# uc-vision/smart-tree

Measured on AMD Instinct MI355X. Metric: points/sec end-to-end (voxelize->sparse-UNet->skeleton), 1M-pt tree, higher is better.
Workload: dtype f32

## Files before the change

### include/smarttree_hip.h

```cpp
#ifndef SMARTTREE_HIP_H
#define SMARTTREE_HIP_H

#include <stdint.h>

#ifdef __cplusplus
extern "C" {
#endif

int st_version(void);
#define ST_SKELETON_STATS_ENTRIES 16
#define ST_SKELETON_TUNING_ENTRIES 24
int st_abi_entries(int what);
const char* st_last_error(void);
int64_t st_query_workspace(int op, int64_t a, int64_t b, int64_t c);

int64_t st_scan_workspace_bytes(int64_t n);
int st_scan_u32(const uint32_t* in, uint32_t* out, int64_t n, uint32_t* total, void* ws, int64_t ws_bytes, void* stream);
int64_t st_sort_workspace_bytes(int64_t n);
int st_sort_pairs_u32(uint32_t* keys, uint32_t* vals, int64_t n, int key_bits, void* ws, int64_t ws_bytes, void* stream);

int64_t st_voxelize_workspace_bytes(int64_t n_points, int max_blocks, int64_t max_voxels);
int st_voxelize_blocks(const float* xyz, const float* rgb, int64_t n, double voxel_size, double block_size,
                       double buffer_size, int min_points, int max_blocks, int64_t max_voxels, float* feats,
                       int32_t* coords, uint8_t* mask, int64_t* point_index, float* block_centres,
                       int64_t* n_voxels_host, int64_t* n_blocks_host, void* ws, int64_t ws_bytes, void* stream);

int64_t st_hash_capacity(int64_t n);
int st_build_coord_hash(const int32_t* coords, int64_t n, unsigned long long* keys, unsigned* vals, int64_t cap, void* stream);
int st_build_subm_rulebook(const int32_t* coords, int64_t n, const unsigned long long* keys, const unsigned* vals,
                           int64_t cap, int32_t* nbr , void* stream);
int64_t st_spatial_order_workspace_bytes(int64_t n);
int st_spatial_order(const int32_t* coords, int64_t n, int32_t* order , void* ws, int64_t ws_bytes, void* stream);
int st_move_rows(const void* src, int row_words, const int32_t* order, int64_t n, void* dst, int scatter, void* stream);
int64_t st_strided_workspace_bytes(int64_t n_fine);
int st_build_strided_outputs(const int32_t* coords, int64_t n, int64_t max_out, int32_t* out_coords,
                             unsigned long long* ckeys, unsigned* cvals, int64_t ccap, int64_t* n_out_host,
                             int32_t* extent_host , void* ws, int64_t ws_bytes, void* stream);
int st_build_strided_rulebook(const int32_t* coords, int64_t n, const unsigned long long* fkeys, const unsigned* fvals,
                              int64_t fcap, const int32_t* out_coords, int64_t n_out, const unsigned long long* ckeys,
                              const unsigned* cvals, int64_t ccap, const int32_t* extent_host,
                              int32_t* nbr_down , int32_t* nbr_up ,
                              int32_t* up_order ,
                              void* stream);

int st_sparse_conv_fwd(const float* x0, int c0, const float* x1, int cin, const int32_t* nbr, int K, int64_t n_out,
                       const float* w, int cout, const float* scale, const float* shift, const float* residual,
                       int relu, float* y, const int32_t* row_order ,
                       void* stream, int64_t nbr_stride );
int st_sparse_conv_mfma_fwd(const float* x0, int c0, const float* x1, int cin, const int32_t* nbr, int K, int64_t n_out,
                            const float* wp, int cout, const float* scale, const float* shift, const float* residual,
                            int relu, float* y, const int32_t* row_order ,
                            void* stream, int64_t nbr_stride ,
                            int variant );
int st_sparse_conv_b3_fwd(const float* x0, int c0, const float* x1, int cin, const int32_t* nbr, int K, int64_t n_out, const void* wq,
                          int cout, const float* scale, const float* shift, const float* residual, int relu, float* y,
                          const int32_t* row_order, void* stream, int64_t nbr_stride, int variant);
int st_sparse_conv_f16_fwd(const void* x0, int c0, const void* x1, int cin, const int32_t* nbr, int K, int64_t n_out,
                           const void* w, int cout, const float* scale, const float* shift, const void* residual, int relu,
                           void* y, int in_half, int out_half, const int32_t* row_order, void* stream, int64_t nbr_stride );

int64_t st_brick_pyramid_workspace_bytes(int64_t n0, int n_blocks, int coord_bound, int depth, const int64_t* caps);
int st_brick_pyramid(const int32_t* coords0 , int64_t n0, int n_blocks ,
                     int coord_bound , int depth, const int32_t* blk_seg ,
                     int nseg, const int64_t* caps ,
                     int32_t* order0 , int32_t* const* coords_out ,
                     int32_t* const* subm , int32_t* const* down ,
                     int32_t* const* up , int32_t* const* up_order ,
                     int64_t* counts_host , void* ws, int64_t ws_bytes, void* stream);
int st_head_param_floats(void);
int st_pointwise_mlp_heads(const float* x, int64_t n, const float* params, float* radius, float* direction,
                           float* class_l, float* medial_vector , int64_t* class_idx , void* stream);

int st_centre_cloud(const float* xyz, int64_t n, float* out, void* ws, int64_t ws_bytes, void* stream);
int st_medial_points(const float* xyz, const float* mv, int64_t n, float* medial, float* radius, void* stream);
int64_t st_knn_workspace_bytes(int64_t n_dst);
int st_knn_radius(const float* src, int64_t n1, const float* dst, int64_t n2, int K, float r, const float* bound,
                  int bound_mode, float cell_hint, int64_t* idx, float* dist, void* ws, int64_t ws_bytes, void* stream);
int64_t st_make_edges_workspace_bytes(int64_t n);
int st_make_edges(const int64_t* idx, const float* dist, int64_t n, int K, int64_t* edges, float* w,
                  int64_t* n_edges_host, void* ws, int64_t ws_bytes, void* stream);
int64_t st_connected_components_workspace_bytes(int64_t n);
int st_connected_components(const int64_t* edges, int64_t E, int64_t n, int32_t* labels, void* ws, int64_t ws_bytes, void* stream);
int64_t st_component_layout_workspace_bytes(int64_t n);
int st_component_layout(const int32_t* labels, int64_t n, int min_vertices, int32_t* comp_size, int32_t* comp_off,
                        int32_t* vert_order, int32_t* new_id, int64_t* n_comp_host, int64_t* n_kept_host, void* ws,
                        int64_t ws_bytes, void* stream);
int64_t st_component_csr_workspace_bytes(int64_t m);
int st_component_csr(const int64_t* edges, const float* w, int64_t E, const int32_t* new_id, int64_t m, uint32_t* row_off,
                     uint32_t* col, float* wgt, void* ws, int64_t ws_bytes, void* stream);
int64_t st_skeleton_workspace_bytes(int64_t m, int64_t n_comp);
int st_skeleton_components(int n_comp, const int32_t* comp_off, const int32_t* comp_size_host, int64_t m, const float* pts,
                           const float* rad, const float* ysurf, const uint32_t* row_off, const uint32_t* col,
                           const float* wgt, float grid_cell, int stages, int block_threads, float* dist, int32_t* pred,
                           int32_t* root_local, float* tree_dist, int32_t* branch_parent, int32_t* branch_off,
                           int32_t* branch_len, int32_t* n_branches, int32_t* path_verts, int32_t* branch_of,
                           int64_t* stats_host, void* ws, int64_t ws_bytes, void* stream);
#define ST_SKELETON_STAGE_ARGS                                                                                          \
    int n_comp, const int32_t *comp_off, const int32_t *comp_size_host, int64_t m, const float *pts, const float *rad, \
        const float *ysurf, const uint32_t *row_off, const uint32_t *col, const float *wgt, float grid_cell,           \
        int block_threads, float *dist, int32_t *pred, int32_t *root_local, float *tree_dist, int32_t *branch_parent,  \
        int32_t *branch_off, int32_t *branch_len, int32_t *n_branches, int32_t *path_verts, int32_t *branch_of,        \
        int64_t *stats_host, void *ws, int64_t ws_bytes, void *stream
int st_sssp(ST_SKELETON_STAGE_ARGS);
int st_tree_distance(ST_SKELETON_STAGE_ARGS);
int st_sample_tree(ST_SKELETON_STAGE_ARGS);
int64_t st_assemble_workspace_bytes(int64_t cap_b);
int st_assemble_branches(int n_comp, const int32_t* comp_off, const int32_t* n_branches, const int32_t* branch_parent,
                         const int32_t* branch_off, const int32_t* branch_len, const int32_t* path_verts,
                         const int32_t* vert_order, const float* medial, const float* radius, int32_t* tree_off,
                         int32_t* parent, int32_t* start, int32_t* length, float* xyz, float* rad, int64_t cap_b,
                         int64_t cap_p, int64_t* counts_host, void* ws, int64_t ws_bytes, void* stream);
int st_post_process(int n_trees, const int32_t* tree_off, const int32_t* parent, const int32_t* start, const int32_t* len,
                    float* xyz, const float* rad_in, float* rad_out, uint8_t* keep, uint8_t* repaired, uint8_t* smoothed,
                    int32_t* depth_scratch, int do_prune, float min_radius, float min_length, int do_repair, int do_smooth, int kernel_size,
                    void* stream);

int st_points_to_nearest_tube(const float* pts, int64_t n, const float* a, const float* b, const float* r1, const float* r2,
                              int64_t m, float* vec, int64_t* idx, float* rad, void* stream);

int64_t st_sample_tubes_workspace_bytes(int64_t m);
int st_sample_tubes_count(const float* a, const float* b, int64_t m, double spacing, int32_t* count, int32_t* off,
                          int64_t* total_host, void* ws, int64_t ws_bytes, void* stream);
int st_sample_tubes_fill(const float* a, const float* b, const float* r1, const float* r2, int64_t m, double spacing,
                         const int32_t* off, int64_t total, float* pts, float* rad, int32_t* tube_of, void* stream);
int64_t st_skeleton_match_workspace_bytes(int64_t n);
int st_skeleton_match(const float* pts, const float* rad, int64_t n, const float* a, const float* b, const float* r1,
                      const float* r2, int64_t m, const float* thr, int n_thr, int ref_mode, float* dist, int32_t* idx,
                      float* tube_rad, void* tally, void* ws, int64_t ws_bytes, void* stream);

int st_centre_cloud_seg(const float* xyz, int64_t n, const int32_t* seg_off, int nseg, float* out, void* ws,
                        int64_t ws_bytes , void* stream);
int st_centre_cloud_box_seg(const float* xyz, int64_t n, const int32_t* seg_off, int nseg, float* out, void* ws,
                            int64_t ws_bytes , void* stream, float* box_out);
int st_voxelize_blocks_box_seg(const float* xyz, const float* rgb, int64_t n, const int32_t* seg_off, int nseg,
                               double voxel_size, double block_size, double buffer_size, int min_points, int max_blocks,
                               int64_t max_voxels, float* feats, int32_t* coords, uint8_t* mask, int64_t* point_index,
                               float* block_centres, int32_t* blk_seg, int32_t* seg_vox_off, int32_t* seg_blk_off,
                               int64_t* n_voxels_host, int64_t* n_blocks_host, void* ws, int64_t ws_bytes, void* stream,
                               const float* centred_box );
int64_t st_voxelize_workspace_bytes_seg(int64_t n_points, int max_blocks, int64_t max_voxels, int nseg);
int st_voxelize_blocks_seg(const float* xyz, const float* rgb, int64_t n, const int32_t* seg_off, int nseg,
                           double voxel_size, double block_size, double buffer_size, int min_points, int max_blocks,
                           int64_t max_voxels, float* feats, int32_t* coords, uint8_t* mask, int64_t* point_index,
                           float* block_centres, int32_t* blk_seg ,
                           int32_t* seg_vox_off , int32_t* seg_blk_off , int64_t* n_voxels_host,
                           int64_t* n_blocks_host, void* ws, int64_t ws_bytes, void* stream);
int st_build_strided_outputs_seg(const int32_t* coords, int64_t n, int64_t max_out, int32_t* out_coords,
                                 unsigned long long* ckeys, unsigned* cvals, int64_t ccap, int64_t* n_out_host,
                                 int32_t* extent_host, const int32_t* blk_seg, int nseg, int32_t* ext_dev ,
                                 void* ws, int64_t ws_bytes, void* stream);
int st_build_strided_rulebook_seg(const int32_t* coords, int64_t n, const unsigned long long* fkeys, const unsigned* fvals,
                                  int64_t fcap, const int32_t* out_coords, int64_t n_out, const unsigned long long* ckeys,
                                  const unsigned* cvals, int64_t ccap, const int32_t* extent_host, int32_t* nbr_down,
                                  int32_t* nbr_up, int32_t* up_order, const int32_t* blk_seg, const int32_t* ext_dev,
// ... 124 lines not shown
```

### smart_tree_amd/_lib.py

```python
from __future__ import annotations

import ctypes
from ctypes import c_double, c_float, c_int, c_int64, c_void_p
from pathlib import Path

import torch

_PKG = Path(__file__).resolve().parent
LIB_PATH = _PKG / "libsmarttree_hip.so"

_LIB = None
_ALLOW_HOST_POINTERS = False

P = c_void_p
I64 = c_int64

SIGNATURES = {
    "st_version": (c_int, []),
    "st_abi_entries": (c_int, [c_int]),
    "st_last_error": (ctypes.c_char_p, []),
    "st_scan_workspace_bytes": (I64, [I64]),
    "st_scan_u32": (c_int, [P, P, I64, P, P, I64, P]),
    "st_sort_workspace_bytes": (I64, [I64]),
    "st_sort_pairs_u32": (c_int, [P, P, I64, c_int, P, I64, P]),
    "st_voxelize_workspace_bytes": (I64, [I64, c_int, I64]),
    "st_voxelize_blocks": (c_int, [P, P, I64, c_double, c_double, c_double, c_int, c_int, I64, P, P, P, P, P,
                                   ctypes.POINTER(I64), ctypes.POINTER(I64), P, I64, P]),
    "st_hash_capacity": (I64, [I64]),
    "st_build_coord_hash": (c_int, [P, I64, P, P, I64, P]),
    "st_build_subm_rulebook": (c_int, [P, I64, P, P, I64, P, P]),
    "st_strided_workspace_bytes": (I64, [I64]),
    "st_spatial_order_workspace_bytes": (I64, [I64]),
    "st_spatial_order": (c_int, [P, I64, P, P, I64, P]),
    "st_move_rows": (c_int, [P, c_int, P, I64, P, c_int, P]),
    "st_build_strided_outputs": (c_int, [P, I64, I64, P, P, P, I64, ctypes.POINTER(I64), ctypes.POINTER(ctypes.c_int32),
                                         P, I64, P]),
    "st_build_strided_rulebook": (c_int, [P, I64, P, P, I64, P, I64, P, P, I64, ctypes.POINTER(ctypes.c_int32), P, P, P, P]),
    "st_sparse_conv_fwd": (c_int, [P, c_int, P, c_int, P, c_int, I64, P, c_int, P, P, P, c_int, P, P, P, I64]),
    "st_sparse_conv_mfma_fwd": (c_int, [P, c_int, P, c_int, P, c_int, I64, P, c_int, P, P, P, c_int, P, P, P, I64, c_int]),
    "st_sparse_conv_b3_fwd": (c_int, [P, c_int, P, c_int, P, c_int, I64, P, c_int, P, P, P, c_int, P, P, P, I64, c_int]),
    "st_sparse_conv_f16_fwd": (c_int, [P, c_int, P, c_int, P, c_int, I64, P, c_int, P, P, P, c_int, P, c_int, c_int, P, P, I64]),
    "st_brick_pyramid_workspace_bytes": (I64, [I64, c_int, c_int, c_int, ctypes.POINTER(I64)]),
    "st_brick_pyramid": (c_int, [P, I64, c_int, c_int, c_int, P, c_int, ctypes.POINTER(I64), P, ctypes.POINTER(P), ctypes.POINTER(P),
                                 ctypes.POINTER(P), ctypes.POINTER(P), ctypes.POINTER(P), ctypes.POINTER(I64), P, I64, P]),
    "st_head_param_floats": (c_int, []),
    "st_pointwise_mlp_heads": (c_int, [P, I64, P, P, P, P, P, P, P]),
    "st_knn_workspace_bytes": (I64, [I64]),
    "st_knn_radius": (c_int, [P, I64, P, I64, c_int, c_float, P, c_int, c_float, P, P, P, I64, P]),
    "st_medial_points": (c_int, [P, P, I64, P, P, P]),
    "st_centre_cloud": (c_int, [P, I64, P, P, I64, P]),
    "st_make_edges_workspace_bytes": (I64, [I64]),
    "st_make_edges": (c_int, [P, P, I64, c_int, P, P, ctypes.POINTER(I64), P, I64, P]),
    "st_connected_components_workspace_bytes": (c_int64, [c_int64]),
    "st_connected_components": (c_int, [P, I64, I64, P, P, I64, P]),
    "st_component_layout_workspace_bytes": (I64, [I64]),
    "st_component_layout": (c_int, [P, I64, c_int, P, P, P, P, ctypes.POINTER(I64), ctypes.POINTER(I64), P, I64, P]),
    "st_component_csr_workspace_bytes": (I64, [I64]),
    "st_component_csr": (c_int, [P, P, I64, P, I64, P, P, P, P, I64, P]),
    "st_assemble_workspace_bytes": (c_int64, [c_int64]),
    "st_assemble_branches": (c_int, [c_int, P, P, P, P, P, P, P, P, P, P, P, P, P, P, P, c_int64, c_int64, P, P, c_int64, P]),
    "st_points_to_nearest_tube": (c_int, [P, c_int64, P, P, P, P, c_int64, P, P, P, P]),
    "st_post_process": (c_int, [c_int, P, P, P, P, P, P, P, P, P, P, P, c_int, c_float, c_float, c_int, c_int, c_int, P]),
    "st_sample_tubes_workspace_bytes": (I64, [I64]),
    "st_sample_tubes_count": (c_int, [P, P, I64, c_double, P, P, ctypes.POINTER(I64), P, I64, P]),
    "st_sample_tubes_fill": (c_int, [P, P, P, P, I64, c_double, P, I64, P, P, P, P]),
    "st_skeleton_match_workspace_bytes": (I64, [I64]),
    "st_skeleton_match": (c_int, [P, P, I64, P, P, P, P, I64, P, c_int, c_int, P, P, P, P, P, I64, P]),
    "st_skeleton_workspace_bytes": (I64, [I64, I64]),
    "st_synth_points_seg": (c_int, [P, P, P, P, P, P, c_int, P, P, P, P, P, P, P, P, P, P]),
    "st_synth_philox": (None, [P, P, P]),
    "st_prediction_metrics_tally_ints": (I64, [c_int, c_int, c_int]),
    "st_prediction_metrics_tally_sums": (I64, [c_int]),
    "st_prediction_metrics_workspace_bytes": (I64, [I64, c_int, c_int]),
    "st_prediction_metrics": (c_int, [P, P, P, c_int, P, c_int, P, I64, P, c_int, c_int, c_int, P, c_int, P, c_int, P, P, P, I64, P]),
    "st_render_workspace_bytes": (I64, [c_int, c_int, c_int]),
    "st_render_clear": (c_int, [c_int, c_int, c_int, P, I64, P]),
    "st_render_points": (c_int, [P, P, I64, I64, c_float, P, c_int, c_int, c_int, c_float, P, I64, P]),
    "st_render_segments": (c_int, [P, P, P, P, I64, I64, c_float, P, c_int, c_int, c_int, c_float, P, I64, P]),
    "st_render_resolve": (c_int, [P, c_int, c_int, c_int, c_int, c_float, c_int, P, P, P, P, I64, P]),
    "st_centre_cloud_seg": (c_int, [P, I64, P, c_int, P, P, I64, P]),
    "st_centre_cloud_box_seg": (c_int, [P, I64, P, c_int, P, P, I64, P, P]),
    "st_voxelize_blocks_box_seg": (c_int, [P, P, I64, P, c_int, c_double, c_double, c_double, c_int, c_int, I64, P, P, P, P, P, P, P, P,
                                           ctypes.POINTER(I64), ctypes.POINTER(I64), P, I64, P, P]),
    "st_voxelize_workspace_bytes_seg": (I64, [I64, c_int, I64, c_int]),
    "st_voxelize_blocks_seg": (c_int, [P, P, I64, P, c_int, c_double, c_double, c_double, c_int, c_int, I64, P, P, P, P, P, P, P, P,
                                       ctypes.POINTER(I64), ctypes.POINTER(I64), P, I64, P]),
    "st_voxelize_cloud_workspace_bytes": (I64, [I64, I64, c_int]),
    "st_voxelize_cloud_seg": (c_int, [P, P, I64, P, c_int, c_double, I64, P, P, P, P, P, ctypes.POINTER(I64), P, I64, P]),
    "st_loss_workspace_bytes": (I64, []),
    "st_loss_forward": (c_int, [P, P, P, c_int, P, c_int, P, I64, c_int, c_int, ctypes.POINTER(ctypes.c_double), P, I64, P]),
    "st_build_strided_outputs_seg": (c_int, [P, I64, I64, P, P, P, I64, ctypes.POINTER(I64), ctypes.POINTER(ctypes.c_int32),
                                             P, c_int, P, P, I64, P]),
    "st_build_strided_rulebook_seg": (c_int, [P, I64, P, P, I64, P, I64, P, P, I64, ctypes.POINTER(ctypes.c_int32), P, P, P, P, P, P]),
    "st_knn_workspace_bytes_seg": (I64, [I64, c_int]),
    "st_knn_radius_seg": (c_int, [P, I64, P, I64, c_int, c_float, P, c_int, c_float, P, P, P, P, c_int, P, I64, P, c_float]),
    "st_radius_count_seg": (c_int, [P, I64, P, I64, c_int, c_float, P, c_int, c_float, P, P, P, c_int, P, I64, P, c_float, P]),
    "st_connected_components_knn": (c_int, [P, I64, c_int, P, P, P, I64, P]),
    "st_component_csr_knn": (c_int, [P, P, I64, c_int, P, P, I64, P, P, P, P, I64, P]),
    "st_component_csr_knn_workspace_bytes": (I64, [I64, I64, c_int]),
    "st_make_edges_seg": (c_int, [P, P, I64, c_int, P, P, ctypes.POINTER(I64), P, c_int, P, I64, P]),
    "st_component_layout_seg": (c_int, [P, I64, c_int, P, c_int, P, P, P, P, P, P, P, ctypes.POINTER(I64), ctypes.POINTER(I64), P, I64, P,
                                        ctypes.POINTER(I64)]),
    "st_skeleton_workspace_bytes_seg": (I64, [I64, I64, c_int]),
    "st_skeleton_components_seg": (c_int, [c_int, P, P, P, c_int, I64, P, P, P, P, P, P, c_float, c_int, c_int, P, P, P, P, P, P, P, P,
                                           P, P, ctypes.POINTER(I64), P, I64, P, ctypes.POINTER(I64)]),
    "st_post_process_seg": (c_int, [c_int, P, P, P, P, P, P, P, P, P, P, P, c_int, c_float, c_float, c_int, c_int, c_int, P, c_int, P]),
    "st_loss_backward": (c_int, [P, P, P, c_int, P, c_int, P, I64, c_int, c_int, c_double, c_double, P, P, P, P, P]),
    "st_sparse_conv_wgrad_workspace_bytes": (I64, [c_int, c_int, c_int, I64]),
    "st_sparse_conv_wgrad": (c_int, [P, c_int, P, c_int, P, c_int, I64, I64, P, c_int, P, P, I64, P]),
    "st_sparse_conv_h_fwd": (c_int, [P, c_int, P, c_int, P, c_int, I64, I64, P, c_int, P, P]),
    "st_sparse_conv_wgrad_h_workspace_bytes": (I64, [c_int, c_int, c_int, I64]),
    "st_sparse_conv_wgrad_h": (c_int, [P, c_int, P, c_int, P, c_int, I64, I64, P, c_int, P, P, I64, P]),
    "st_move_rows_h": (c_int, [P, c_int, P, I64, P, c_int, P]),
    "st_bn_workspace_bytes": (I64, [I64, c_int]),
    "st_bn_stats": (c_int, [P, c_int, I64, c_int, P, P, I64, P]),
    "st_bn_apply": (c_int, [P, c_int, I64, c_int, P, P, P, P, P, P]),
    "st_bn_backward_stats": (c_int, [P, P, c_int, I64, c_int, P, P, P, P, I64, P]),
    "st_bn_backward_apply": (c_int, [P, P, c_int, I64, c_int, P, P, P, P, P, P, P]),
    "st_bridge_components_workspace_bytes": (I64, [I64, I64, c_int]),
    "st_bridge_components_seg": (c_int, [P, I64, P, I64, P, P, I64, P, c_int, c_float, P, P, I64, ctypes.POINTER(I64),
                                         ctypes.POINTER(I64), P, I64, P]),
    "st_skeleton_components": (c_int, [c_int, P, P, I64, P, P, P, P, P, P, c_float, c_int, c_int, P, P, P, P, P, P, P, P,
                                       P, P, ctypes.POINTER(I64), P, I64, P]),
    "st_segment_workspace_bytes": (I64, [I64, I64, c_int]),
    "st_segment_points_seg": (c_int, [P, I64, P, P, P, P, P, I64, P, c_int, c_float, c_int, P, P, P, P, P, P, I64, P]),
}


ENQUEUE_ONLY = frozenset({
    "st_version", "st_abi_entries", "st_last_error", "st_scan_workspace_bytes", "st_sort_workspace_bytes", "st_voxelize_workspace_bytes",
    "st_hash_capacity", "st_strided_workspace_bytes", "st_head_param_floats", "st_knn_workspace_bytes",
    "st_make_edges_workspace_bytes", "st_connected_components_workspace_bytes", "st_component_layout_workspace_bytes",
    "st_component_csr_workspace_bytes", "st_assemble_workspace_bytes", "st_skeleton_workspace_bytes",
    "st_build_coord_hash", "st_build_subm_rulebook", "st_build_strided_rulebook", "st_sparse_conv_fwd",
    "st_sparse_conv_mfma_fwd", "st_sparse_conv_b3_fwd", "st_sparse_conv_f16_fwd", "st_pointwise_mlp_heads", "st_medial_points", "st_centre_cloud",
    "st_connected_components", "st_component_csr", "st_post_process", "st_knn_radius", "st_brick_pyramid_workspace_bytes",
    "st_centre_cloud_seg", "st_centre_cloud_box_seg", "st_voxelize_workspace_bytes_seg", "st_build_strided_rulebook_seg", "st_knn_workspace_bytes_seg",
    "st_knn_radius_seg", "st_skeleton_workspace_bytes_seg", "st_post_process_seg", "st_radius_count_seg",
    "st_voxelize_cloud_workspace_bytes", "st_loss_workspace_bytes", "st_spatial_order_workspace_bytes", "st_spatial_order", "st_connected_components_knn", "st_component_csr_knn", "st_component_csr_knn_workspace_bytes", "st_move_rows",
    "st_loss_backward", "st_sparse_conv_wgrad_workspace_bytes", "st_sparse_conv_wgrad",
    "st_sparse_conv_h_fwd", "st_sparse_conv_wgrad_h_workspace_bytes", "st_sparse_conv_wgrad_h", "st_move_rows_h",
    "st_bn_workspace_bytes", "st_bn_stats", "st_bn_apply", "st_bn_backward_stats", "st_bn_backward_apply",
    "st_sample_tubes_workspace_bytes", "st_sample_tubes_fill", "st_skeleton_match_workspace_bytes", "st_skeleton_match",
    "st_synth_points_seg", "st_synth_philox",
    "st_prediction_metrics_tally_ints", "st_prediction_metrics_tally_sums", "st_prediction_metrics_workspace_bytes", "st_prediction_metrics",
    "st_render_workspace_bytes", "st_render_clear", "st_render_points", "st_render_segments", "st_render_resolve",
    "st_bridge_components_workspace_bytes", "st_segment_workspace_bytes", "st_segment_points_seg",
})


NOWAIT_VARIANTS = ("st_make_edges", "st_assemble_branches", "st_make_edges_seg")


class StRenderItem(ctypes.Structure):
    _fields_ = [("count", c_int64), ("mode", ctypes.c_int32), ("n_classes", ctypes.c_int32), ("data", c_void_p), ("cmap", c_void_p),
                ("lo", c_float), ("hi", c_float), ("rgb", c_float * 3), ("reserved", c_float)]


class _Bound:

    def __init__(self, cdll):
        self._cdll = cdll

    def __getattr__(self, name):
        return getattr(self._cdll, name)


def declare(cdll, pydll=None):
    out = _Bound(cdll) if pydll is not None else cdll
    for name, (res, args) in SIGNATURES.items():
        for handle in ((cdll, pydll) if pydll is not None else (cdll,)):
            fn = getattr(handle, name)
            fn.restype = res
            fn.argtypes = args
        if pydll is not None:
            setattr(out, name, getattr(pydll if name in ENQUEUE_ONLY else cdll, name))
    for name in NOWAIT_VARIANTS:
        setattr(out, name + "_nowait", getattr(pydll if pydll is not None else cdll, name))
    return out


def lib():
    global _LIB
    if _LIB is None:
        if not LIB_PATH.exists():
            raise RuntimeError(
                f"{LIB_PATH} is missing: the HIP extension has not been built. "
                "Run `python -c 'import __graft_entry__ as g; g.build()'` (needs hipcc). "
                "smart_tree_amd has no CPU fallback.")
        import os
        if os.environ.get("ST_CDLL_ONLY") == "1":
            _LIB = declare(ctypes.CDLL(str(LIB_PATH)))
        else:
            _LIB = declare(ctypes.CDLL(str(LIB_PATH)), ctypes.PyDLL(str(LIB_PATH)))
    return _LIB


class StError(RuntimeError):
    pass


def check(rc: int) -> None:
    if rc != 0:
        raise StError(f"smarttree_hip error {rc}: {lib().st_last_error().decode()}")


def ptr(t):
    if t is None:
        return None
    if not t.is_cuda and not _ALLOW_HOST_POINTERS:
        raise StError("smart_tree_amd kernels need tensors on the GPU (got a CPU tensor); there is no CPU fallback")
    if not t.is_contiguous():
        raise StError("smart_tree_amd kernels need contiguous tensors")
    return t.data_ptr()


_HAS_GPU = None
_RAW_STREAM = getattr(torch._C, "_cuda_getCurrentRawStream", None)


def stream(device=None):
    global _HAS_GPU
    if _HAS_GPU is None:
        _HAS_GPU = torch.cuda.is_available()
    if _HAS_GPU and not _ALLOW_HOST_POINTERS:
        if _RAW_STREAM is not None:
            idx = device.index if isinstance(device, torch.device) and device.index is not None else torch.cuda.current_device()
            return _RAW_STREAM(idx)
        return torch.cuda.current_stream(device).cuda_stream
    return None
# ... 8 lines not shown
```

### smart_tree_amd/csrc/brick.hip

```cpp
#include "st_common.h"
#include "st_grid.h"
#include "st_rule.h"

#define BK_BLOCK 256
#define BK_MAX_DEPTH 6

struct alignas(16) BkRec {
    unsigned long long mask[8];
    unsigned char cum[8];
    unsigned tidx;
    unsigned cum_hi;
};

struct BkLevel {
    int mb;
    unsigned mt;
    int64_t ntab;
    uint32_t* p;
    BkRec* rec;
    uint32_t* base;
    int64_t slot_cap;
    int64_t* n_slots;
    int64_t* n_vox;
};

struct BkState {
    int ext[ST_MAX_SEG][3];
    unsigned fail;
};

__device__ __forceinline__ unsigned bk_spread3(unsigned v) {
    v &= 0x7fu;
    v = (v | (v << 8)) & 0x0000700fu;
    v = (v | (v << 4)) & 0x000430c3u;
    v = (v | (v << 2)) & 0x00049249u;
    return v;
}
__device__ __forceinline__ unsigned bk_compact3(unsigned v) {
    v &= 0x00049249u;
    v = (v | (v >> 2)) & 0x000430c3u;
    v = (v | (v >> 4)) & 0x0000700fu;
    v = (v | (v >> 8)) & 0x0000007fu;
    return v;
}
__device__ __forceinline__ unsigned bk_morton(int bz, int by, int bx) { return (bk_spread3((unsigned)bz) << 2) | (bk_spread3((unsigned)by) << 1) | bk_spread3((unsigned)bx); }
__device__ __forceinline__ unsigned bk_cum(const BkRec& r, int w) { return (unsigned)r.cum[w] + (((r.cum_hi >> w) & 1u) << 8); }

__device__ __forceinline__ int64_t bk_tab(const BkLevel& L, int b, int z, int y, int x) {
    return (int64_t)b * L.mt + bk_morton(z >> 3, y >> 3, x >> 3);
}
__device__ __forceinline__ int bk_lookup(const BkLevel& L, int b, int z, int y, int x) {
    const int lim = 8 << L.mb;
    if ((unsigned)z >= (unsigned)lim || (unsigned)y >= (unsigned)lim || (unsigned)x >= (unsigned)lim) return -1;
    const int64_t t = bk_tab(L, b, z, y, x);
    const uint32_t s = L.p[t];
    if (L.p[t + 1] == s) return -1;
    const BkRec& r = L.rec[s];
    const int w = z & 7, bit = ((y & 7) << 3) | (x & 7);
    const unsigned long long m = r.mask[w];
    if (!((m >> bit) & 1ull)) return -1;
    return (int)(L.base[s] + bk_cum(r, w) + (unsigned)__popcll(m & ((1ull << bit) - 1ull)));
}

#define BK_LOOP(i, n) for (int64_t i = (int64_t)blockIdx.x * blockDim.x + threadIdx.x; i < (n); i += (int64_t)gridDim.x * blockDim.x)

static inline unsigned bk_grid(int64_t n) {
    int64_t g = st_div_up(n > 0 ? n : 1, BK_BLOCK);
    return (unsigned)(g < 16384 ? g : 16384);
}

__global__ void __launch_bounds__(BK_BLOCK) k_bk_mark0(const int32_t* coords, int64_t n, BkLevel L, BkState* st, const int32_t* blk_seg,
                                                       int nseg, int nblk) {
    __shared__ int m[ST_MAX_SEG * 3];
    st_ext_clear(m, nseg);
    const int lim = 8 << L.mb;
    BK_LOOP(i, n) {
        const int4 c = reinterpret_cast<const int4*>(coords)[i];
        if ((unsigned)c.x >= (unsigned)nblk || (unsigned)c.y >= (unsigned)lim || (unsigned)c.z >= (unsigned)lim || (unsigned)c.w >= (unsigned)lim) {
            atomicOr(&st->fail, 2u);
            continue;
        }
        L.p[bk_tab(L, c.x, c.y, c.z, c.w)] = 1u;
        st_ext_offer(m, blk_seg ? blk_seg[c.x] : 0, c.y, c.z, c.w);
    }
    st_ext_flush(m, nseg, &st->ext[0][0]);
// ... 202 lines not shown
                word |= (unsigned long long)rb << (8 * oy);
            }
        }
        Lc.rec[s].mask[w] = word;
    }
}

__global__ void __launch_bounds__(BK_BLOCK) k_bk_emit(BkLevel L, int32_t* coords, int64_t cap, BkState* st) {
    if (st->fail) return;
    const int64_t ns = *L.n_slots < L.slot_cap ? *L.n_slots : L.slot_cap;
    BK_LOOP(idx, ns * 8) {
        const int64_t s = idx >> 3;
        const int w = (int)(idx & 7);
        const BkRec& r = L.rec[s];
        unsigned long long m = r.mask[w];
        if (m == 0ull) continue;
        const unsigned t = r.tidx, mc = t & (L.mt - 1u);
        const int b = (int)(t >> (3 * L.mb));
        const int z = (int)(bk_compact3(mc >> 2) << 3) | w, y0 = (int)(bk_compact3(mc >> 1) << 3), x0 = (int)(bk_compact3(mc) << 3);
        int64_t row = (int64_t)L.base[s] + bk_cum(r, w);
        while (m) {
            const int bit = __ffsll((long long)m) - 1;
            m &= m - 1ull;
            if (row < cap) reinterpret_cast<int4*>(coords)[row] = make_int4(b, z, y0 + (bit >> 3), x0 + (bit & 7));
            else atomicOr(&st->fail, 1u);
            row++;
        }
    }
}

__global__ void __launch_bounds__(BK_BLOCK) k_bk_updown(const int32_t* coords, const int64_t* n_dev, int64_t cap_f, BkLevel Lc, const BkState* st,
                                                        int level, const int32_t* blk_seg, const int64_t* m_dev, int64_t cap_c,
                                                        int32_t* nbr_up, int32_t* nbr_down, uint32_t* parity_count) {
    __shared__ uint32_t hist[8];
    if (st->fail) return;
    if (threadIdx.x < 8) hist[threadIdx.x] = 0;
    __syncthreads();
    const int64_t n = *n_dev < cap_f ? *n_dev : cap_f;
    const int64_t m = *m_dev < cap_c ? *m_dev : cap_c;
    BK_LOOP(i, n) {
        const int4 c4 = reinterpret_cast<const int4*>(coords)[i];
        const int b = c4.x, c[3] = {c4.y, c4.z, c4.w};
        const int* e = st->ext[blk_seg ? blk_seg[b] : 0];
        const int omax[3] = {st_rule_omax(e[0], level), st_rule_omax(e[1], level), st_rule_omax(e[2], level)};
        atomicAdd(&hist[st_rule_parity_class(c[0], c[1], c[2])], 1u);
        int64_t t_have = -1;
        int slot = -1, w_have = -1;
        unsigned bs = 0u, cu = 0u;
        unsigned long long mw = 0ull;
        const int limc = 8 << Lc.mb;
#pragma unroll
        for (int kz = 0; kz < 3; kz++)
#pragma unroll
            for (int j = 0; j < 9; j++) {
                const int k = kz * 9 + j;
                int r = -1, o[3];
                if (st_rule_out(c, k, omax, o)) {
                    const int oz = o[0], oy = o[1], ox = o[2];
                    if (oz < limc && oy < limc && ox < limc) {
                        const int64_t tc = bk_tab(Lc, b, oz, oy, ox);
                        if (tc != t_have) {
                            t_have = tc;
                            w_have = -1;
                            const uint32_t sc = Lc.p[tc];
                            slot = Lc.p[tc + 1] != sc ? (int)sc : -1;
                            bs = slot >= 0 ? Lc.base[slot] : 0u;
                        }
                        if (slot >= 0) {
                            const int wz = oz & 7;
                            if (wz != w_have) { w_have = wz; const BkRec& rc = Lc.rec[slot]; mw = rc.mask[wz]; cu = bs + bk_cum(rc, wz); }
                            const int bit = ((oy & 7) << 3) | (ox & 7);
                            if ((mw >> bit) & 1ull) r = (int)(cu + (unsigned)__popcll(mw & ((1ull << bit) - 1ull)));
                        }
                    }
                }
                nbr_up[(int64_t)k * cap_f + i] = r;
                if (r >= 0 && r < m) nbr_down[(int64_t)k * cap_c + r] = (int32_t)i;
            }
    }
    __syncthreads();
    if (threadIdx.x < 8 && hist[threadIdx.x]) atomicAdd(&parity_count[threadIdx.x], hist[threadIdx.x]);
}

struct BkPlan {
    int depth;
    int mb[BK_MAX_DEPTH + 1];
    int64_t ntab[BK_MAX_DEPTH + 1], slot_cap[BK_MAX_DEPTH + 1];
};

static bool bk_plan(int64_t n0, int n_blocks, int coord_bound, int depth, const int64_t* caps, BkPlan* P) {
    if (depth < 0 || depth > BK_MAX_DEPTH || n_blocks < 1 || coord_bound < 1) return false;
    P->depth = depth;
    int bound = coord_bound;
    for (int l = 0; l <= depth; l++) {
        int nb = (bound + 7) / 8, mb = 0;
        while ((1 << mb) < nb) mb++;
        if (mb > 7) return false;
        P->mb[l] = mb;
        P->ntab[l] = (int64_t)n_blocks << (3 * mb);
        if (P->ntab[l] >= (1ll << 31)) return false;
        const int64_t cap = l == 0 ? n0 : caps[l];
        if ((l == 0 && caps && caps[0] > cap ? caps[0] : cap) >= ST_RULE_ROW_LIMIT) return false;
        P->slot_cap[l] = cap < P->ntab[l] ? cap : P->ntab[l];
        bound = (bound - 1) / 2 + 1;
    }
    return true;
}

struct BkLayout {
    BkState* st;
    int64_t* counts;
    uint32_t* p[BK_MAX_DEPTH + 1];
    BkRec* rec[BK_MAX_DEPTH + 1];
    uint32_t* base[BK_MAX_DEPTH + 1];
    char* scan_ws;
    int64_t scan_bytes;
};

static void bk_layout(StArena& a, const BkPlan& P, BkLayout* Y) {
    Y->st = a.take<BkState>(1);
    Y->counts = a.take<int64_t>(2 * (BK_MAX_DEPTH + 1));
    int64_t scan_n = 1;
    for (int l = 0; l <= P.depth; l++) {
        Y->p[l] = a.take<uint32_t>(P.ntab[l] + 1);
        Y->rec[l] = a.take<BkRec>(P.slot_cap[l]);
        Y->base[l] = a.take<uint32_t>(P.slot_cap[l] + 1);
        if (P.ntab[l] + 1 > scan_n) scan_n = P.ntab[l] + 1;
        if (P.slot_cap[l] + 1 > scan_n) scan_n = P.slot_cap[l] + 1;
    }
    Y->scan_bytes = st_scan_ws_bytes(scan_n);
    Y->scan_ws = a.take<char>(Y->scan_bytes);
}

extern "C" int64_t st_brick_pyramid_workspace_bytes(int64_t n0, int n_blocks, int coord_bound, int depth, const int64_t* caps) {
    BkPlan P;
    if (!bk_plan(n0 > 0 ? n0 : 1, n_blocks, coord_bound, depth, caps, &P)) return 0;
    StArena a(nullptr, 0);
    BkLayout Y;
    bk_layout(a, P, &Y);
    return a.used;
}

extern "C" int st_brick_pyramid(const int32_t* coords0, int64_t n0, int n_blocks, int coord_bound, int depth, const int32_t* blk_seg,
                                int nseg, const int64_t* caps, int32_t* order0, int32_t* const* coords_out, int32_t* const* subm,
                                int32_t* const* down, int32_t* const* up, int32_t* const* up_order, int64_t* counts_host, void* ws,
                                int64_t ws_bytes, void* stream_) {
    hipStream_t stream = (hipStream_t)stream_;
    for (int l = 0; l <= depth && l <= BK_MAX_DEPTH; l++) counts_host[l] = 0;
    if (n0 <= 0) return ST_OK;
    ST_REQUIRE(nseg >= 1 && nseg <= ST_MAX_SEG && (nseg == 1 || blk_seg), "brick pyramid: 1 <= clouds per batch <= %d", ST_MAX_SEG);
    ST_REQUIRE(caps && caps[0] >= n0, "brick pyramid: caps[0] must hold the input voxels");
    if (nseg == 1) blk_seg = nullptr;
    BkPlan P;
    ST_REQUIRE(bk_plan(n0, n_blocks, coord_bound, depth, caps, &P), "brick pyramid: cannot be sized for %d blocks of %d^3 cells", n_blocks, coord_bound);
    StArena a(ws, ws_bytes);
    BkLayout Y;
    bk_layout(a, P, &Y);
    if (!a.ok() || !Y.scan_ws) {
        st_set_error("brick pyramid: workspace too small (%lld < %lld)", (long long)ws_bytes, (long long)a.used);
        return ST_ERR_WORKSPACE;
    }
    (void)hipMemsetAsync(Y.st, 0, sizeof(BkState), stream);
    (void)hipMemsetAsync(Y.counts, 0, 2 * (BK_MAX_DEPTH + 1) * sizeof(int64_t), stream);
    BkLevel L[BK_MAX_DEPTH + 1];
    for (int l = 0; l <= depth; l++) {
        L[l].mb = P.mb[l]; L[l].mt = 1u << (3 * P.mb[l]); L[l].ntab = P.ntab[l]; L[l].p = Y.p[l]; L[l].rec = Y.rec[l];
        L[l].base = Y.base[l]; L[l].slot_cap = P.slot_cap[l]; L[l].n_slots = &Y.counts[2 * l]; L[l].n_vox = &Y.counts[2 * l + 1];
        (void)hipMemsetAsync(Y.p[l], 0, (P.ntab[l] + 1) * sizeof(uint32_t), stream);
    }
    auto close_flags = [&](int l) -> int {
        ST_TRY(st_exclusive_scan_u32(L[l].p, L[l].p, L[l].ntab + 1, reinterpret_cast<uint32_t*>(L[l].n_slots), Y.scan_ws, Y.scan_bytes, stream));
        hipLaunchKernelGGL(k_bk_init_rec, dim3(bk_grid(L[l].ntab)), dim3(BK_BLOCK), 0, stream, L[l], Y.st);
        return ST_OK;
    };
    auto close_bits = [&](int l) -> int {
        hipLaunchKernelGGL(k_bk_count, dim3(bk_grid(L[l].slot_cap)), dim3(BK_BLOCK), 0, stream, L[l]);
        ST_TRY(st_exclusive_scan_u32(L[l].base, L[l].base, L[l].slot_cap, reinterpret_cast<uint32_t*>(L[l].n_vox), Y.scan_ws, Y.scan_bytes,
                                     stream, L[l].n_slots));
        return ST_OK;
    };
    hipLaunchKernelGGL(k_bk_mark0, dim3(bk_grid(n0)), dim3(BK_BLOCK), 0, stream, coords0, n0, L[0], Y.st, blk_seg, nseg, n_blocks);
    ST_TRY(close_flags(0));
    hipLaunchKernelGGL(k_bk_bits0, dim3(bk_grid(n0)), dim3(BK_BLOCK), 0, stream, coords0, n0, L[0], (const BkState*)Y.st);
    ST_TRY(close_bits(0));
    hipLaunchKernelGGL(k_bk_order0, dim3(bk_grid(n0)), dim3(BK_BLOCK), 0, stream, coords0, n0, L[0], order0, coords_out[0], (const BkState*)Y.st);
    for (int l = 0;; l++) {
        const int64_t cap = caps[l];
        hipLaunchKernelGGL(k_bk_subm, dim3(bk_grid(cap)), dim3(BK_BLOCK), 0, stream, (const int32_t*)coords_out[l], (const int64_t*)L[l].n_vox, cap,
                           L[l], subm[l], (const BkState*)Y.st);
        if (l == depth) break;
        const int64_t cap_c = caps[l + 1];
        hipLaunchKernelGGL(k_bk_coarse_mark, dim3(bk_grid(L[l].slot_cap)), dim3(BK_BLOCK), 0, stream, L[l], L[l + 1], (const BkState*)Y.st, l, blk_seg);
        ST_TRY(close_flags(l + 1));
        hipLaunchKernelGGL(k_bk_coarse_stencil, dim3(bk_grid(L[l + 1].slot_cap * 8)), dim3(BK_BLOCK), 0, stream, L[l], L[l + 1], (const BkState*)Y.st, l,
                           blk_seg);
        ST_TRY(close_bits(l + 1));
        hipLaunchKernelGGL(k_bk_emit, dim3(bk_grid(L[l + 1].slot_cap * 8)), dim3(BK_BLOCK), 0, stream, L[l + 1], coords_out[l + 1], cap_c, Y.st);
        (void)hipMemsetAsync(down[l], 0xff, 27 * cap_c * sizeof(int32_t), stream);
        uint32_t* pc = reinterpret_cast<uint32_t*>(up_order[l] + cap);
        (void)hipMemsetAsync(pc, 0, 16 * sizeof(uint32_t), stream);
        hipLaunchKernelGGL(k_bk_updown, dim3(bk_grid(cap)), dim3(BK_BLOCK), 0, stream, (const int32_t*)coords_out[l], (const int64_t*)L[l].n_vox, cap,
                           L[l + 1], (const BkState*)Y.st, l, blk_seg, (const int64_t*)L[l + 1].n_vox, cap_c, up[l], down[l], pc);
        st_rule_parity_order(coords_out[l], cap, L[l].n_vox, &Y.st->fail, pc, up_order[l], stream);
    }
    struct { int64_t counts[2 * (BK_MAX_DEPTH + 1)]; } hc;
    unsigned hfail = 0;
    (void)hipMemcpyAsync(&hc, Y.counts, sizeof(hc), hipMemcpyDeviceToHost, stream);
    (void)hipMemcpyAsync(&hfail, &Y.st->fail, sizeof(unsigned), hipMemcpyDeviceToHost, stream);
    st_stream_wait(stream);
    ST_CHECK_LAUNCH();
    ST_REQUIRE(!(hfail & 2u), "brick pyramid: a coordinate lies outside the declared bounds (%d blocks, %d cells per axis)", n_blocks, coord_bound);
    for (int l = 0; l <= depth; l++) counts_host[l] = hc.counts[2 * l + 1];
    bool over = (hfail & 1u) != 0;
    for (int l = 0; l <= depth; l++) over = over || hc.counts[2 * l + 1] > caps[l] || hc.counts[2 * l] > P.slot_cap[l];
    if (over) {
        st_set_error("brick pyramid: a level needs more rows than its capacity (caps)");
        return ST_ERR_WORKSPACE;
    }
    ST_REQUIRE(hc.counts[1] == n0, "brick pyramid: %lld distinct voxels among %lld input rows (duplicate coordinates)", (long long)hc.counts[1],
               (long long)n0);
    return ST_OK;
}
```

### smart_tree_amd/csrc/prims.hip

```cpp
#include <cstdarg>

#include "st_common.h"

static thread_local char g_err[512] = "";

void st_set_error(const char* fmt, ...) {
    va_list ap;
    va_start(ap, fmt);
    vsnprintf(g_err, sizeof(g_err), fmt, ap);
    va_end(ap);
}

extern "C" const char* st_last_error(void) { return g_err; }
void st_stream_wait(hipStream_t stream) { (void)hipStreamSynchronize(stream); }

extern "C" int st_version(void) { return 111; }

#define SCAN_BLOCK 256
#define SCAN_ITEMS 16
#define SCAN_TILE (SCAN_BLOCK * SCAN_ITEMS)
#define SCAN_DIRECT_BLOCKS 1024

__device__ __forceinline__ void scan_load(const uint32_t* in, int64_t base, int64_t n, uint32_t (&v)[SCAN_ITEMS]) {
    if (base + SCAN_ITEMS <= n && ((((uintptr_t)in) & 15) == 0)) {
        const uint4* p = reinterpret_cast<const uint4*>(in + base);
#pragma unroll
        for (int q = 0; q < SCAN_ITEMS / 4; q++) {
            const uint4 t = p[q];
            v[4 * q] = t.x; v[4 * q + 1] = t.y; v[4 * q + 2] = t.z; v[4 * q + 3] = t.w;
        }
    } else {
#pragma unroll
        for (int i = 0; i < SCAN_ITEMS; i++) v[i] = base + i < n ? in[base + i] : 0u;
    }
}

__global__ void __launch_bounds__(SCAN_BLOCK) k_scan_reduce(const uint32_t* in, uint32_t* block_sums, int64_t n, const int64_t* n_dev) {
    __shared__ uint32_t lds[SCAN_BLOCK / 64 + 1];
    if (n_dev) {
        const int64_t m = *n_dev;
        n = m < n ? m : n;
        if ((int64_t)blockIdx.x * SCAN_TILE >= n) { if (threadIdx.x == 0) block_sums[blockIdx.x] = 0u; return; }
    }
    int64_t base = (int64_t)blockIdx.x * SCAN_TILE + (int64_t)threadIdx.x * SCAN_ITEMS;
    uint32_t v[SCAN_ITEMS];
    scan_load(in, base, n, v);
    uint32_t s = 0;
#pragma unroll
    for (int i = 0; i < SCAN_ITEMS; i++) s += v[i];
    uint32_t total;
    block_exclusive_scan(s, lds, &total);
    if (threadIdx.x == 0) block_sums[blockIdx.x] = total;
}

__global__ void __launch_bounds__(SCAN_BLOCK) k_scan_apply(const uint32_t* in, uint32_t* out, const uint32_t* block_sums,
                                                           int64_t n, uint32_t* total_out, int sums_scanned, const int64_t* n_dev) {
    __shared__ uint32_t lds[SCAN_BLOCK / 64 + 1];
    if (n_dev) {
        const int64_t m = *n_dev;
        n = m < n ? m : n;
        const bool last_live = (int64_t)blockIdx.x * SCAN_TILE < n && ((int64_t)blockIdx.x + 1) * SCAN_TILE >= n;
        if ((int64_t)blockIdx.x * SCAN_TILE >= n && !(n == 0 && blockIdx.x == 0)) return;
        if (total_out && !last_live && !(n == 0)) total_out = nullptr;
    } else if (blockIdx.x != gridDim.x - 1) {
        total_out = nullptr;
    }
    uint32_t carry;
    if (sums_scanned) {
        carry = block_sums[blockIdx.x];
    } else {
        uint32_t pre = 0;
        for (int64_t j = threadIdx.x; j < (int64_t)blockIdx.x; j += SCAN_BLOCK) pre += block_sums[j];
        block_exclusive_scan(pre, lds, &carry);
    }
    int64_t base = (int64_t)blockIdx.x * SCAN_TILE + (int64_t)threadIdx.x * SCAN_ITEMS;
    uint32_t v[SCAN_ITEMS];
    scan_load(in, base, n, v);
    uint32_t s = 0;
#pragma unroll
    for (int i = 0; i < SCAN_ITEMS; i++) s += v[i];
    uint32_t total;
    uint32_t ex = block_exclusive_scan(s, lds, &total) + carry;
    if (base + SCAN_ITEMS <= n && ((((uintptr_t)out) & 15) == 0)) {
        uint4* p = reinterpret_cast<uint4*>(out + base);
#pragma unroll
        for (int q = 0; q < SCAN_ITEMS / 4; q++) {
            uint4 t;
            t.x = ex; ex += v[4 * q];
            t.y = ex; ex += v[4 * q + 1];
            t.z = ex; ex += v[4 * q + 2];
            t.w = ex; ex += v[4 * q + 3];
            p[q] = t;
        }
    } else {
#pragma unroll
        for (int i = 0; i < SCAN_ITEMS; i++) {
            if (base + i < n) out[base + i] = ex;
            ex += v[i];
        }
// ... 193 lines not shown
```

### smart_tree_amd/csrc/rulebook.hip

```cpp
#include "st_common.h"
#include "st_grid.h"
#include "st_rule.h"

#define RB_BLOCK 256

static inline unsigned rb_grid(int64_t n) {
    int64_t g = st_div_up(n > 0 ? n : 1, RB_BLOCK);
    return (unsigned)(g < 8192 ? g : 8192);
}

__global__ void __launch_bounds__(RB_BLOCK) k_rb_insert(const int32_t* coords, int64_t n, unsigned long long* keys,
                                                        unsigned* vals, unsigned long long cap, unsigned* fail) {
    for (int64_t i = (int64_t)blockIdx.x * blockDim.x + threadIdx.x; i < n; i += (int64_t)gridDim.x * blockDim.x) {
        unsigned long long key = st_pack_key(coords[4 * i], coords[4 * i + 1], coords[4 * i + 2], coords[4 * i + 3]);
        if (!st_hash_insert_min(keys, vals, cap, key, (unsigned)i) && fail) atomicOr(fail, 1u);
    }
}

__global__ void __launch_bounds__(RB_BLOCK) k_rb_subm(const int32_t* coords, int64_t n, const unsigned long long* keys,
                                                      const unsigned* vals, unsigned long long cap, int32_t* nbr) {
    for (int64_t o = (int64_t)blockIdx.x * blockDim.x + threadIdx.x; o < n; o += (int64_t)gridDim.x * blockDim.x) {
        const int b = coords[4 * o], z = coords[4 * o + 1], y = coords[4 * o + 2], x = coords[4 * o + 3];
#pragma unroll
        for (int dz = -1; dz <= 1; dz++) {
// ... 285 lines not shown
                                        int32_t* extent_host , void* ws, int64_t ws_bytes,
                                        void* stream_) {
    return st_build_strided_outputs_seg(coords, n, max_out, out_coords, ckeys, cvals, ccap, n_out_host, extent_host, nullptr, 1,
                                        nullptr, ws, ws_bytes, stream_);
}

extern "C" int st_build_strided_rulebook_seg(const int32_t* coords, int64_t n, const unsigned long long* fkeys,
                                         const unsigned* fvals, int64_t fcap, const int32_t* out_coords, int64_t n_out,
                                         const unsigned long long* ckeys, const unsigned* cvals, int64_t ccap,
                                         const int32_t* extent_host, int32_t* nbr_down, int32_t* nbr_up,
                                         int32_t* up_order , const int32_t* blk_seg, const int32_t* ext_dev,
                                         void* stream_) {
    hipStream_t stream = (hipStream_t)stream_;
    if (n == 0) return ST_OK;
    ST_REQUIRE((blk_seg == nullptr) == (ext_dev == nullptr), "strided: blk_seg and ext_dev go together");
    ST_REQUIRE(up_order == nullptr || n < ST_RULE_ROW_LIMIT, "strided: the tagged row order holds at most 2^28 rows");
    (void)fkeys; (void)fvals; (void)fcap;
    if (n_out) (void)hipMemsetAsync(nbr_down, 0xff, 27 * n_out * sizeof(int32_t), stream);
    uint32_t* pc = up_order ? reinterpret_cast<uint32_t*>(up_order + n) : nullptr;
    if (pc) (void)hipMemsetAsync(pc, 0, 16 * sizeof(uint32_t), stream);
    hipLaunchKernelGGL(k_rb_up_nbr, dim3(rb_grid(n)), dim3(RB_BLOCK), 0, stream, coords, n, extent_host[0], extent_host[1],
                       extent_host[2], ckeys, cvals, (unsigned long long)ccap, nbr_up, nbr_down, n_out, pc, blk_seg, ext_dev);
    if (pc) st_rule_parity_order(coords, n, nullptr, nullptr, pc, up_order, stream);
    ST_CHECK_LAUNCH();
    return ST_OK;
}

extern "C" int st_build_strided_rulebook(const int32_t* coords, int64_t n, const unsigned long long* fkeys,
                                         const unsigned* fvals, int64_t fcap, const int32_t* out_coords, int64_t n_out,
                                         const unsigned long long* ckeys, const unsigned* cvals, int64_t ccap,
                                         const int32_t* extent_host, int32_t* nbr_down, int32_t* nbr_up,
                                         int32_t* up_order , void* stream_) {
    return st_build_strided_rulebook_seg(coords, n, fkeys, fvals, fcap, out_coords, n_out, ckeys, cvals, ccap, extent_host,
                                         nbr_down, nbr_up, up_order, nullptr, nullptr, stream_);
}

__device__ __forceinline__ uint32_t rb_spread3(uint32_t v) {
    v &= 0x3ffu;
    v = (v | (v << 16)) & 0x030000ffu;
    v = (v | (v << 8)) & 0x0300f00fu;
    v = (v | (v << 4)) & 0x030c30c3u;
    v = (v | (v << 2)) & 0x09249249u;
    return v;
}
__global__ void __launch_bounds__(RB_BLOCK) k_rb_morton_keys(const int32_t* coords, int64_t n, uint32_t* keys, uint32_t* vals) {
    for (int64_t i = (int64_t)blockIdx.x * blockDim.x + threadIdx.x; i < n; i += (int64_t)gridDim.x * blockDim.x) {
        keys[i] = (rb_spread3((uint32_t)coords[4 * i + 1]) << 2) | (rb_spread3((uint32_t)coords[4 * i + 2]) << 1) |
                  rb_spread3((uint32_t)coords[4 * i + 3]);
        vals[i] = (uint32_t)i;
    }
}
__global__ void __launch_bounds__(RB_BLOCK) k_rb_block_keys(const int32_t* coords, int64_t n, const uint32_t* vals, uint32_t* keys) {
    for (int64_t i = (int64_t)blockIdx.x * blockDim.x + threadIdx.x; i < n; i += (int64_t)gridDim.x * blockDim.x)
        keys[i] = (uint32_t)coords[4 * (int64_t)vals[i]];
}

extern "C" int64_t st_spatial_order_workspace_bytes(int64_t n) {
    StArena a(nullptr, 0);
    a.take<uint32_t>(n);
    a.take<char>(st_sort_ws_bytes(n));
    return a.used;
}

extern "C" int st_spatial_order(const int32_t* coords, int64_t n, int32_t* order, void* ws, int64_t ws_bytes, void* stream_) {
    hipStream_t stream = (hipStream_t)stream_;
    if (n <= 0) return ST_OK;
    ST_REQUIRE(n < (1ll << 31), "spatial_order: too many voxels");
    StArena a(ws, ws_bytes);
    uint32_t* keys = a.take<uint32_t>(n);
    const int64_t sb = st_sort_ws_bytes(n);
    char* sw = a.take<char>(sb);
    if (!keys || !sw) { st_set_error("spatial_order: workspace too small (%lld < %lld)", (long long)ws_bytes, (long long)a.used); return ST_ERR_WORKSPACE; }
    uint32_t* vals = reinterpret_cast<uint32_t*>(order);
    hipLaunchKernelGGL(k_rb_morton_keys, dim3(rb_grid(n)), dim3(RB_BLOCK), 0, stream, coords, n, keys, vals);
    ST_TRY(st_radix_sort_pairs_u32(keys, vals, n, 30, sw, sb, stream));
    hipLaunchKernelGGL(k_rb_block_keys, dim3(rb_grid(n)), dim3(RB_BLOCK), 0, stream, coords, n, (const uint32_t*)vals, keys);
    ST_TRY(st_radix_sort_pairs_u32(keys, vals, n, 16, sw, sb, stream));
    ST_CHECK_LAUNCH();
    return ST_OK;
}

template <int VEC>
__global__ void __launch_bounds__(RB_BLOCK) k_rb_move_rows(const uint32_t* __restrict__ src, int row_words, const int32_t* __restrict__ order,
                                                           int64_t n, uint32_t* __restrict__ dst, int scatter) {
    const int per_row = row_words / VEC;
    const int64_t total = n * per_row;
    for (int64_t t = (int64_t)blockIdx.x * blockDim.x + threadIdx.x; t < total; t += (int64_t)gridDim.x * blockDim.x) {
        const int64_t p = t / per_row;
        const int c = (int)(t % per_row) * VEC;
        const int64_t o = order[p];
        const int64_t from = (scatter ? p : o) * row_words + c, to = (scatter ? o : p) * row_words + c;
        if (VEC == 4) *reinterpret_cast<uint4*>(dst + to) = *reinterpret_cast<const uint4*>(src + from);
        else dst[to] = src[from];
    }
}

extern "C" int st_move_rows(const void* src, int row_words, const int32_t* order, int64_t n, void* dst, int scatter, void* stream_) {
    hipStream_t stream = (hipStream_t)stream_;
    if (n <= 0) return ST_OK;
    ST_REQUIRE(row_words >= 1 && row_words <= 256, "move_rows: rows of 1..256 words");
    const bool vec = row_words % 4 == 0 && ((((uintptr_t)src) | ((uintptr_t)dst)) & 15) == 0;
    const int64_t total = n * (vec ? row_words / 4 : row_words);
    if (vec)
        hipLaunchKernelGGL((k_rb_move_rows<4>), dim3(rb_grid(total)), dim3(RB_BLOCK), 0, stream, (const uint32_t*)src, row_words, order, n,
                           (uint32_t*)dst, scatter);
    else
        hipLaunchKernelGGL((k_rb_move_rows<1>), dim3(rb_grid(total)), dim3(RB_BLOCK), 0, stream, (const uint32_t*)src, row_words, order, n,
                           (uint32_t*)dst, scatter);
    ST_CHECK_LAUNCH();
    return ST_OK;
}
```

### smart_tree_amd/csrc/skeleton.hip

```cpp
#include "st_common.h"
#include "st_grid.h"
#include "smarttree_hip.h"

#include <atomic>

#define SK_MAX_WAVES 16
#define SK_EMPTY64 0xffffffffffffffffull
#define SK_WIDE_BLOCK 256
#define SK_SSSP_BLOCKS 2048
#define SK_MARK 0xfffffffeu
#define SK_ANC 64

struct SkJob {
    unsigned seq, done, quit;
    int len, id, csz, nrows, ny, x0, y0, z0, z1, path_off;
    float rp;
    unsigned gone;
    unsigned alive;
};

struct SkArgs {
    int C;
    int64_t m;
    const int* comp_off;
// ... 1428 lines not shown
    A->s_cursor = a.take<int>(C);
    A->s_wide = a.take<int>(C);
    H->sort_keys = a.take<unsigned>(m);
    A->order = a.take<unsigned>(m);
    A->order_init = a.take<float>(m);
    H->sort_bytes = st_sort_ws_bytes(m);
    H->sort_ws = a.take<char>(H->sort_bytes);
    A->blk_first = a.take<int>(C);
    A->blk_count = a.take<int>(C);
    A->blk_comp = a.take<int>(C + st_div_up(m, 1024));
    A->hl_comp = a.take<int>(SK_HELP_POOL);
    A->hl_rank = a.take<int>(SK_HELP_POOL);
    A->c_nhelp = a.take<int>(C);
    A->jobs = a.take<SkJob>(C);
    A->grid = a.take<StGrid>(1);
    A->cell_start = a.take<uint32_t>(sk_grid_cells(nseg, m) + 1);
    A->recs = a.take<float4>(m);
    H->gws_bytes = st_grid_ws_bytes(m, sk_grid_cells(nseg, m));
    H->gws = a.take<char>(H->gws_bytes);
}

#define ST_TUNE_DEFAULT INT64_MIN
#define ST_TUNE_ENTRIES 24
#define SK_MAX_LAUNCH_BATCH 32
struct SkTuning {
    float prune_factor = 1.0f, grid_mean_mult = 1.0f;
    int small_work = SK_SMALL_WORK, iters_per_launch = SK_ITERS_PER_LAUNCH, launch_batch = 24, local_items = 0, wave_work = SK_WAVE_WORK, long_mode = 1;
    int sssp_hops = 6 , sssp_batch = 36 , sssp_lanes = 32, sssp_first = 2, sssp_blocks = SK_SSSP_BLOCKS, sssp_lcap = SK_LQ;
    int sssp_coop = 0, helpers = -1;
    long long help_lifetime_us = SK_HELP_LIFETIME_US, help_timeout_us = SK_HELP_TIMEOUT_US, help_announce_us = SK_HELP_ANNOUNCE_US;
    bool small_work_set = false, iters_set = false, long_set = false, launch_set = false;
    long long* ticks = nullptr;
    explicit SkTuning(const int64_t* t) {
        if (!t) return;
        auto has = [&](int i) { return t[i] != ST_TUNE_DEFAULT; };
        if (has(0)) prune_factor = (float)t[0] / 1000.0f;
        if (has(1)) { small_work = (int)t[1]; small_work_set = true; }
        if (has(2)) { iters_per_launch = (int)t[2]; iters_set = true; }
        if (has(3)) { launch_batch = t[3] < 1 ? 1 : (t[3] > SK_MAX_LAUNCH_BATCH ? SK_MAX_LAUNCH_BATCH : (int)t[3]); launch_set = true; }
        if (has(4)) local_items = (int)t[4];
        if (has(5)) wave_work = (int)t[5];
        if (has(6)) sssp_hops = t[6] < 1 ? 1 : (int)t[6];
        if (has(7)) sssp_batch = t[7] < 1 ? 1 : (t[7] > 64 ? 64 : (int)t[7]);
        if (has(8)) sssp_lanes = t[8] == 64 ? 64 : (t[8] == 32 ? 32 : 16);
        if (has(9)) sssp_first = t[9] < 1 ? 1 : (t[9] > 8 ? 8 : (int)t[9]);
        if (has(10)) sssp_blocks = t[10] < 1 ? 1 : (t[10] > 8192 ? 8192 : (int)t[10]);
        if (has(11)) grid_mean_mult = (float)t[11] / 100.0f;
        if (has(12)) { sssp_coop = (t[12] & 1) != 0; if (t[12] >= 256) helpers = (int)(t[12] >> 8) - 1; }
        if (has(13)) sssp_lcap = t[13] == 0 ? -SK_LQ : (t[13] > SK_LQ ? SK_LQ : (int)t[13]);
        if (has(14)) { long_mode = t[14] != 0; long_set = true; }
        if (has(15)) ticks = (long long*)(intptr_t)t[15];
        if (has(16)) help_lifetime_us = t[16] < 0 ? 0 : t[16];
        if (has(17)) help_timeout_us = t[17] < 0 ? 0 : t[17];
        if (has(18)) help_announce_us = t[18] < 0 ? 0 : t[18];
    }
};

static std::atomic<int> g_helpers_out{0};
static int sk_cu_count() {
    int dev = 0, cus = 0;
    if (hipGetDevice(&dev) != hipSuccess || hipDeviceGetAttribute(&cus, hipDeviceAttributeMultiprocessorCount, dev) != hipSuccess) {
        (void)hipGetLastError();
        return 0;
    }
    return cus;
}
static int sk_helper_cap() {
    const int cap = sk_cu_count() * 5 / 8;
    return cap < SK_HELP_POOL ? cap : SK_HELP_POOL;
}
struct SkHelperLease {
    int n = 0;
    int take(int want) {
        const int cap = sk_helper_cap();
        int cur = g_helpers_out.load();
        do { n = want < cap - cur ? want : cap - cur; if (n <= 0) { n = 0; return 0; } } while (!g_helpers_out.compare_exchange_weak(cur, cur + n));
        return n;
    }
    ~SkHelperLease() { if (n > 0) g_helpers_out.fetch_sub(n); }
};

static_assert(ST_TUNE_ENTRIES == ST_SKELETON_TUNING_ENTRIES, "header and library disagree about the tuning array");
extern "C" int st_abi_entries(int what) {
    return what == 0 ? ST_SKELETON_STATS_ENTRIES : (what == 1 ? ST_SKELETON_TUNING_ENTRIES : (what == 2 ? ST_MAX_SEG : -1));
}

extern "C" int64_t st_skeleton_workspace_bytes_seg(int64_t m, int64_t n_comp, int nseg) {
    StArena a(nullptr, 0);
    SkArgs A;
    SkHost H;
    sk_layout(a, m > 0 ? m : 1, n_comp > 0 ? n_comp : 1, &A, &H, nseg);
    return a.used;
}
extern "C" int64_t st_skeleton_workspace_bytes(int64_t m, int64_t n_comp) { return st_skeleton_workspace_bytes_seg(m, n_comp, 1); }

template <class T>
static inline T* sk_rw(const T* p) { return const_cast<T*>(p); }

static inline unsigned sk_vgrid(int64_t m) {
    int64_t g = st_div_up(m > 0 ? m : 1, SK_WIDE_BLOCK);
    return (unsigned)(g < 2048 ? g : 2048);
}

static int sk_read(void* dst, const void* src, size_t bytes, hipStream_t stream) {
    (void)hipMemcpyAsync(dst, src, bytes, hipMemcpyDeviceToHost, stream);
    st_stream_wait(stream);
    ST_CHECK_LAUNCH();
    return ST_OK;
}

extern "C" int st_skeleton_components_seg(int n_comp, const int32_t* comp_off, const int32_t* comp_seg,
                                          const int32_t* vert_seg_off, int nseg, int64_t m,
                                      const float* pts, const float* rad, const float* ysurf, const uint32_t* row_off,
                                      const uint32_t* col, const float* wgt, float grid_cell, int stages, int block_threads,
                                      float* dist, int32_t* pred, int32_t* root_local, float* tree_dist,
                                      int32_t* branch_parent, int32_t* branch_off, int32_t* branch_len, int32_t* n_branches,
                                      int32_t* path_verts, int32_t* branch_of, int64_t* stats_host, void* ws,
                                      int64_t ws_bytes, void* stream_, const int64_t* tuning) {
    hipStream_t stream = (hipStream_t)stream_;
    const bool time_select = stats_host && stats_host[7] != 0;
    if (stats_host) for (int i = 0; i < ST_SKELETON_STATS_ENTRIES; i++) if (i != 7) stats_host[i] = 0;
    if (n_comp <= 0 || m <= 0) return ST_OK;
    ST_REQUIRE(!(stages & 2) || tree_dist != nullptr, "skeleton: stage 2 needs a tree_dist buffer");
    if (block_threads <= 0) block_threads = 1024;
    ST_REQUIRE(block_threads % 64 == 0 && block_threads <= 1024, "skeleton: block_threads must be a multiple of 64, <= 1024");
    ST_REQUIRE(m < (1ll << 28), "skeleton: at most 2^28 graph vertices");
    ST_REQUIRE(nseg >= 1 && nseg <= ST_MAX_SEG, "skeleton: 1 <= clouds per batch <= %d", ST_MAX_SEG);
    ST_REQUIRE(nseg == 1 || (comp_seg && vert_seg_off), "skeleton: a batch needs comp_seg and vert_seg_off");
    if (nseg == 1) { comp_seg = nullptr; vert_seg_off = nullptr; }
    StArena a(ws, ws_bytes);
    SkArgs A;
    SkHost H;
    memset(&A, 0, sizeof(A));
    sk_layout(a, m, n_comp, &A, &H, nseg);
    if (!a.ok() || !H.gws) {
        st_set_error("skeleton: workspace too small (%lld < %lld)", (long long)ws_bytes, (long long)a.used);
        return ST_ERR_WORKSPACE;
    }
    A.C = n_comp; A.m = m; A.comp_off = comp_off; A.comp_seg = comp_seg; A.pts = pts; A.rad = rad; A.ysurf = ysurf;
    A.row_off = row_off; A.col = col; A.wgt = wgt; A.help_bits = A.term_bits + sk_term_words(m, n_comp); A.fcnt = A.cnt + 8;
    A.dist = dist; A.pred = pred; A.root_local = root_local; A.tree_dist = tree_dist;
    A.branch_parent = branch_parent; A.branch_off = branch_off; A.branch_len = branch_len; A.n_branches = n_branches;
    A.path_verts = path_verts; A.branch_of = branch_of;
    const SkTuning T(tuning);
    A.ticks = T.ticks;
    A.help_lifetime = T.help_lifetime_us * 100; A.help_timeout = T.help_timeout_us * 100; A.help_announce = T.help_announce_us * 100;
    A.prune_factor = T.prune_factor; A.small_work = T.small_work; A.iters_per_launch = T.iters_per_launch; A.local_items = T.local_items; A.wave_work = T.wave_work; A.long_mode = T.long_mode;
    int first_launches = T.launch_batch;
    SkHelperLease lease;
    int helpers_want = 0;
    if ((stages & 4) && T.helpers != 0 && block_threads >= 256 && m >= SK_HELP_MIN && (T.helpers > 0 || nseg <= SK_HELP_SEGS))
        helpers_want = T.helpers > 0 ? T.helpers : (int)st_min64(SK_HELP_POOL, m / SK_HELP_PER);
    const bool helpers_avail = lease.take(helpers_want) > 0;
    if (nseg > 1 || helpers_avail) {
        if (!T.small_work_set) A.small_work = 1 << 20;
        if (!T.iters_set) A.iters_per_launch = 1 << 20;
        if (!T.launch_set && A.long_mode && A.iters_per_launch >= (1 << 20)) first_launches = 1;
    } else if (!T.long_set) {
        A.long_mode = 0;
    }

    const unsigned vg = sk_vgrid(m);
    const unsigned fg = (unsigned)st_min64(st_div_up(m, SK_WIDE_BLOCK), T.sssp_blocks);
    unsigned h[8 + 3 * (SK_FS + 1)];
    int64_t sssp_rounds = 0;
    const bool defer_plateaus = (stages & 1) && (stages & 4) && !(stages & 2);
    auto resolve_plateaus = [&](unsigned unresolved) -> int {
// ... 176 lines not shown
```

### smart_tree_amd/csrc/sparse_conv.hip

```cpp
#include "st_common.h"
#include "st_rule.h"

#define CONV_BLOCK 256

typedef _Float16 st_h;
typedef _Float16 st_v4h __attribute__((ext_vector_type(4)));
__device__ __forceinline__ float4 conv_load4(const float* p) { return *reinterpret_cast<const float4*>(p); }
__device__ __forceinline__ float4 conv_load4(const st_h* p) {
    const st_v4h v = *reinterpret_cast<const st_v4h*>(p);
    return make_float4((float)v.x, (float)v.y, (float)v.z, (float)v.w);
}
__device__ __forceinline__ void conv_store4(float* p, float a, float b, float c, float d) { *reinterpret_cast<float4*>(p) = make_float4(a, b, c, d); }
__device__ __forceinline__ void conv_store4(st_h* p, float a, float b, float c, float d) {
    *reinterpret_cast<st_v4h*>(p) = st_v4h{(st_h)a, (st_h)b, (st_h)c, (st_h)d};
}

template <int CIN, int COT, class TIN = float, class TOUT = float>
__global__ void __launch_bounds__(CONV_BLOCK) k_sparse_conv(const TIN* __restrict__ x0, int c0,
                                                            const TIN* __restrict__ x1, const int32_t* __restrict__ nbr,
                                                            int K, int64_t n_out, int64_t nstride, const float* __restrict__ w, int cout,
                                                            const float* __restrict__ scale, const float* __restrict__ shift,
                                                            const float* __restrict__ residual, int relu,
                                                            TOUT* __restrict__ y, const int32_t* __restrict__ row_order) {
    const int co_tiles = cout / COT;
// ... 53 lines not shown
#pragma unroll 2
            for (int ci = 0; ci < CIN; ci += 4) {
                const TIN* row = ci < c0 ? x0 + (int64_t)idx * c0 + ci : x1 + (int64_t)idx * c1 + (ci - c0);
                const float4 v = conv_load4(row);
                const float xs[4] = {v.x, v.y, v.z, v.w};
#pragma unroll
                for (int j = 0; j < 4; j++)
#pragma unroll
                    for (int c = 0; c < COT; c++) acc[c] = fmaf(xs[j], wk[(ci + j) * cout + c], acc[c]);
            }
        } else {
            for (int ci = 0; ci < CIN; ci++) {
                const float xv = (float)x0[(int64_t)idx * CIN + ci];
#pragma unroll
                for (int c = 0; c < COT; c++) acc[c] = fmaf(xv, wk[ci * cout + c], acc[c]);
            }
        }
    }
    if (!active) return;
#pragma unroll
    for (int c = 0; c < COT; c++) {
        float v = acc[c];
        if (scale) v = fmaf(v, scale[co0 + c], shift[co0 + c]);
        if (residual) v += residual[o * cout + co0 + c];
        if (relu) v = v > 0.0f ? v : 0.0f;
        acc[c] = v;
    }
    TOUT* out = y + o * cout + co0;
    if (COT % 4 == 0) {
#pragma unroll
        for (int c = 0; c < COT; c += 4) conv_store4(out + c, acc[c], acc[c + 1], acc[c + 2], acc[c + 3]);
    } else {
#pragma unroll
        for (int c = 0; c < COT; c++) out[c] = (TOUT)acc[c];
    }
}

__global__ void __launch_bounds__(CONV_BLOCK) k_sparse_conv_any(const float* __restrict__ x0, int c0, const float* __restrict__ x1, int cin,
                                                                const int32_t* __restrict__ nbr, int K, int64_t n_out, int64_t nstride,
                                                                const float* __restrict__ w, int cout, const float* __restrict__ scale,
                                                                const float* __restrict__ shift, const float* __restrict__ residual, int relu,
                                                                float* __restrict__ y, const int32_t* __restrict__ row_order) {
    const int64_t pos = (int64_t)blockIdx.x * CONV_BLOCK + threadIdx.x;
    if (pos >= n_out) return;
    const int co0 = (int)blockIdx.y * 4, nco = cout - co0 < 4 ? cout - co0 : 4;
    const int32_t entry = row_order ? row_order[pos] : 0;
    const int64_t o = row_order ? (int64_t)st_rule_row(entry) : pos;
    const uint32_t live = st_rule_live_offsets(entry, K);
    const int c1 = cin - c0;
    float acc[4] = {0.0f, 0.0f, 0.0f, 0.0f};
    for (int k = 0; k < K; k++) {
        if (K <= 32 && !((live >> k) & 1u)) continue;
        const int idx = nbr ? nbr[(int64_t)k * nstride + o] : (int)o;
        if (idx < 0) continue;
        const float* __restrict__ wk = w + (int64_t)k * cin * cout + co0;
        for (int ci = 0; ci < cin; ci++) {
            const float xv = ci < c0 ? x0[(int64_t)idx * c0 + ci] : x1[(int64_t)idx * c1 + (ci - c0)];
            for (int c = 0; c < nco; c++) acc[c] = fmaf(xv, wk[(int64_t)ci * cout + c], acc[c]);
        }
    }
    for (int c = 0; c < nco; c++) {
        float v = acc[c];
        if (scale) v = fmaf(v, scale[co0 + c], shift[co0 + c]);
        if (residual) v += residual[o * cout + co0 + c];
        if (relu) v = v > 0.0f ? v : 0.0f;
        y[o * cout + co0 + c] = v;
    }
}

struct ConvArgs {
    const void* x0;
    int c0;
    const void* x1;
    const int32_t* nbr;
    int K;
    int64_t n_out, nstride;
    const void* w;
    const float *scale, *shift;
    const void* residual;
    int relu;
    void* y;
    const int32_t* row_order;
    hipStream_t stream;
};

static int conv_check_args(ConvArgs* a, int cin) {
    if (a->nstride <= 0) a->nstride = a->n_out;
    ST_REQUIRE(a->K >= 1 && (a->nbr != nullptr || a->K == 1), "conv: a NULL neighbour table means pointwise (K = 1)");
    ST_REQUIRE(a->c0 > 0 && a->c0 <= cin && (a->c0 == cin || a->x1 != nullptr), "conv: bad concat split");
    ST_REQUIRE((a->scale == nullptr) == (a->shift == nullptr), "conv: scale and shift go together");
    return ST_OK;
}

template <int CIN, int COT, class TIN = float, class TOUT = float>
static int conv_launch(const ConvArgs& a, int cout) {
    int64_t blocks = st_div_up(a.n_out, CONV_BLOCK) * (cout / COT);
    hipLaunchKernelGGL((k_sparse_conv<CIN, COT, TIN, TOUT>), dim3((unsigned)blocks), dim3(CONV_BLOCK), 0, a.stream, (const TIN*)a.x0, a.c0,
                       (const TIN*)a.x1, a.nbr, a.K, a.n_out, a.nstride, (const float*)a.w, cout, a.scale, a.shift, (const float*)a.residual,
                       a.relu, (TOUT*)a.y, a.row_order);
    ST_CHECK_LAUNCH();
    return ST_OK;
}

typedef float st_v4f __attribute__((ext_vector_type(4)));
#define MF_BLOCK 256

struct MfF32 {
    typedef float T;
    typedef float4 W, A, B;
    static constexpr int CHUNK = 16, PLANES = 1;
    typedef float4 Row;
    static __device__ __forceinline__ Row no_row() { return make_float4(0.0f, 0.0f, 0.0f, 0.0f); }
    static __device__ __forceinline__ Row load_row(const T* row) { return *reinterpret_cast<const float4*>(row); }
    static __device__ __forceinline__ A fragment(const Row& r) { return r; }
    static __device__ __forceinline__ B load_b(const W* wc, int) { return *wc; }
    static __device__ __forceinline__ void mma(const A& a, const B& b, st_v4f& d) {
        d = __builtin_amdgcn_mfma_f32_16x16x4f32(a.x, b.x, d, 0, 0, 0);
        d = __builtin_amdgcn_mfma_f32_16x16x4f32(a.y, b.y, d, 0, 0, 0);
        d = __builtin_amdgcn_mfma_f32_16x16x4f32(a.z, b.z, d, 0, 0, 0);
        d = __builtin_amdgcn_mfma_f32_16x16x4f32(a.w, b.w, d, 0, 0, 0);
    }
};

typedef __bf16 st_bf8 __attribute__((ext_vector_type(8)));
struct StB3 { uint4 h, m, l; };
__device__ __forceinline__ unsigned b3_pack_hi(unsigned u0, unsigned u1) { return __builtin_amdgcn_perm(u1, u0, 0x07060302u); }
__device__ __forceinline__ void b3_split_pair(float a0, float a1, unsigned* h, unsigned* m, unsigned* l) {
    const unsigned u0 = __float_as_uint(a0), u1 = __float_as_uint(a1);
    *h = b3_pack_hi(u0, u1);
    const float r0 = a0 - __uint_as_float(u0 & 0xffff0000u), r1 = a1 - __uint_as_float(u1 & 0xffff0000u);
    const unsigned v0 = __float_as_uint(r0), v1 = __float_as_uint(r1);
    *m = b3_pack_hi(v0, v1);
    const float s0 = r0 - __uint_as_float(v0 & 0xffff0000u), s1 = r1 - __uint_as_float(v1 & 0xffff0000u);
    *l = b3_pack_hi(__float_as_uint(s0), __float_as_uint(s1));
}
__device__ __forceinline__ StB3 b3_split8(float4 a, float4 b) {
    StB3 o;
    b3_split_pair(a.x, a.y, &o.h.x, &o.m.x, &o.l.x);
    b3_split_pair(a.z, a.w, &o.h.y, &o.m.y, &o.l.y);
    b3_split_pair(b.x, b.y, &o.h.z, &o.m.z, &o.l.z);
    b3_split_pair(b.z, b.w, &o.h.w, &o.m.w, &o.l.w);
    return o;
}
__device__ __forceinline__ st_bf8 b3_bf8(uint4 v) { return __builtin_bit_cast(st_bf8, v); }

struct MfB3 {
    typedef float T;
    typedef uint4 W;
    typedef StB3 A;
    struct B { st_bf8 h, m, l; };
    static constexpr int CHUNK = 32, PLANES = 3;
    struct Row { float4 lo4, hi4; };
    static __device__ __forceinline__ Row no_row() { return Row{make_float4(0.0f, 0.0f, 0.0f, 0.0f), make_float4(0.0f, 0.0f, 0.0f, 0.0f)}; }
    static __device__ __forceinline__ Row load_row(const T* row) { return Row{*reinterpret_cast<const float4*>(row), *reinterpret_cast<const float4*>(row + 4)}; }
    static __device__ __forceinline__ A fragment(const Row& r) { return b3_split8(r.lo4, r.hi4); }
    static __device__ __forceinline__ B load_b(const W* wc, int plane) { return B{b3_bf8(wc[0]), b3_bf8(wc[plane]), b3_bf8(wc[2 * plane])}; }
    static __device__ __forceinline__ void mma(const A& a, const B& b, st_v4f& d) {
        const st_bf8 ah = b3_bf8(a.h), am = b3_bf8(a.m), al = b3_bf8(a.l);
        d = __builtin_amdgcn_mfma_f32_16x16x32_bf16(al, b.h, d, 0, 0, 0);
        d = __builtin_amdgcn_mfma_f32_16x16x32_bf16(ah, b.l, d, 0, 0, 0);
        d = __builtin_amdgcn_mfma_f32_16x16x32_bf16(am, b.m, d, 0, 0, 0);
        d = __builtin_amdgcn_mfma_f32_16x16x32_bf16(am, b.h, d, 0, 0, 0);
        d = __builtin_amdgcn_mfma_f32_16x16x32_bf16(ah, b.m, d, 0, 0, 0);
        d = __builtin_amdgcn_mfma_f32_16x16x32_bf16(ah, b.h, d, 0, 0, 0);
    }
};

typedef _Float16 st_v8h __attribute__((ext_vector_type(8)));
struct MfF16 {
    typedef st_h T;
// ... 50 lines not shown
        bool any = false;
#pragma unroll
        for (int t = 0; t < RT; t++) {
            idx[t] = (!PAIR || k < K) && orow[t] >= 0 && ((live[t] >> k) & 1u) ? (nbr ? nbr[(int64_t)k * nstride + orow[t]] : (int)orow[t]) : -1;
            any = any || idx[t] >= 0;
        }
        if (LDSW) __syncthreads();
        if (__ballot(any) == 0ull) continue;
        const W* wb = LDSW ? wl : w + (int64_t)j * WSTEP;
#pragma unroll
        for (int c = 0; c < NC; c++) {
            const int ci = PAIR ? LCH * (g & 1) : OP::CHUNK * c + LCH * g;
            typename OP::A a[RT];
#pragma unroll
            for (int t = 0; t < RT; t++) {
                typename OP::Row r = OP::no_row();
                if (idx[t] >= 0) {
                    const T* row = PAIR ? x0 + (int64_t)idx[t] * CIN + ci : ci < c0 ? x0 + (int64_t)idx[t] * c0 + ci : x1 + (int64_t)idx[t] * c1 + (ci - c0);
                    r = OP::load_row(row);
                }
                a[t] = OP::fragment(r);
            }
#pragma unroll
            for (int ct = 0; ct < CT; ct++) {
                const typename OP::B b = OP::load_b(wb + (c * OP::PLANES * 4 + g) * COUT + ct * 16 + i16, PLANE);
#pragma unroll
                for (int t = 0; t < RT; t++) OP::mma(a[t], b, acc[t][ct]);
            }
        }
    }
#pragma unroll
    for (int ct = 0; ct < CT; ct++) {
        const int ch = ct * 16 + i16;
        const float sc = scale ? scale[ch] : 1.0f, sh = scale ? shift[ch] : 0.0f;
#pragma unroll
        for (int t = 0; t < RT; t++)
#pragma unroll
            for (int r = 0; r < 4; r++) {
                const int64_t pos = obase + t * 16 + g * 4 + r;
                if (pos >= n_out) continue;
                const int64_t o = row_order ? (int64_t)st_rule_row(row_order[pos]) : pos;
                float v = acc[t][ct][r];
                if (scale) v = fmaf(v, sc, sh);
                if (residual) v += (float)residual[o * COUT + ch];
                if (relu) v = v > 0.0f ? v : 0.0f;
                y[o * COUT + ch] = (T)v;
            }
    }
}

template <int CIN, int COUT, int RT, bool LDSW>
__global__ void __launch_bounds__(MF_BLOCK) k_sparse_conv_mfma(MF_PARAMS(float, float4)) { conv_rule_gemm<MfF32, CIN, COUT, RT, LDSW>(MF_ARGS); }
template <int CIN, int COUT, int RT>
__global__ void __launch_bounds__(MF_BLOCK) k_sparse_conv_mfma_b3(MF_PARAMS(float, uint4)) { conv_rule_gemm<MfB3, CIN, COUT, RT, false>(MF_ARGS); }
template <int COUT, int RT>
__global__ void __launch_bounds__(MF_BLOCK) k_sparse_conv_mfma_b3_c16(MF_PARAMS(float, uint4)) { conv_rule_gemm<MfB3, 16, COUT, RT, false>(MF_ARGS); }
template <int CIN, int COUT, int RT>
__global__ void __launch_bounds__(MF_BLOCK) k_sparse_conv_mfma_f16x(MF_PARAMS(st_h, st_v8h)) { conv_rule_gemm<MfF16, CIN, COUT, RT, false>(MF_ARGS); }
template <int COUT, int RT>
__global__ void __launch_bounds__(MF_BLOCK) k_sparse_conv_mfma_f16x_c16(MF_PARAMS(st_h, st_v8h)) { conv_rule_gemm<MfF16, 16, COUT, RT, false>(MF_ARGS); }

template <class T, class W>
using mf_kernel_t = void (*)(MF_PARAMS(T, W));
template <int CIN, int COUT, int RT>
static mf_kernel_t<float, uint4> b3_kernel() {
    if constexpr (CIN == 16) return k_sparse_conv_mfma_b3_c16<COUT, RT>;
    else return k_sparse_conv_mfma_b3<CIN, COUT, RT>;
}
template <int CIN, int COUT, int RT>
static mf_kernel_t<st_h, st_v8h> f16x_kernel() {
    if constexpr (CIN == 16) return k_sparse_conv_mfma_f16x_c16<COUT, RT>;
    else return k_sparse_conv_mfma_f16x<CIN, COUT, RT>;
}

template <class T, class W>
static int mf_launch(mf_kernel_t<T, W> kernel, int rt, const ConvArgs& a) {
    hipLaunchKernelGGL(kernel, dim3((unsigned)st_div_up(a.n_out, (MF_BLOCK / 64) * 16 * rt)), dim3(MF_BLOCK), 0, a.stream, (const T*)a.x0, a.c0,
                       (const T*)a.x1, a.nbr, a.K, a.n_out, a.nstride, (const W*)a.w, a.scale, a.shift, (const T*)a.residual, a.relu, (T*)a.y,
                       a.row_order);
    ST_CHECK_LAUNCH();
    return ST_OK;
}

static int conv_row_tiles(const ConvArgs& a) { return a.n_out >= (a.row_order == nullptr ? 56000 : 300000) ? 2 : 1; }

template <int CIN, int COUT>
static int conv_launch_mfma(const ConvArgs& a, int v) {
    if (v == 0) v = (a.row_order == nullptr && a.n_out >= 150000) ? 18 : 1;
    switch (v) {
        case 1: return mf_launch(k_sparse_conv_mfma<CIN, COUT, 1, false>, 1, a);
        case 2: return mf_launch(k_sparse_conv_mfma<CIN, COUT, 2, false>, 2, a);
        case 4: return mf_launch(k_sparse_conv_mfma<CIN, COUT, 4, false>, 4, a);
        case 17: return mf_launch(k_sparse_conv_mfma<CIN, COUT, 1, true>, 1, a);
        default: return mf_launch(k_sparse_conv_mfma<CIN, COUT, 2, true>, 2, a);
    }
}

extern "C" int st_sparse_conv_b3_fwd(const float* x0, int c0, const float* x1, int cin, const int32_t* nbr, int K, int64_t n_out,
                                     const void* wq, int cout, const float* scale, const float* shift, const float* residual,
                                     int relu, float* y, const int32_t* row_order, void* stream_, int64_t nbr_stride, int variant) {
    ConvArgs a = {x0, c0, x1, nbr, K, n_out, nbr_stride, wq, scale, shift, residual, relu, y, row_order, (hipStream_t)stream_};
    ST_TRY(conv_check_args(&a, cin));
    ST_REQUIRE((cin % 32 == 0 || (cin == 16 && c0 == cin)) && cout % 16 == 0 && c0 % 8 == 0,
               "conv(b3): Cin % 32 (or Cin = 16 without concat), Cout % 16 and a concat split % 8 are required");
    if (n_out <= 0) return ST_OK;
    const int rt = variant == 1 || variant == 2 ? variant : conv_row_tiles(a);
#define B3_CASE(CI, CO) \
    if (cin == CI && cout == CO) return rt == 2 ? mf_launch(b3_kernel<CI, CO, 2>(), 2, a) : mf_launch(b3_kernel<CI, CO, 1>(), 1, a);
    B3_CASE(16, 16)
    B3_CASE(16, 32)
    B3_CASE(32, 16)
    B3_CASE(32, 32)
    B3_CASE(32, 64)
    B3_CASE(64, 32)
    B3_CASE(64, 64)
#undef B3_CASE
    st_set_error("conv(b3): no kernel instance for cin=%d cout=%d", cin, cout);
    return ST_ERR_INVALID;
}

extern "C" int st_sparse_conv_f16_fwd(const void* x0, int c0, const void* x1, int cin, const int32_t* nbr, int K, int64_t n_out,
                                      const void* w, int cout, const float* scale, const float* shift, const void* residual,
                                      int relu, void* y, int in_half, int out_half, const int32_t* row_order, void* stream_,
                                      int64_t nbr_stride) {
    ConvArgs a = {x0, c0, x1, nbr, K, n_out, nbr_stride, w, scale, shift, residual, relu, y, row_order, (hipStream_t)stream_};
    ST_TRY(conv_check_args(&a, cin));
    ST_REQUIRE(in_half || out_half, "conv(f16): neither side is half precision -- use st_sparse_conv_fwd");
    if (n_out <= 0) return ST_OK;
    if (in_half && out_half) {
        ST_REQUIRE(cin % 16 == 0 && cout % 16 == 0 && c0 % 16 == 0, "conv(f16): channels and concat split must be multiples of 16");
        const int rt = conv_row_tiles(a);
#define F16X_CASE(CI, CO) \
    if (cin == CI && cout == CO) return rt == 2 ? mf_launch(f16x_kernel<CI, CO, 2>(), 2, a) : mf_launch(f16x_kernel<CI, CO, 1>(), 1, a);
        F16X_CASE(16, 16)
        F16X_CASE(16, 32)
        F16X_CASE(32, 16)
        F16X_CASE(32, 32)
        F16X_CASE(32, 64)
        F16X_CASE(64, 32)
        F16X_CASE(64, 64)
#undef F16X_CASE
        st_set_error("conv(f16): no kernel instance for cin=%d cout=%d", cin, cout);
        return ST_ERR_INVALID;
    }
    ST_REQUIRE(residual == nullptr && c0 == cin, "conv(f16): the converting kernels take no residual and no concat");
    ST_REQUIRE(cin % 4 == 0 && cout % 4 == 0, "conv(f16): channels must be multiples of 4");
#define CAST_CASE(CI, CO, COT_) \
    if (cin == CI && cout == CO) return in_half ? conv_launch<CI, COT_, st_h, float>(a, cout) : conv_launch<CI, COT_, float, st_h>(a, cout);
    CAST_CASE(8, 16, 16)
    CAST_CASE(16, 8, 8)
    CAST_CASE(16, 32, 16)
    CAST_CASE(32, 16, 16)
#undef CAST_CASE
    st_set_error("conv(f16): no converting kernel instance for cin=%d cout=%d", cin, cout);
    return ST_ERR_INVALID;
}

extern "C" int st_sparse_conv_mfma_fwd(const float* x0, int c0, const float* x1, int cin, const int32_t* nbr, int K,
                                       int64_t n_out, const float* wp, int cout, const float* scale, const float* shift,
                                       const float* residual, int relu, float* y, const int32_t* row_order, void* stream_,
                                       int64_t nbr_stride, int variant) {
    ConvArgs a = {x0, c0, x1, nbr, K, n_out, nbr_stride, wp, scale, shift, residual, relu, y, row_order, (hipStream_t)stream_};
    ST_TRY(conv_check_args(&a, cin));
    ST_REQUIRE(cin % 16 == 0 && cout % 16 == 0 && c0 % 16 == 0, "conv(mfma): channels and concat split must be multiples of 16");
    if (n_out <= 0) return ST_OK;
#define MFMA_CASE(CI, CO) \
    if (cin == CI && cout == CO) return conv_launch_mfma<CI, CO>(a, variant);
    MFMA_CASE(16, 16)
    MFMA_CASE(16, 32)
    MFMA_CASE(32, 16)
    MFMA_CASE(32, 32)
    MFMA_CASE(32, 64)
    MFMA_CASE(64, 32)
    MFMA_CASE(64, 64)
#undef MFMA_CASE
    st_set_error("conv(mfma): no kernel instance for cin=%d cout=%d", cin, cout);
    return ST_ERR_INVALID;
}

extern "C" int st_sparse_conv_fwd(const float* x0, int c0, const float* x1, int cin, const int32_t* nbr, int K,
                                  int64_t n_out, const float* w, int cout, const float* scale, const float* shift,
                                  const float* residual, int relu, float* y, const int32_t* row_order, void* stream_,
                                  int64_t nbr_stride) {
    ConvArgs a = {x0, c0, x1, nbr, K, n_out, nbr_stride, w, scale, shift, residual, relu, y, row_order, (hipStream_t)stream_};
    ST_TRY(conv_check_args(&a, cin));
    ST_REQUIRE(cout >= 1, "conv: cout must be positive");
    if (n_out <= 0) return ST_OK;
#define CONV_CASE(CI, CO, COT_) \
    if (cin == CI && cout == CO && (c0 == cin || (CI % 4 == 0 && c0 % 4 == 0))) return conv_launch<CI, COT_>(a, cout);
    CONV_CASE(3, 8, 8)
    CONV_CASE(8, 8, 8)
    CONV_CASE(8, 16, 16)
    CONV_CASE(16, 8, 8)
    CONV_CASE(16, 16, 16)
    CONV_CASE(16, 32, 16)
    CONV_CASE(32, 16, 16)
    CONV_CASE(32, 32, 16)
    CONV_CASE(32, 64, 16)
    CONV_CASE(64, 32, 16)
    CONV_CASE(64, 64, 16)
#undef CONV_CASE
    hipLaunchKernelGGL(k_sparse_conv_any, dim3((unsigned)st_div_up(n_out, CONV_BLOCK), (unsigned)st_div_up(cout, 4)), dim3(CONV_BLOCK), 0, a.stream, x0, c0,
                       x1, cin, nbr, K, n_out, a.nstride, w, cout, scale, shift, residual, relu, y, row_order);
    ST_CHECK_LAUNCH();
    return ST_OK;
}

#define HEAD_W1 0
#define HEAD_S1 64
#define HEAD_T1 72
#define HEAD_W2 80
#define HEAD_S2 112
#define HEAD_T2 116
#define HEAD_W3 120
#define HEAD_STRIDE 132

template <int NOUT>
__device__ __forceinline__ void head_eval(const float* __restrict__ p, const float* x, float* out) {
    float h1[8], h2[4];
#pragma unroll
    for (int co = 0; co < 8; co++) {
        float a = 0.0f;
#pragma unroll
        for (int ci = 0; ci < 8; ci++) a = fmaf(x[ci], p[HEAD_W1 + ci * 8 + co], a);
        a = fmaf(a, p[HEAD_S1 + co], p[HEAD_T1 + co]);
        h1[co] = a > 0.0f ? a : 0.0f;
    }
#pragma unroll
    for (int co = 0; co < 4; co++) {
        float a = 0.0f;
#pragma unroll
        for (int ci = 0; ci < 8; ci++) a = fmaf(h1[ci], p[HEAD_W2 + ci * 4 + co], a);
        a = fmaf(a, p[HEAD_S2 + co], p[HEAD_T2 + co]);
        h2[co] = a > 0.0f ? a : 0.0f;
    }
#pragma unroll
    for (int co = 0; co < NOUT; co++) {
        float a = 0.0f;
#pragma unroll
        for (int ci = 0; ci < 4; ci++) a = fmaf(h2[ci], p[HEAD_W3 + ci * NOUT + co], a);
        out[co] = a;
    }
}

__global__ void __launch_bounds__(CONV_BLOCK) k_heads(const float* __restrict__ x, int64_t n, const float* __restrict__ params,
                                                      float* __restrict__ radius, float* __restrict__ direction,
                                                      float* __restrict__ class_l, float* __restrict__ medial_vector,
                                                      int64_t* __restrict__ class_idx) {
    int64_t i = (int64_t)blockIdx.x * CONV_BLOCK + threadIdx.x;
    if (i >= n) return;
    const float4 a = *reinterpret_cast<const float4*>(x + i * 8);
    const float4 b = *reinterpret_cast<const float4*>(x + i * 8 + 4);
    const float xv[8] = {a.x, a.y, a.z, a.w, b.x, b.y, b.z, b.w};
    float r[1], d[3], c[2];
    head_eval<1>(params, xv, r);
    head_eval<3>(params + HEAD_STRIDE, xv, d);
    head_eval<2>(params + 2 * HEAD_STRIDE, xv, c);
    float norm = sqrtf(d[0] * d[0] + d[1] * d[1] + d[2] * d[2]);
    float den = norm > 1e-12f ? norm : 1e-12f;
    d[0] /= den; d[1] /= den; d[2] /= den;
    radius[i] = r[0];
    direction[3 * i] = d[0]; direction[3 * i + 1] = d[1]; direction[3 * i + 2] = d[2];
    class_l[2 * i] = c[0]; class_l[2 * i + 1] = c[1];
    if (medial_vector) {
        float e = expf(r[0]);
        medial_vector[3 * i] = e * d[0]; medial_vector[3 * i + 1] = e * d[1]; medial_vector[3 * i + 2] = e * d[2];
    }
    if (class_idx) class_idx[i] = c[1] > c[0] ? 1 : 0;
}

extern "C" int st_head_param_floats(void) { return 3 * HEAD_STRIDE; }

extern "C" int st_pointwise_mlp_heads(const float* x, int64_t n, const float* params, float* radius, float* direction,
                                      float* class_l, float* medial_vector, int64_t* class_idx, void* stream_) {
    hipStream_t stream = (hipStream_t)stream_;
    if (n <= 0) return ST_OK;
    hipLaunchKernelGGL(k_heads, dim3((unsigned)st_div_up(n, CONV_BLOCK)), dim3(CONV_BLOCK), 0, stream, x, n, params, radius,
                       direction, class_l, medial_vector, class_idx);
    ST_CHECK_LAUNCH();
    return ST_OK;
}
```

### smart_tree_amd/csrc/st_rule.h

```cpp
#pragma once

#include "st_common.h"


__host__ __device__ inline int st_rule_omax(int ext, int level = 0) { return (ext >> level) >> 1; }

__device__ __forceinline__ bool st_rule_axis(int c, int k, int omax, int* o) {
    const int n = c + 1 - k;
    *o = n >> 1;
    return !(n & 1) && n >= 0 && *o <= omax;
}
__device__ __forceinline__ bool st_rule_out(const int c[3], int kz, int ky, int kx, const int omax[3], int o[3]) {
    const bool z = st_rule_axis(c[0], kz, omax[0], &o[0]);
    const bool y = st_rule_axis(c[1], ky, omax[1], &o[1]);
    const bool x = st_rule_axis(c[2], kx, omax[2], &o[2]);
    return z && y && x;
}
__device__ __forceinline__ bool st_rule_out(const int c[3], int k, const int omax[3], int o[3]) {
    return st_rule_out(c, k / 9, (k / 3) % 3, k % 3, omax, o);
}

#define ST_RULE_ROW_LIMIT (1ll << 28)
#define ST_RULE_ROW_MASK 0x0fffffff

__device__ __forceinline__ int st_rule_parity_class(int z, int y, int x) { return ((z & 1) << 2) | ((y & 1) << 1) | (x & 1); }
__device__ __forceinline__ int32_t st_rule_tag(int64_t row, int cls) { return (int32_t)((uint32_t)row | ((8u + (uint32_t)cls) << 28)); }
__device__ __forceinline__ int32_t st_rule_row(int32_t entry) { return entry & ST_RULE_ROW_MASK; }
__device__ __forceinline__ uint32_t st_rule_live_offsets(int32_t entry, int K) {
    const uint32_t tag = (uint32_t)entry >> 28;
    if (!(tag & 8u) || K != 27) return 0xffffffffu;
    const uint32_t ax[3] = {(tag & 4u) ? 5u : 2u, (tag & 2u) ? 5u : 2u, (tag & 1u) ? 5u : 2u};
    uint32_t live = 0;
#pragma unroll
    for (int k = 0; k < 27; k++)
        if (((ax[0] >> (k / 9)) & (ax[1] >> ((k / 3) % 3)) & (ax[2] >> (k % 3))) & 1u) live |= 1u << k;
    return live;
}

void st_rule_parity_order(const int32_t* coords, int64_t cap, const int64_t* n_dev, const unsigned* fail, uint32_t* pc, int32_t* order,
                          hipStream_t stream);

__device__ __forceinline__ void st_ext_clear(int* m, int nseg) {
    for (int i = threadIdx.x; i < nseg * 3; i += blockDim.x) m[i] = 0;
    __syncthreads();
}
__device__ __forceinline__ void st_ext_offer(int* m, int seg, int z, int y, int x) {
    if (z > m[3 * seg]) atomicMax(&m[3 * seg], z);
    if (y > m[3 * seg + 1]) atomicMax(&m[3 * seg + 1], y);
    if (x > m[3 * seg + 2]) atomicMax(&m[3 * seg + 2], x);
}
__device__ __forceinline__ void st_ext_flush(const int* m, int nseg, int* ext) {
    __syncthreads();
    for (int i = threadIdx.x; i < nseg * 3; i += blockDim.x) if (m[i]) atomicMax(&ext[i], m[i]);
}
```

### smart_tree_amd/model/model.py

```python
from __future__ import annotations

import contextlib

from typing import Dict, Mapping

import numpy as np
import torch

from . import sparse_ops as ops
from .. import profiling

BN_EPS = 1e-4


def _conv_weight(t: torch.Tensor) -> torch.Tensor:
    cout, cin = t.shape[0], t.shape[-1]
    return t.reshape(cout, -1, cin).permute(1, 2, 0).contiguous().float()


class _Affine:

    def __init__(self, sd: Mapping[str, torch.Tensor], prefix: str, device):
        g = sd[prefix + ".weight"].double()
        b = sd[prefix + ".bias"].double()
# ... 19 lines not shown
        self.bn: Dict[str, _Affine] = {}
        self.use_mfma = True
        self.fp16 = bool(fp16)
        self.wp16: Dict[str, torch.Tensor] = {}
        self.wq: Dict[str, torch.Tensor] = {}
        self.use_b3 = True
        for key, t in sd.items():
            if key.endswith(".weight") and t.ndim == 5 and "_head." not in key:
                name = key[: -len(".weight")]
                self.w[name] = _conv_weight(t).to(self.device)
                cin_, cout_ = self.w[name].shape[1], self.w[name].shape[2]
                if self.fp16 and not (ops.mfma_eligible(cin_, cout_, 16) or (cin_, cout_) in ((3, 8), (8, 8), (8, 16), (16, 8))):
                    raise ValueError(f"fp16 storage mode has kernels for the shipped widths only (layer {name}: {cin_} -> {cout_})")
                if ops.mfma_eligible(cin_, cout_, 16):
                    self.wp[name] = ops.mfma_weight(self.w[name])
                    if self.w[name].shape[1] % 32 == 0 or (self.w[name].shape[0] == 27 and ops.b3_eligible(*self.w[name].shape[1:], self.w[name].shape[1])):
                        self.wq[name] = ops.b3_weight(self.w[name])
                    if self.fp16:
                        self.wp16[name] = ops.mfma_weight16_half(self.w[name])
            elif key.endswith(".running_mean") and "_head." not in key:
                p = key[: -len(".running_mean")]
                self.bn[p] = _Affine(sd, p, self.device)
        self.generic_heads = not self._heads_are_standard(sd)
        self.head_params = None if self.generic_heads else self._pack_heads(sd).to(self.device)
        if self.generic_heads:
            self.head_layers = {}
            for name in ("radius_head", "direction_head", "class_head"):
                mat = lambda i: sd[f"{name}.sequence.{i}.weight"].reshape(sd[f"{name}.sequence.{i}.weight"].shape[0], -1).T.contiguous().float()
                self.head_layers[name] = [(mat(0).unsqueeze(0).to(self.device), _Affine(sd, f"{name}.sequence.1", self.device)),
                                          (mat(3).unsqueeze(0).to(self.device), _Affine(sd, f"{name}.sequence.4", self.device)),
                                          (mat(6).unsqueeze(0).to(self.device), None)]
        self.use_bricks = True
        self.spatial_order = True
        self.trace = None

    def eval(self):
        return self

    def to(self, device):
        return self if torch.device(device) == self.device else Smart_Tree(self._state, device, self.fp16)

    @staticmethod
    def _heads_are_standard(sd) -> bool:
        for name, nout in (("radius_head", 1), ("direction_head", 3), ("class_head", 2)):
            shapes = [tuple(sd[f"{name}.sequence.{i}.weight"].reshape(sd[f"{name}.sequence.{i}.weight"].shape[0], -1).shape) for i in (0, 3, 6)]
            if shapes != [(8, 8), (4, 8), (nout, 4)]:
                return False
        return True

    def _generic_heads(self, x: torch.Tensor, with_tail: bool):
        n = x.shape[0]
        outs = []
        for name in ("radius_head", "direction_head", "class_head"):
            h = x
            for w, aff in self.head_layers[name]:
                h = ops.sparse_conv(h, w, None, n, scale=aff.scale if aff else None, shift=aff.shift if aff else None, relu=aff is not None)
            outs.append(h)
        radius, direction, class_l = outs[0], torch.nn.functional.normalize(outs[1]), outs[2]
        if not with_tail:
            return radius, direction, class_l, None, None
        return radius, direction, class_l, torch.exp(radius) * direction, torch.argmax(class_l, dim=1, keepdim=True)

    @staticmethod
    def _pack_heads(sd) -> torch.Tensor:
        blocks = []
        for name, nout in (("radius_head", 1), ("direction_head", 3), ("class_head", 2)):
            def mat(i):
                t = sd[f"{name}.sequence.{i}.weight"]
                return t.reshape(t.shape[0], t.shape[-1]).T.contiguous().double()

            def affine(i):
                g, b = sd[f"{name}.sequence.{i}.weight"].double(), sd[f"{name}.sequence.{i}.bias"].double()
                m, v = sd[f"{name}.sequence.{i}.running_mean"].double(), sd[f"{name}.sequence.{i}.running_var"].double()
                s = g / torch.sqrt(v + BN_EPS)
                return s, b - m * s

            s1, t1 = affine(1)
            s2, t2 = affine(4)
            w3 = torch.zeros(12, dtype=torch.float64)
            w3[: 4 * nout] = mat(6).reshape(-1)
            blocks.append(torch.cat([mat(0).reshape(-1), s1, t1, mat(3).reshape(-1), s2, t2, w3]))
        return torch.cat(blocks).float().contiguous()

    def _conv(self, name, x, nbr, n_out, x1=None, bn=None, residual=None, relu=False, row_order=None):
        a = self.bn[bn] if bn else None
        out_half = self.fp16 and self.w[name].shape[2] % 16 == 0
        return ops.sparse_conv(x, self.w[name], nbr, n_out, x1=x1, scale=a.scale if a else None,
                               shift=a.shift if a else None, residual=residual, relu=relu,
                               wp=self.wp.get(name) if self.use_mfma else None, out_half=out_half,
                               wp16=self.wp16.get(name), row_order=row_order,
                               wq=self.wq.get(name) if self.use_mfma and self.use_b3 and not self.fp16 else None)

    def _res_block(self, prefix, x, nbr, x1=None):
        n = x.shape[0]
        h = self._conv(prefix + ".sequence.0", x, nbr, n, x1=x1, bn=prefix + ".sequence.1", relu=True)
        ident = self._conv(prefix + ".identity.0", x, None, n, x1=x1) if x1 is not None else x
        return self._conv(prefix + ".sequence.3", h, nbr, n, bn=prefix + ".sequence.4", residual=ident, relu=True)

    def _ublock(self, prefix, x, pyr, level):
        x = self._res_block(prefix + ".Head", x, pyr.subm[level])
        self._record(f"head{level}", x)
        if level == self.depth:
            return x
        n_fine, n_coarse = x.shape[0], pyr.coords[level + 1].shape[0]
        z = self._conv(prefix + ".Encode.sequence.0", x, pyr.down[level], n_coarse, bn=prefix + ".Encode.sequence.1",
                       relu=True)
        self._record(f"enc{level}", z)
        z = self._ublock(prefix + ".U", z, pyr, level + 1)
        d = self._conv(prefix + ".Decode.sequence.0", z, pyr.up[level], n_fine, bn=prefix + ".Decode.sequence.1",
                       relu=True, row_order=pyr.up_order[level] if pyr.up_order else None)
        self._record(f"dec{level}", d)
        x = self._res_block(prefix + ".Tail", x, pyr.subm[level], x1=d)
        self._record(f"tail{level}", x)
        return x

    def _record(self, name, x):
        if self.trace is not None:
            self.trace[name] = x

    def features(self, sparse_input):
        coords = sparse_input.indices.contiguous()
        feats = sparse_input.features.contiguous().float()
        blk_seg, n_seg = getattr(sparse_input, "blk_seg", None), getattr(sparse_input, "n_seg", 1)
        reorder = self.spatial_order and self.trace is None and coords.shape[0] > 1
        hint = getattr(sparse_input, "brick_hint", None)
        bricks = ops.brick_pyramid(coords, self.depth, hint[0], hint[1], blk_seg, n_seg) if reorder and hint and self.use_bricks else None
        if bricks is not None:
            pyr, order = bricks
            feats = ops.move_rows(feats, order)
        else:
            order = ops.spatial_order(coords) if reorder else None
            if order is not None:
                coords, feats = ops.move_rows(coords, order), ops.move_rows(feats, order)
            pyr = ops.build_pyramid(coords, self.depth, blk_seg, n_seg)
        gate = getattr(self, "conv_gate", None)
        with (gate() if gate is not None else contextlib.nullcontext()), profiling.kernel_family("k_sparse_conv* (one forward pass)"):
            x = self._conv("input_conv.sequence.0", feats, None, feats.shape[0], bn="input_conv.sequence.1", relu=True)
            self._record("input", x)
            x = self._ublock("UNet", x, pyr, 0)
        if order is not None:
            x = ops.move_rows(x, order, scatter=True)
        return x

    def forward(self, sparse_input) -> Dict[str, torch.Tensor]:
        x = self.features(sparse_input)
        radius, direction, class_l, _, _ = self._generic_heads(x, False) if self.generic_heads else ops.mlp_heads(x, self.head_params)
        return {"radius": radius, "direction": direction, "class_l": class_l}

    __call__ = forward

    def forward_fused_tail(self, sparse_input):
        x = self.features(sparse_input)
        return self._generic_heads(x, True) if self.generic_heads else ops.mlp_heads(x, self.head_params, with_tail=True)
```

### smart_tree_amd/model/model_inference.py

```python
from __future__ import annotations

from pathlib import Path

import numpy as np
import torch

from .. import profiling
from ..data_types.cloud import Cloud, MaskedCloud
from ..dataset.dataset import SingleTreeInference, voxelize_cloud
from .model import Smart_Tree
from .sparse import sparse_from_batch

_WEIGHTS_DIR = Path(__file__).resolve().parent / "weights"


def _load_state_dict(weights_path):
    p = Path(str(weights_path))
    if not p.exists():
        bundled = _WEIGHTS_DIR / (p.name.replace("_model_weights.pt", "").replace("_model.pt", "").replace(".npz", "") + ".npz")
        if not bundled.exists():
            raise FileNotFoundError(f"weights not found: {weights_path}")
        p = bundled
    if p.suffix == ".npz":
        with np.load(p) as z:
            return {k: torch.from_numpy(z[k]) for k in z.files}
    return torch.load(str(p), map_location="cpu", weights_only=True)


def load_model(model_path, weights_path, device=torch.device("cuda:0"), fp16: bool = False):
    return Smart_Tree(_load_state_dict(weights_path), device=device, fp16=fp16).eval()


class ModelInference:
    def __init__(self, model_path, weights_path, voxel_size: float, block_size: float, buffer_size: float,
                 num_workers=8, batch_size=4, device=torch.device("cuda:0"), verbose=False, fp16: bool = False,
                 blocking: str = "blocks"):
        if blocking not in ("blocks", "whole"):
            raise ValueError(f"ModelInference: blocking must be 'blocks' or 'whole', got {blocking!r}")
        self.blocking = blocking
        self.device = torch.device(device)
        self.verbose = verbose
        self.voxel_size = voxel_size
        self.block_size = block_size
        self.buffer_size = buffer_size
        self.num_workers = num_workers
        self.batch_size = batch_size
        self.model = load_model(model_path, weights_path, self.device, fp16=fp16)
        self.on_network_done = None
        self.last_point_index = None
        if self.verbose:
            print("Model Loaded Succesfully")

    def forward(self, cloud: Cloud, return_masked: bool = True) -> Cloud:
        cloud = cloud.to_device(self.device)
        if cloud.rgb is None:
            cloud = Cloud(cloud.xyz, torch.zeros_like(cloud.xyz), seg_off=cloud.seg_off, centred_box=cloud.centred_box)
        with profiling.stage("voxelize"):
            if self.blocking == "whole":
                vb = voxelize_cloud(cloud.xyz, cloud.rgb, self.voxel_size, seg_off=cloud.seg_off)
                if vb.n_seg > 1:
                    vb.blk_seg = torch.arange(vb.n_seg, dtype=torch.int32, device=self.device)
            else:
                vb = SingleTreeInference(cloud, self.voxel_size, self.block_size, self.buffer_size).batch
        hint = None
        if self.blocking == "blocks" and vb.block_centres.shape[0] > 0:
            hint = (int(vb.block_centres.shape[0]), int(round((self.block_size + 2 * self.buffer_size) / self.voxel_size)) + 2)
        sparse_input = sparse_from_batch(vb.feats[:, :3].contiguous(), vb.coords, device=self.device, blk_seg=vb.blk_seg,
                                         n_seg=vb.n_seg, brick_hint=hint)
        with profiling.stage("unet"):
            _, _, _, mv, cls = self.model.forward_fused_tail(sparse_input)
        masks = vb.mask
        self.last_point_index = vb.point_index
        lc = Cloud(xyz=sparse_input.features, rgb=vb.feats[:, 3:6].contiguous(), medial_vector=mv, class_l=cls,
                   seg_off=vb.seg_vox_off)
        if self.on_network_done is not None:
            self.on_network_done()
        return MaskedCloud(lc, masks) if return_masked else lc

    @staticmethod
    def from_cfg(cfg):
        return ModelInference(model_path=cfg.model_path, weights_path=cfg.weights_path, voxel_size=cfg.voxel_size,
                              block_size=cfg.block_size, buffer_size=cfg.buffer_size, num_workers=cfg.num_workers,
                              batch_size=cfg.batch_size, blocking=getattr(cfg, "blocking", "blocks"))
```

### smart_tree_amd/model/sparse_ops.py

```python
from __future__ import annotations

import ctypes
from dataclasses import dataclass, field
from typing import List, Optional

import torch

from .. import _lib, profiling


@dataclass
class CoordHash:
    keys: torch.Tensor
    vals: torch.Tensor
    cap: int


def build_coord_hash(coords: torch.Tensor) -> CoordHash:
    L = _lib.lib()
    n = coords.shape[0]
    cap = L.st_hash_capacity(n)
    keys = torch.empty(cap, dtype=torch.int64, device=coords.device)
    vals = torch.empty(cap, dtype=torch.int32, device=coords.device)
    _lib.check(L.st_build_coord_hash(_lib.ptr(coords), n, _lib.ptr(keys), _lib.ptr(vals), cap, _lib.stream(coords.device)))
    return CoordHash(keys, vals, cap)


def build_subm_rulebook(coords: torch.Tensor, h: CoordHash) -> torch.Tensor:
    L = _lib.lib()
    n = coords.shape[0]
    nbr = torch.empty((27, n), dtype=torch.int32, device=coords.device)
    _lib.check(L.st_build_subm_rulebook(_lib.ptr(coords), n, _lib.ptr(h.keys), _lib.ptr(h.vals), h.cap, _lib.ptr(nbr),
                                        _lib.stream(coords.device)))
    return nbr


@dataclass
class StridedRulebook:
    out_coords: torch.Tensor
    out_hash: CoordHash
    nbr_down: torch.Tensor
    nbr_up: torch.Tensor
    up_order: torch.Tensor = None


def build_strided_rulebook(coords: torch.Tensor, h: CoordHash, blk_seg: Optional[torch.Tensor] = None,
                           n_seg: int = 1) -> StridedRulebook:
    L = _lib.lib()
    dev = coords.device
    n = coords.shape[0]
    if blk_seg is None or blk_seg.numel() == 0:
        n_seg = 1
    ext_dev = torch.empty(3 * n_seg, dtype=torch.int32, device=dev) if n_seg > 1 else None
    ws = _lib.workspace(L.st_strided_workspace_bytes(n), dev)
    n_out = ctypes.c_int64(0)
    extent = (ctypes.c_int32 * 3)()
    rc = -1
    for max_out in (n + 1024, 8 * n + 1024):
        out_coords = torch.empty((max_out, 4), dtype=torch.int32, device=dev)
        ccap = L.st_hash_capacity(max_out)
        ckeys = torch.empty(ccap, dtype=torch.int64, device=dev)
        cvals = torch.empty(ccap, dtype=torch.int32, device=dev)
        rc = L.st_build_strided_outputs_seg(_lib.ptr(coords), n, max_out, _lib.ptr(out_coords), _lib.ptr(ckeys),
                                            _lib.ptr(cvals), ccap, ctypes.byref(n_out), extent, _lib.ptr(blk_seg) if n_seg > 1 else None,
                                            n_seg, _lib.ptr(ext_dev), _lib.ptr(ws), ws.numel(), _lib.stream(dev))
        if rc == 0 or b"max_out" not in L.st_last_error():
            break
    _lib.check(rc)
    m = n_out.value
    out_coords = out_coords[:m].contiguous()
    nbr_down = torch.empty((27, m), dtype=torch.int32, device=dev)
    nbr_up = torch.empty((27, n), dtype=torch.int32, device=dev)
    up_order = torch.empty(n + 16, dtype=torch.int32, device=dev)
    _lib.check(L.st_build_strided_rulebook_seg(_lib.ptr(coords), n, _lib.ptr(h.keys), _lib.ptr(h.vals), h.cap,
                                               _lib.ptr(out_coords), m, _lib.ptr(ckeys), _lib.ptr(cvals), ccap, extent,
                                               _lib.ptr(nbr_down), _lib.ptr(nbr_up), _lib.ptr(up_order),
                                               _lib.ptr(blk_seg) if n_seg > 1 else None, _lib.ptr(ext_dev), _lib.stream(dev)))
    return StridedRulebook(out_coords, CoordHash(ckeys, cvals, ccap), nbr_down, nbr_up, up_order[:n])


@dataclass
class RulebookPyramid:
    coords: List[torch.Tensor] = field(default_factory=list)
    subm: List[torch.Tensor] = field(default_factory=list)
    down: List[torch.Tensor] = field(default_factory=list)
    up: List[torch.Tensor] = field(default_factory=list)
    up_order: List[torch.Tensor] = field(default_factory=list)


def build_pyramid(coords: torch.Tensor, depth: int, blk_seg: Optional[torch.Tensor] = None, n_seg: int = 1) -> RulebookPyramid:
    pyr = RulebookPyramid()
    h = build_coord_hash(coords)
    for level in range(depth + 1):
        pyr.coords.append(coords)
        pyr.subm.append(build_subm_rulebook(coords, h))
        if level == depth:
            break
        s = build_strided_rulebook(coords, h, blk_seg, n_seg)
        pyr.down.append(s.nbr_down)
        pyr.up.append(s.nbr_up)
        pyr.up_order.append(s.up_order)
        coords, h = s.out_coords, s.out_hash
    return pyr


def brick_pyramid(coords: torch.Tensor, depth: int, n_blocks: int, coord_bound: int, blk_seg: Optional[torch.Tensor] = None,
                  n_seg: int = 1):
    L = _lib.lib()
    dev = coords.device
    n0 = coords.shape[0]
    if n0 == 0 or n_blocks < 1 or coord_bound < 1:
        return None
    if blk_seg is None or blk_seg.numel() == 0:
        n_seg = 1
    i32 = dict(dtype=torch.int32, device=dev)
    for attempt in range(2):
        caps = [n0]
        for l in range(depth):
            side = -(-int(coord_bound) // (2 << l)) + 1
            geom = int(n_blocks) * side ** 3
            caps.append((3 * caps[-1]) // 4 + 4096 if attempt == 0 else min(8 * caps[-1] + 4096, geom))
        if attempt == 1 and sum(caps) * 27 * 4 * 3 > (16 << 30):
            return None
        c_caps = (ctypes.c_int64 * (depth + 1))(*caps)
        nbytes = L.st_brick_pyramid_workspace_bytes(n0, int(n_blocks), int(coord_bound), depth, c_caps)
        if nbytes <= 0 or nbytes > (24 << 30):
            return None
        try:
            ws = _lib.workspace(nbytes, dev)
            order0 = torch.empty(n0, **i32)
            coords_out = [torch.empty((caps[l], 4), **i32) for l in range(depth + 1)]
            subm = [torch.empty((27, caps[l]), **i32) for l in range(depth + 1)]
            down = [torch.empty((27, caps[l + 1]), **i32) for l in range(depth)]
            up = [torch.empty((27, caps[l]), **i32) for l in range(depth)]
            up_order = [torch.empty(caps[l] + 16, **i32) for l in range(depth)]
        except torch.OutOfMemoryError:
            return None
        arr = lambda ts: (ctypes.c_void_p * max(len(ts), 1))(*[t.data_ptr() for t in ts])
        counts = (ctypes.c_int64 * (depth + 1))()
        rc = L.st_brick_pyramid(_lib.ptr(coords), n0, int(n_blocks), int(coord_bound), depth, _lib.ptr(blk_seg) if n_seg > 1 else None,
                                n_seg, c_caps, _lib.ptr(order0), arr(coords_out), arr(subm), arr(down), arr(up), arr(up_order), counts,
                                _lib.ptr(ws), ws.numel(), _lib.stream(dev))
        if rc == 0:
            break
        if b"outside the declared bounds" in L.st_last_error():
            return None
        if b"capacity" not in L.st_last_error():
            _lib.check(rc)
        if attempt == 1:
            return None
        del ws, order0, coords_out, subm, down, up, up_order
    n = [int(counts[l]) for l in range(depth + 1)]
    pyr = RulebookPyramid()
    for l in range(depth + 1):
        pyr.coords.append(coords_out[l][: n[l]])
        pyr.subm.append(subm[l][:, : n[l]])
        if l < depth:
            pyr.down.append(down[l][:, : n[l + 1]])
            pyr.up.append(up[l][:, : n[l]])
            pyr.up_order.append(up_order[l][: n[l]])
    return pyr, order0


def _nbr_args(nbr: Optional[torch.Tensor]):
    if nbr is None:
        return None, 0
    if nbr.ndim != 2 or (nbr.shape[1] > 1 and nbr.stride(1) != 1):
        raise _lib.StError("neighbour table must be [K, n] with unit column stride")
    if not nbr.is_cuda and not _lib._ALLOW_HOST_POINTERS:
        raise _lib.StError("smart_tree_amd kernels need tensors on the GPU (got a CPU tensor); there is no CPU fallback")
    return nbr.data_ptr(), int(nbr.stride(0)) if nbr.shape[0] > 1 else int(max(nbr.shape[1], 1))


B3_VARIANT = 0
MFMA_VARIANT = 0


def spatial_order(coords: torch.Tensor) -> torch.Tensor:
    L = _lib.lib()
    n = coords.shape[0]
    order = torch.empty(n, dtype=torch.int32, device=coords.device)
    if n:
        ws = _lib.workspace(L.st_spatial_order_workspace_bytes(n), coords.device)
        _lib.check(L.st_spatial_order(_lib.ptr(coords), n, _lib.ptr(order), _lib.ptr(ws), ws.numel(), _lib.stream(coords.device)))
    return order


def move_rows(x: torch.Tensor, order: torch.Tensor, scatter: bool = False) -> torch.Tensor:
    L = _lib.lib()
    x = x.contiguous()
    assert x.element_size() in (4, 2) and x.ndim == 2 and order.dtype == torch.int32
    out = torch.empty_like(x)
    move = L.st_move_rows if x.element_size() == 4 else L.st_move_rows_h
    if x.element_size() == 4 or x.shape[1]:
        _lib.check(move(_lib.ptr(x), x.shape[1], _lib.ptr(order), x.shape[0], _lib.ptr(out), int(scatter), _lib.stream(x.device)))
    return out


def sparse_conv_half(x0: torch.Tensor, w: torch.Tensor, nbr: Optional[torch.Tensor], n_out: int,
                     x1: Optional[torch.Tensor] = None) -> torch.Tensor:
    L = _lib.lib()
    K, cin, cout = w.shape
    if x0.dtype != torch.float16 or w.dtype != torch.float16 or (x1 is not None and x1.dtype != torch.float16):
        raise ValueError("sparse_conv_half takes float16 features and weights")
    c0 = x0.shape[1]
    if c0 + (x1.shape[1] if x1 is not None else 0) != cin:
        raise ValueError(f"input channels {c0} + {x1.shape[1] if x1 is not None else 0} do not match the weights' {cin}")
    nbr_ptr, nbr_stride = _nbr_args(nbr)
    y = torch.empty((n_out, cout), dtype=torch.float16, device=x0.device)
    if n_out == 0:
        return y
    nbytes = (lambda: (_pair_count(nbr) if nbr is not None else n_out) * (cin * 2 + (4 if nbr is not None else 0))
              + n_out * cout * 2) if profiling.enabled() else 0
    nflops = (lambda: 2.0 * (_pair_count(nbr) if nbr is not None else n_out) * cin * cout) if profiling.enabled() else 0
    form = "k_hconv_mfma" if cin >= 16 and cout >= 16 else "k_hconv_vec"
    with profiling.kernel(f"{form}<{cin},{cout}>" + ("" if nbr is not None else " k1"), nbytes, nflops):
        _lib.check(L.st_sparse_conv_h_fwd(_lib.ptr(x0), c0, _lib.ptr(x1), cin, nbr_ptr, K, n_out, nbr_stride, _lib.ptr(w), cout,
                                          _lib.ptr(y), _lib.stream(x0.device)))
    return y


def mfma_weight(w: torch.Tensor) -> torch.Tensor:
    K, cin, cout = w.shape
    return w.reshape(K, cin // 16, 4, 4, cout).permute(0, 1, 2, 4, 3).contiguous()


def mfma_weight32(w: torch.Tensor) -> torch.Tensor:
    K, cin, cout = w.shape
    return w.reshape(K, cin // 32, 4, 8, cout).permute(0, 1, 2, 4, 3).contiguous()


def mfma_weight16_half(w: torch.Tensor) -> torch.Tensor:
    K, cin, cout = w.shape
    if cin % 32 == 0:
        return mfma_weight32(w).half()
    if cin == 16 and cout in (16, 32):
        if K % 2:
            w = torch.cat([w, torch.zeros((1, cin, cout), dtype=w.dtype, device=w.device)], 0)
        return mfma_weight32(w.reshape((K + 1) // 2, 32, cout)).half()
    raise ValueError(f"no half-precision matrix-core kernel for cin={cin} cout={cout}")


_MFMA_SHAPES = ((16, 16), (16, 32), (32, 16), (32, 32), (32, 64), (64, 32), (64, 64))


def mfma_eligible(cin: int, cout: int, c0: int) -> bool:
    return (cin, cout) in _MFMA_SHAPES and c0 % 16 == 0


def b3_eligible(cin: int, cout: int, c0: int) -> bool:
    if cin == 16:
        return c0 == 16 and cout in (16, 32)
    return cin % 32 == 0 and cout % 16 == 0 and c0 % 8 == 0 and (cin, cout) in ((32, 16), (32, 32), (32, 64), (64, 32), (64, 64))


def b3_weight(w: torch.Tensor) -> torch.Tensor:
    K, cin, cout = w.shape
    w = w.detach().to(torch.float32).contiguous()
    if cin == 16:
        if K % 2:
            w = torch.cat([w, torch.zeros((1, cin, cout), dtype=w.dtype, device=w.device)], 0)
        w = w.reshape((K + 1) // 2, 32, cout)
        K, cin = w.shape[0], 32
    mask = torch.tensor(-65536, dtype=torch.int32, device=w.device)
    planes, r = [], w
    for _ in range(3):
        top = (r.view(torch.int32) & mask).view(torch.float32)
        planes.append((r.view(torch.int32) >> 16).to(torch.int16))
        r = r - top
    q = torch.stack(planes, 0)
    q = q.reshape(3, K, cin // 32, 4, 8, cout).permute(1, 2, 0, 3, 5, 4).contiguous()
    return q


def sparse_conv(x0: torch.Tensor, w: torch.Tensor, nbr: Optional[torch.Tensor], n_out: int,
                x1: Optional[torch.Tensor] = None, scale: Optional[torch.Tensor] = None,
                shift: Optional[torch.Tensor] = None, residual: Optional[torch.Tensor] = None,
                relu: bool = False, wp: Optional[torch.Tensor] = None, out_half: bool = False,
                wp16: Optional[torch.Tensor] = None, row_order: Optional[torch.Tensor] = None,
                wq: Optional[torch.Tensor] = None) -> torch.Tensor:
    L = _lib.lib()
    K, cin, cout = w.shape
    c0 = x0.shape[1]
    nbr_ptr, nbr_stride = _nbr_args(nbr)
    if n_out == 0:
        return torch.empty((0, cout), dtype=torch.float16 if out_half else torch.float32, device=x0.device)
    in_half = x0.dtype == torch.float16
    big_16 = cin == 16 and cout == 16 and nbr is not None and row_order is None and x1 is None
    mid, tail = (), ()
    if in_half or out_half:
        both = in_half and out_half
        if both and wp16 is None:
            raise ValueError("half -> half convolution needs the half-precision MFMA weights (wp16)")
        entry, wt, mid = L.st_sparse_conv_f16_fwd, (wp16 if both else w), (int(in_half), int(out_half))
        name = f"k_sparse_conv_mfma_f16x<{cin},{cout}>" if both else f"k_sparse_conv<{cin},{cout}> {'h->f' if in_half else 'f->h'}"
    elif wq is not None and b3_eligible(cin, cout, c0):
        entry, wt, name, tail = L.st_sparse_conv_b3_fwd, wq, f"k_sparse_conv_mfma_b3<{cin},{cout}>", (int(B3_VARIANT),)
    elif wp is not None and mfma_eligible(cin, cout, c0) and not big_16:
        entry, wt, name, tail = L.st_sparse_conv_mfma_fwd, wp, f"k_sparse_conv_mfma<{cin},{cout}>", (int(MFMA_VARIANT),)
    else:
        entry, wt, name = L.st_sparse_conv_fwd, w, f"k_sparse_conv<{cin},{cout}>"
    esz_in, esz_out = (2 if in_half else 4), (2 if out_half else 4)
    y = torch.empty((n_out, cout), dtype=torch.float16 if out_half else torch.float32, device=x0.device)
    nbytes = (lambda: (_pair_count(nbr) if nbr is not None else n_out) * (cin * esz_in + (4 if nbr is not None else 0))
              + n_out * cout * esz_out) if profiling.enabled() else 0
    nflops = (lambda: 2.0 * (_pair_count(nbr) if nbr is not None else n_out) * cin * cout) if profiling.enabled() else 0
    with profiling.kernel(name + ("" if nbr is not None else " k1"), nbytes, nflops):
        _lib.check(entry(_lib.ptr(x0), c0, _lib.ptr(x1), cin, nbr_ptr, K, n_out, _lib.ptr(wt), cout, _lib.ptr(scale), _lib.ptr(shift),
                         _lib.ptr(residual), int(relu), _lib.ptr(y), *mid, _lib.ptr(row_order), _lib.stream(x0.device), nbr_stride, *tail))
    return y


_pairs_cache = {}


def _pair_count(nbr: torch.Tensor) -> int:
    key = (id(nbr), profiling.generation())
    if key not in _pairs_cache:
        if len(_pairs_cache) > 4096:
            _pairs_cache.clear()
        _pairs_cache[key] = int((nbr >= 0).sum().item())
    return _pairs_cache[key]


def mlp_heads(x: torch.Tensor, params: torch.Tensor, with_tail: bool = False):
    L = _lib.lib()
    n, dev = x.shape[0], x.device
    radius = torch.empty((n, 1), dtype=torch.float32, device=dev)
    direction = torch.empty((n, 3), dtype=torch.float32, device=dev)
    class_l = torch.empty((n, 2), dtype=torch.float32, device=dev)
    mv = torch.empty((n, 3), dtype=torch.float32, device=dev) if with_tail else None
    cls = torch.empty((n, 1), dtype=torch.int64, device=dev) if with_tail else None
    if n == 0:
        return radius, direction, class_l, mv, cls
    _lib.check(L.st_pointwise_mlp_heads(_lib.ptr(x), n, _lib.ptr(params), _lib.ptr(radius), _lib.ptr(direction),
                                        _lib.ptr(class_l), _lib.ptr(mv), _lib.ptr(cls), _lib.stream(dev)))
    return radius, direction, class_l, mv, cls
```

Before: 933.2 million.

## Compute UNet features only for voxels that feed inner (non-buffer) block outputs

Adds a per-block bounding box of inner voxels and classifies each voxel at every pyramid level by whether it can influence an inner output. This produces need lists and filtered up-sampling lists. Convolution, row-move and MLP-head kernels get list variants that process only the listed rows, and the heads can skip non-kept points. The aim is to avoid computing the sparse UNet over buffer-region voxels whose outputs are discarded. The cost is extra classification and compaction kernels, and rows outside the lists stay uninitialised or zero.

```diff
diff --git a/include/smarttree_hip.h b/include/smarttree_hip.h
--- a/include/smarttree_hip.h
+++ b/include/smarttree_hip.h
@@ -8,6 +8,7 @@
 #endif
 
 int st_version(void);
+#define ST_BRICK_NEED_COUNTS 4
 #define ST_SKELETON_STATS_ENTRIES 16
 #define ST_SKELETON_TUNING_ENTRIES 24
 int st_abi_entries(int what);
@@ -32,6 +33,8 @@
 int64_t st_spatial_order_workspace_bytes(int64_t n);
 int st_spatial_order(const int32_t* coords, int64_t n, int32_t* order , void* ws, int64_t ws_bytes, void* stream);
 int st_move_rows(const void* src, int row_words, const int32_t* order, int64_t n, void* dst, int scatter, void* stream);
+int st_move_rows_list(const void* src, int row_words, const int32_t* order, const int32_t* list, int64_t n, void* dst, int scatter,
+                      void* stream);
 int64_t st_strided_workspace_bytes(int64_t n_fine);
 int st_build_strided_outputs(const int32_t* coords, int64_t n, int64_t max_out, int32_t* out_coords,
                              unsigned long long* ckeys, unsigned* cvals, int64_t ccap, int64_t* n_out_host,
@@ -58,6 +61,17 @@
 int st_sparse_conv_f16_fwd(const void* x0, int c0, const void* x1, int cin, const int32_t* nbr, int K, int64_t n_out,
                            const void* w, int cout, const float* scale, const float* shift, const void* residual, int relu,
                            void* y, int in_half, int out_half, const int32_t* row_order, void* stream, int64_t nbr_stride );
+int st_sparse_conv_mfma_list_fwd(const float* x0, int c0, const float* x1, int cin, const int32_t* nbr, int K, int64_t n_out,
+                                 const float* wp, int cout, const float* scale, const float* shift, const float* residual, int relu,
+                                 float* y, const int32_t* row_order, void* stream, int64_t nbr_stride, int variant, int64_t level_rows,
+                                 int parity);
+int st_sparse_conv_b3_list_fwd(const float* x0, int c0, const float* x1, int cin, const int32_t* nbr, int K, int64_t n_out, const void* wq,
+                               int cout, const float* scale, const float* shift, const float* residual, int relu, float* y,
+                               const int32_t* row_order, void* stream, int64_t nbr_stride, int variant, int64_t level_rows, int parity);
+int st_sparse_conv_f16_list_fwd(const void* x0, int c0, const void* x1, int cin, const int32_t* nbr, int K, int64_t n_out,
+                                const void* w, int cout, const float* scale, const float* shift, const void* residual, int relu,
+                                void* y, int in_half, int out_half, const int32_t* row_order, void* stream, int64_t nbr_stride,
+                                int64_t level_rows, int parity);
 
 int64_t st_brick_pyramid_workspace_bytes(int64_t n0, int n_blocks, int coord_bound, int depth, const int64_t* caps);
 int st_brick_pyramid(const int32_t* coords0 , int64_t n0, int n_blocks ,
@@ -67,9 +81,16 @@
                      int32_t* const* subm , int32_t* const* down ,
                      int32_t* const* up , int32_t* const* up_order ,
                      int64_t* counts_host , void* ws, int64_t ws_bytes, void* stream);
+int st_brick_pyramid_need(const int32_t* coords0, int64_t n0, int n_blocks, int coord_bound, int depth, const int32_t* blk_seg, int nseg,
+                          const int64_t* caps, int32_t* order0, int32_t* const* coords_out, int32_t* const* subm, int32_t* const* down,
+                          int32_t* const* up, int32_t* const* up_order, int64_t* counts_host, const unsigned char* inner ,
+                          int32_t* const* need_order , int32_t* const* up_need ,
+                          int64_t* need_counts_host , void* ws, int64_t ws_bytes, void* stream);
 int st_head_param_floats(void);
 int st_pointwise_mlp_heads(const float* x, int64_t n, const float* params, float* radius, float* direction,
                            float* class_l, float* medial_vector , int64_t* class_idx , void* stream);
+int st_pointwise_mlp_heads_keep(const float* x, int64_t n, const unsigned char* keep, const float* params, float* radius, float* direction,
+                                float* class_l, float* medial_vector , int64_t* class_idx , void* stream);
 
 int st_centre_cloud(const float* xyz, int64_t n, float* out, void* ws, int64_t ws_bytes, void* stream);
 int st_medial_points(const float* xyz, const float* mv, int64_t n, float* medial, float* radius, void* stream);
diff --git a/smart_tree_amd/_lib.py b/smart_tree_amd/_lib.py
--- a/smart_tree_amd/_lib.py
+++ b/smart_tree_amd/_lib.py
@@ -43,6 +43,14 @@
     "st_brick_pyramid_workspace_bytes": (I64, [I64, c_int, c_int, c_int, ctypes.POINTER(I64)]),
     "st_brick_pyramid": (c_int, [P, I64, c_int, c_int, c_int, P, c_int, ctypes.POINTER(I64), P, ctypes.POINTER(P), ctypes.POINTER(P),
                                  ctypes.POINTER(P), ctypes.POINTER(P), ctypes.POINTER(P), ctypes.POINTER(I64), P, I64, P]),
+    "st_brick_pyramid_need": (c_int, [P, I64, c_int, c_int, c_int, P, c_int, ctypes.POINTER(I64), P, ctypes.POINTER(P), ctypes.POINTER(P),
+                                      ctypes.POINTER(P), ctypes.POINTER(P), ctypes.POINTER(P), ctypes.POINTER(I64), P, ctypes.POINTER(P),
+                                      ctypes.POINTER(P), ctypes.POINTER(I64), P, I64, P]),
+    "st_sparse_conv_mfma_list_fwd": (c_int, [P, c_int, P, c_int, P, c_int, I64, P, c_int, P, P, P, c_int, P, P, P, I64, c_int, I64, c_int]),
+    "st_sparse_conv_b3_list_fwd": (c_int, [P, c_int, P, c_int, P, c_int, I64, P, c_int, P, P, P, c_int, P, P, P, I64, c_int, I64, c_int]),
+    "st_sparse_conv_f16_list_fwd": (c_int, [P, c_int, P, c_int, P, c_int, I64, P, c_int, P, P, P, c_int, P, c_int, c_int, P, P, I64, I64, c_int]),
+    "st_pointwise_mlp_heads_keep": (c_int, [P, I64, P, P, P, P, P, P, P, P]),
+    "st_move_rows_list": (c_int, [P, c_int, P, P, I64, P, c_int, P]),
     "st_head_param_floats": (c_int, []),
     "st_pointwise_mlp_heads": (c_int, [P, I64, P, P, P, P, P, P, P]),
     "st_knn_workspace_bytes": (I64, [I64]),
@@ -146,6 +154,7 @@
     "st_prediction_metrics_tally_ints", "st_prediction_metrics_tally_sums", "st_prediction_metrics_workspace_bytes", "st_prediction_metrics",
     "st_render_workspace_bytes", "st_render_clear", "st_render_points", "st_render_segments", "st_render_resolve",
     "st_bridge_components_workspace_bytes", "st_segment_workspace_bytes", "st_segment_points_seg",
+    "st_sparse_conv_mfma_list_fwd", "st_sparse_conv_b3_list_fwd", "st_sparse_conv_f16_list_fwd", "st_pointwise_mlp_heads_keep", "st_move_rows_list",
 })
 
 
diff --git a/smart_tree_amd/csrc/brick.hip b/smart_tree_amd/csrc/brick.hip
--- a/smart_tree_amd/csrc/brick.hip
+++ b/smart_tree_amd/csrc/brick.hip
@@ -1,6 +1,7 @@
 #include "st_common.h"
 #include "st_grid.h"
 #include "st_rule.h"
+#include "smarttree_hip.h"
 
 #define BK_BLOCK 256
 #define BK_MAX_DEPTH 6
@@ -369,15 +370,147 @@
     if (threadIdx.x < 8 && hist[threadIdx.x]) atomicAdd(&parity_count[threadIdx.x], hist[threadIdx.x]);
 }
 
+#define BK_BOX_SPAN 32
+__device__ __forceinline__ void bk_box_flush(int* lo, int* hi, int b, int mn[3], int mx[3], int lane) {
+    for (int d = 32; d >= 1; d >>= 1)
+#pragma unroll
+        for (int a = 0; a < 3; a++) {
+            const int o = __shfl_xor(mn[a], d), p = __shfl_xor(mx[a], d);
+            mn[a] = o < mn[a] ? o : mn[a];
+            mx[a] = p > mx[a] ? p : mx[a];
+        }
+    if (lane == 0 && b >= 0)
+#pragma unroll
+        for (int a = 0; a < 3; a++) {
+            if (mn[a] <= mx[a]) { atomicMin(&lo[3 * b + a], mn[a]); atomicMax(&hi[3 * b + a], mx[a]); }
+        }
+#pragma unroll
+    for (int a = 0; a < 3; a++) { mn[a] = 0x7fffffff; mx[a] = -1; }
+}
+__global__ void __launch_bounds__(BK_BLOCK) k_bk_inner_box(const int32_t* coords0, const unsigned char* inner, int64_t n, int nblk, int lim, int* box,
+                                                           const BkState* st) {
+    if (st->fail) return;
+    const int lane = threadIdx.x & 63;
+    int *lo = box, *hi = box + 3 * nblk;
+    const int64_t first = (((int64_t)blockIdx.x * blockDim.x + threadIdx.x) >> 6) * (64 * BK_BOX_SPAN);
+    int cur = -1, mn[3] = {0x7fffffff, 0x7fffffff, 0x7fffffff}, mx[3] = {-1, -1, -1};
+    for (int g = 0; g < BK_BOX_SPAN && first + 64 * g < n; g++) {
+        const int64_t i = first + 64 * g + lane;
+        int4 c = make_int4(-1, 0, 0, 0);
+        bool in = false;
+        if (i < n && inner[i] != 0) {
+            c = reinterpret_cast<const int4*>(coords0)[i];
+            in = (unsigned)c.x < (unsigned)nblk && (unsigned)c.y < (unsigned)lim && (unsigned)c.z < (unsigned)lim && (unsigned)c.w < (unsigned)lim;
+        }
+        const unsigned long long who = __ballot(in);
+        if (who == 0ull) continue;
+        if (__ballot(in && c.x != cur) != 0ull) {
+            if (cur >= 0) bk_box_flush(lo, hi, cur, mn, mx, lane);
+            cur = __shfl(c.x, __ffsll((long long)who) - 1);
+            if (__ballot(in && c.x != cur) != 0ull) {
+                cur = -1;
+                if (in) {
+                    atomicMin(&lo[3 * c.x], c.y); atomicMax(&hi[3 * c.x], c.y);
+                    atomicMin(&lo[3 * c.x + 1], c.z); atomicMax(&hi[3 * c.x + 1], c.z);
+                    atomicMin(&lo[3 * c.x + 2], c.w); atomicMax(&hi[3 * c.x + 2], c.w);
+                }
+                continue;
+            }
+        }
+        if (in) {
+            mn[0] = c.y < mn[0] ? c.y : mn[0]; mx[0] = c.y > mx[0] ? c.y : mx[0];
+            mn[1] = c.z < mn[1] ? c.z : mn[1]; mx[1] = c.z > mx[1] ? c.z : mx[1];
+            mn[2] = c.w < mn[2] ? c.w : mn[2]; mx[2] = c.w > mx[2] ? c.w : mx[2];
+        }
+    }
+    if (cur >= 0) bk_box_flush(lo, hi, cur, mn, mx, lane);
+}
+
+#define BK_NEED_LISTS (ST_RULE_NEED_CLASSES + 1)
+static_assert(BK_NEED_LISTS == ST_BRICK_NEED_COUNTS, "header and library disagree about the need counts per level");
+__global__ void __launch_bounds__(BK_BLOCK) k_bk_need_class(const int32_t* coords, const int64_t* n_dev, int64_t cap, const int* box, int nblk,
+                                                            int level, unsigned char* cls, const BkState* st) {
+    if (st->fail) return;
+    const int64_t n = *n_dev < cap ? *n_dev : cap;
+    BK_LOOP(row, n) {
+        const int4 c = reinterpret_cast<const int4*>(coords)[row];
+        const int cc[3] = {c.y, c.z, c.w};
+        cls[row] = (unsigned char)((unsigned)c.x < (unsigned)nblk ? st_rule_need_class(cc, box + 3 * c.x, box + 3 * nblk + 3 * c.x, level)
+                                                                  : ST_RULE_NEED_CLASSES);
+    }
+}
+__device__ __forceinline__ void bk_need_classify(const unsigned char* cls8, int64_t n, int64_t pos, const int32_t* up_order, int* cls, bool* keep,
+                                                 int32_t* entry) {
+    *cls = ST_RULE_NEED_CLASSES;
+    *keep = false;
+    *entry = 0;
+    if (pos >= n) return;
+    *cls = cls8[pos];
+    *entry = up_order[pos];
+    const int64_t row = st_rule_row(*entry);
+    *keep = row < n && cls8[row] < ST_RULE_NEED_CLASSES;
+}
+__global__ void __launch_bounds__(BK_BLOCK) k_bk_need_count(const unsigned char* cls8, const int64_t* n_dev, int64_t cap, const int32_t* up_order,
+                                                            uint32_t* cnt, int64_t ntiles, const BkState* st) {
+    if (st->fail) return;
+    const int64_t n = *n_dev < cap ? *n_dev : cap, pos = (int64_t)blockIdx.x * BK_BLOCK + threadIdx.x;
+    int cls;
+    bool keep;
+    int32_t entry;
+    bk_need_classify(cls8, n, pos, up_order, &cls, &keep, &entry);
+#pragma unroll
+    for (int q = 0; q < BK_NEED_LISTS; q++) {
+        const unsigned long long b = __ballot(q < ST_RULE_NEED_CLASSES ? cls == q : keep);
+        if ((threadIdx.x & 63) == 0 && b != 0ull) atomicAdd(&cnt[q * ntiles + blockIdx.x], (uint32_t)__popcll(b));
+    }
+}
+__global__ void __launch_bounds__(BK_BLOCK) k_bk_need_emit(const unsigned char* cls8, const int64_t* n_dev, int64_t cap, const int32_t* up_order,
+                                                           const uint32_t* base, int64_t ntiles,
+                                                           int32_t* need_order, int32_t* up_need, int64_t* counts, const BkState* st) {
+    __shared__ uint32_t wcnt[BK_BLOCK / 64][BK_NEED_LISTS];
+    if (st->fail) return;
+    const int64_t n = *n_dev < cap ? *n_dev : cap, pos = (int64_t)blockIdx.x * BK_BLOCK + threadIdx.x;
+    const int lane = threadIdx.x & 63, wave = threadIdx.x >> 6;
+    int cls;
+    bool keep;
+    int32_t entry;
+    bk_need_classify(cls8, n, pos, up_order, &cls, &keep, &entry);
+    uint32_t rank[BK_NEED_LISTS];
+#pragma unroll
+    for (int q = 0; q < BK_NEED_LISTS; q++) {
+        const unsigned long long b = __ballot(q < ST_RULE_NEED_CLASSES ? cls == q : keep);
+        rank[q] = (uint32_t)__popcll(b & ((1ull << lane) - 1ull));
+        if (lane == 0) wcnt[wave][q] = (uint32_t)__popcll(b);
+    }
+    __syncthreads();
+    const uint32_t up0 = base[ST_RULE_NEED_CLASSES * ntiles];
+#pragma unroll
+    for (int q = 0; q < BK_NEED_LISTS; q++) {
+        if (q < ST_RULE_NEED_CLASSES ? cls != q : !keep) continue;
+        int64_t at = (int64_t)base[q * ntiles + blockIdx.x] + rank[q];
+        for (int w = 0; w < wave; w++) at += wcnt[w][q];
+        if (q < ST_RULE_NEED_CLASSES) { if (at < n) need_order[at] = (int32_t)pos; }
+        else if (at - up0 < n) up_need[at - up0] = entry;
+    }
+    if (blockIdx.x == 0 && threadIdx.x == 0) {
+        for (int q = 0; q < ST_RULE_NEED_CLASSES; q++) counts[q] = base[(q + 1) * ntiles];
+        counts[ST_RULE_NEED_CLASSES] = (int64_t)base[BK_NEED_LISTS * ntiles] - up0;
+    }
+}
+
 struct BkPlan {
     int depth;
     int mb[BK_MAX_DEPTH + 1];
     int64_t ntab[BK_MAX_DEPTH + 1], slot_cap[BK_MAX_DEPTH + 1];
+    int n_blocks;
+    int64_t cap_max;
 };
 
 static bool bk_plan(int64_t n0, int n_blocks, int coord_bound, int depth, const int64_t* caps, BkPlan* P) {
     if (depth < 0 || depth > BK_MAX_DEPTH || n_blocks < 1 || coord_bound < 1) return false;
     P->depth = depth;
+    P->n_blocks = n_blocks;
+    P->cap_max = 1;
     int bound = coord_bound;
     for (int l = 0; l <= depth; l++) {
         int nb = (bound + 7) / 8, mb = 0;
@@ -389,14 +522,22 @@
         const int64_t cap = l == 0 ? n0 : caps[l];
         if ((l == 0 && caps && caps[0] > cap ? caps[0] : cap) >= ST_RULE_ROW_LIMIT) return false;
         P->slot_cap[l] = cap < P->ntab[l] ? cap : P->ntab[l];
+        const int64_t rows = l == 0 && caps && caps[0] > cap ? caps[0] : cap;
+        if (rows > P->cap_max) P->cap_max = rows;
         bound = (bound - 1) / 2 + 1;
     }
     return true;
 }
+
+#define BK_COUNTS (2 * (BK_MAX_DEPTH + 1) + BK_NEED_LISTS * BK_MAX_DEPTH)
+static inline int64_t bk_need_tiles(int64_t cap) { return st_div_up(cap > 0 ? cap : 1, BK_BLOCK); }
 
 struct BkLayout {
     BkState* st;
     int64_t* counts;
+    int* box;
+    unsigned char* need_cls;
+    uint32_t* need_cnt;
     uint32_t* p[BK_MAX_DEPTH + 1];
     BkRec* rec[BK_MAX_DEPTH + 1];
     uint32_t* base[BK_MAX_DEPTH + 1];
@@ -406,8 +547,12 @@
 
 static void bk_layout(StArena& a, const BkPlan& P, BkLayout* Y) {
     Y->st = a.take<BkState>(1);
-    Y->counts = a.take<int64_t>(2 * (BK_MAX_DEPTH + 1));
-    int64_t scan_n = 1;
+    Y->counts = a.take<int64_t>(BK_COUNTS);
+    Y->box = a.take<int>(6 * (int64_t)P.n_blocks);
+    const int64_t need_n = BK_NEED_LISTS * bk_need_tiles(P.cap_max) + 1;
+    Y->need_cls = a.take<unsigned char>(P.cap_max);
+    Y->need_cnt = a.take<uint32_t>(need_n);
+    int64_t scan_n = need_n;
     for (int l = 0; l <= P.depth; l++) {
         Y->p[l] = a.take<uint32_t>(P.ntab[l] + 1);
         Y->rec[l] = a.take<BkRec>(P.slot_cap[l]);
@@ -428,12 +573,15 @@
     return a.used;
 }
 
-extern "C" int st_brick_pyramid(const int32_t* coords0, int64_t n0, int n_blocks, int coord_bound, int depth, const int32_t* blk_seg,
-                                int nseg, const int64_t* caps, int32_t* order0, int32_t* const* coords_out, int32_t* const* subm,
-                                int32_t* const* down, int32_t* const* up, int32_t* const* up_order, int64_t* counts_host, void* ws,
-                                int64_t ws_bytes, void* stream_) {
+extern "C" int st_brick_pyramid_need(const int32_t* coords0, int64_t n0, int n_blocks, int coord_bound, int depth, const int32_t* blk_seg,
+                                     int nseg, const int64_t* caps, int32_t* order0, int32_t* const* coords_out, int32_t* const* subm,
+                                     int32_t* const* down, int32_t* const* up, int32_t* const* up_order, int64_t* counts_host,
+                                     const unsigned char* inner, int32_t* const* need_order, int32_t* const* up_need,
+                                     int64_t* need_counts_host, void* ws, int64_t ws_bytes, void* stream_) {
     hipStream_t stream = (hipStream_t)stream_;
     for (int l = 0; l <= depth && l <= BK_MAX_DEPTH; l++) counts_host[l] = 0;
+    ST_REQUIRE(!inner || (need_order && up_need && need_counts_host), "brick pyramid: an inner mask needs the arrays of the need lists");
+    for (int i = 0; inner && i < BK_NEED_LISTS * depth && i < BK_NEED_LISTS * BK_MAX_DEPTH; i++) need_counts_host[i] = 0;
     if (n0 <= 0) return ST_OK;
     ST_REQUIRE(nseg >= 1 && nseg <= ST_MAX_SEG && (nseg == 1 || blk_seg), "brick pyramid: 1 <= clouds per batch <= %d", ST_MAX_SEG);
     ST_REQUIRE(caps && caps[0] >= n0, "brick pyramid: caps[0] must hold the input voxels");
@@ -448,7 +596,7 @@
         return ST_ERR_WORKSPACE;
     }
     (void)hipMemsetAsync(Y.st, 0, sizeof(BkState), stream);
-    (void)hipMemsetAsync(Y.counts, 0, 2 * (BK_MAX_DEPTH + 1) * sizeof(int64_t), stream);
+    (void)hipMemsetAsync(Y.counts, 0, BK_COUNTS * sizeof(int64_t), stream);
     BkLevel L[BK_MAX_DEPTH + 1];
     for (int l = 0; l <= depth; l++) {
         L[l].mb = P.mb[l]; L[l].mt = 1u << (3 * P.mb[l]); L[l].ntab = P.ntab[l]; L[l].p = Y.p[l]; L[l].rec = Y.rec[l];
@@ -490,7 +638,25 @@
                            L[l + 1], (const BkState*)Y.st, l, blk_seg, (const int64_t*)L[l + 1].n_vox, cap_c, up[l], down[l], pc);
         st_rule_parity_order(coords_out[l], cap, L[l].n_vox, &Y.st->fail, pc, up_order[l], stream);
     }
-    struct { int64_t counts[2 * (BK_MAX_DEPTH + 1)]; } hc;
+    if (inner) {
+        (void)hipMemsetAsync(Y.box, 0x7f, 3 * (size_t)n_blocks * sizeof(int), stream);
+        (void)hipMemsetAsync(Y.box + 3 * (int64_t)n_blocks, 0xff, 3 * (size_t)n_blocks * sizeof(int), stream);
+        hipLaunchKernelGGL(k_bk_inner_box, dim3((unsigned)st_div_up(n0, BK_BLOCK * BK_BOX_SPAN)), dim3(BK_BLOCK), 0, stream, coords0, inner, n0,
+                           n_blocks, 8 << P.mb[0], Y.box, (const BkState*)Y.st);
+        for (int l = 0; l < depth; l++) {
+            const int64_t cap = caps[l], ntiles = bk_need_tiles(cap), cnt_n = BK_NEED_LISTS * ntiles + 1;
+            (void)hipMemsetAsync(Y.need_cnt, 0, cnt_n * sizeof(uint32_t), stream);
+            hipLaunchKernelGGL(k_bk_need_class, dim3(bk_grid(cap)), dim3(BK_BLOCK), 0, stream, (const int32_t*)coords_out[l], (const int64_t*)L[l].n_vox, cap,
+                               (const int*)Y.box, n_blocks, l, Y.need_cls, (const BkState*)Y.st);
+            hipLaunchKernelGGL(k_bk_need_count, dim3((unsigned)ntiles), dim3(BK_BLOCK), 0, stream, (const unsigned char*)Y.need_cls,
+                               (const int64_t*)L[l].n_vox, cap, (const int32_t*)up_order[l], Y.need_cnt, ntiles, (const BkState*)Y.st);
+            ST_TRY(st_exclusive_scan_u32(Y.need_cnt, Y.need_cnt, cnt_n, nullptr, Y.scan_ws, Y.scan_bytes, stream));
+            hipLaunchKernelGGL(k_bk_need_emit, dim3((unsigned)ntiles), dim3(BK_BLOCK), 0, stream, (const unsigned char*)Y.need_cls,
+                               (const int64_t*)L[l].n_vox, cap, (const int32_t*)up_order[l], (const uint32_t*)Y.need_cnt, ntiles, need_order[l],
+                               up_need[l], Y.counts + 2 * (BK_MAX_DEPTH + 1) + BK_NEED_LISTS * l, (const BkState*)Y.st);
+        }
+    }
+    struct { int64_t counts[BK_COUNTS]; } hc;
     unsigned hfail = 0;
     (void)hipMemcpyAsync(&hc, Y.counts, sizeof(hc), hipMemcpyDeviceToHost, stream);
     (void)hipMemcpyAsync(&hfail, &Y.st->fail, sizeof(unsigned), hipMemcpyDeviceToHost, stream);
@@ -506,5 +672,14 @@
     }
     ST_REQUIRE(hc.counts[1] == n0, "brick pyramid: %lld distinct voxels among %lld input rows (duplicate coordinates)", (long long)hc.counts[1],
                (long long)n0);
+    for (int i = 0; inner && i < BK_NEED_LISTS * depth; i++) need_counts_host[i] = hc.counts[2 * (BK_MAX_DEPTH + 1) + i];
     return ST_OK;
 }
+
+extern "C" int st_brick_pyramid(const int32_t* coords0, int64_t n0, int n_blocks, int coord_bound, int depth, const int32_t* blk_seg,
+                                int nseg, const int64_t* caps, int32_t* order0, int32_t* const* coords_out, int32_t* const* subm,
+                                int32_t* const* down, int32_t* const* up, int32_t* const* up_order, int64_t* counts_host, void* ws,
+                                int64_t ws_bytes, void* stream_) {
+    return st_brick_pyramid_need(coords0, n0, n_blocks, coord_bound, depth, blk_seg, nseg, caps, order0, coords_out, subm, down, up, up_order,
+                                 counts_host, nullptr, nullptr, nullptr, nullptr, ws, ws_bytes, stream_);
+}
diff --git a/smart_tree_amd/csrc/prims.hip b/smart_tree_amd/csrc/prims.hip
--- a/smart_tree_amd/csrc/prims.hip
+++ b/smart_tree_amd/csrc/prims.hip
@@ -14,7 +14,7 @@
 extern "C" const char* st_last_error(void) { return g_err; }
 void st_stream_wait(hipStream_t stream) { (void)hipStreamSynchronize(stream); }
 
-extern "C" int st_version(void) { return 111; }
+extern "C" int st_version(void) { return 112; }
 
 #define SCAN_BLOCK 256
 #define SCAN_ITEMS 16
diff --git a/smart_tree_amd/csrc/rulebook.hip b/smart_tree_amd/csrc/rulebook.hip
--- a/smart_tree_amd/csrc/rulebook.hip
+++ b/smart_tree_amd/csrc/rulebook.hip
@@ -391,11 +391,11 @@
 
 template <int VEC>
 __global__ void __launch_bounds__(RB_BLOCK) k_rb_move_rows(const uint32_t* __restrict__ src, int row_words, const int32_t* __restrict__ order,
-                                                           int64_t n, uint32_t* __restrict__ dst, int scatter) {
+                                                           int64_t n, uint32_t* __restrict__ dst, int scatter, const int32_t* __restrict__ list) {
     const int per_row = row_words / VEC;
     const int64_t total = n * per_row;
     for (int64_t t = (int64_t)blockIdx.x * blockDim.x + threadIdx.x; t < total; t += (int64_t)gridDim.x * blockDim.x) {
-        const int64_t p = t / per_row;
+        const int64_t p = list ? (int64_t)list[t / per_row] : t / per_row;
         const int c = (int)(t % per_row) * VEC;
         const int64_t o = order[p];
         const int64_t from = (scatter ? p : o) * row_words + c, to = (scatter ? o : p) * row_words + c;
@@ -404,7 +404,8 @@
     }
 }
 
-extern "C" int st_move_rows(const void* src, int row_words, const int32_t* order, int64_t n, void* dst, int scatter, void* stream_) {
+extern "C" int st_move_rows_list(const void* src, int row_words, const int32_t* order, const int32_t* list, int64_t n, void* dst, int scatter,
+                                 void* stream_) {
     hipStream_t stream = (hipStream_t)stream_;
     if (n <= 0) return ST_OK;
     ST_REQUIRE(row_words >= 1 && row_words <= 256, "move_rows: rows of 1..256 words");
@@ -412,10 +413,14 @@
     const int64_t total = n * (vec ? row_words / 4 : row_words);
     if (vec)
         hipLaunchKernelGGL((k_rb_move_rows<4>), dim3(rb_grid(total)), dim3(RB_BLOCK), 0, stream, (const uint32_t*)src, row_words, order, n,
-                           (uint32_t*)dst, scatter);
+                           (uint32_t*)dst, scatter, list);
     else
         hipLaunchKernelGGL((k_rb_move_rows<1>), dim3(rb_grid(total)), dim3(RB_BLOCK), 0, stream, (const uint32_t*)src, row_words, order, n,
-                           (uint32_t*)dst, scatter);
-    ST_CHECK_LAUNCH();
-    return ST_OK;
-}
+                           (uint32_t*)dst, scatter, list);
+    ST_CHECK_LAUNCH();
+    return ST_OK;
+}
+
+extern "C" int st_move_rows(const void* src, int row_words, const int32_t* order, int64_t n, void* dst, int scatter, void* stream_) {
+    return st_move_rows_list(src, row_words, order, nullptr, n, dst, scatter, stream_);
+}
diff --git a/smart_tree_amd/csrc/skeleton.hip b/smart_tree_amd/csrc/skeleton.hip
--- a/smart_tree_amd/csrc/skeleton.hip
+++ b/smart_tree_amd/csrc/skeleton.hip
@@ -1534,7 +1534,7 @@
 
 static_assert(ST_TUNE_ENTRIES == ST_SKELETON_TUNING_ENTRIES, "header and library disagree about the tuning array");
 extern "C" int st_abi_entries(int what) {
-    return what == 0 ? ST_SKELETON_STATS_ENTRIES : (what == 1 ? ST_SKELETON_TUNING_ENTRIES : (what == 2 ? ST_MAX_SEG : -1));
+    return what == 0 ? ST_SKELETON_STATS_ENTRIES : (what == 1 ? ST_SKELETON_TUNING_ENTRIES : (what == 2 ? ST_MAX_SEG : (what == 3 ? ST_BRICK_NEED_COUNTS : -1)));
 }
 
 extern "C" int64_t st_skeleton_workspace_bytes_seg(int64_t m, int64_t n_comp, int nseg) {
diff --git a/smart_tree_amd/csrc/sparse_conv.hip b/smart_tree_amd/csrc/sparse_conv.hip
--- a/smart_tree_amd/csrc/sparse_conv.hip
+++ b/smart_tree_amd/csrc/sparse_conv.hip
@@ -159,10 +159,14 @@
     void* y;
     const int32_t* row_order;
     hipStream_t stream;
+    int64_t level_rows = 0;
+    bool parity = false;
 };
 
 static int conv_check_args(ConvArgs* a, int cin) {
     if (a->nstride <= 0) a->nstride = a->n_out;
+    if (a->level_rows <= 0) { a->level_rows = a->n_out; a->parity = a->row_order != nullptr; }
+    ST_REQUIRE(a->level_rows >= a->n_out && (a->level_rows == a->n_out || a->row_order != nullptr), "conv: a launch over fewer rows than the level has needs their list");
     ST_REQUIRE(a->K >= 1 && (a->nbr != nullptr || a->K == 1), "conv: a NULL neighbour table means pointwise (K = 1)");
     ST_REQUIRE(a->c0 > 0 && a->c0 <= cin && (a->c0 == cin || a->x1 != nullptr), "conv: bad concat split");
     ST_REQUIRE((a->scale == nullptr) == (a->shift == nullptr), "conv: scale and shift go together");
@@ -379,11 +383,11 @@
     return ST_OK;
 }
 
-static int conv_row_tiles(const ConvArgs& a) { return a.n_out >= (a.row_order == nullptr ? 56000 : 300000) ? 2 : 1; }
+static int conv_row_tiles(const ConvArgs& a) { return a.level_rows >= (!a.parity ? 56000 : 300000) ? 2 : 1; }
 
 template <int CIN, int COUT>
 static int conv_launch_mfma(const ConvArgs& a, int v) {
-    if (v == 0) v = (a.row_order == nullptr && a.n_out >= 150000) ? 18 : 1;
+    if (v == 0) v = (!a.parity && a.level_rows >= 150000) ? 18 : 1;
     switch (v) {
         case 1: return mf_launch(k_sparse_conv_mfma<CIN, COUT, 1, false>, 1, a);
         case 2: return mf_launch(k_sparse_conv_mfma<CIN, COUT, 2, false>, 2, a);
@@ -393,10 +397,11 @@
     }
 }
 
-extern "C" int st_sparse_conv_b3_fwd(const float* x0, int c0, const float* x1, int cin, const int32_t* nbr, int K, int64_t n_out,
-                                     const void* wq, int cout, const float* scale, const float* shift, const float* residual,
-                                     int relu, float* y, const int32_t* row_order, void* stream_, int64_t nbr_stride, int variant) {
-    ConvArgs a = {x0, c0, x1, nbr, K, n_out, nbr_stride, wq, scale, shift, residual, relu, y, row_order, (hipStream_t)stream_};
+extern "C" int st_sparse_conv_b3_list_fwd(const float* x0, int c0, const float* x1, int cin, const int32_t* nbr, int K, int64_t n_out,
+                                          const void* wq, int cout, const float* scale, const float* shift, const float* residual,
+                                          int relu, float* y, const int32_t* row_order, void* stream_, int64_t nbr_stride, int variant,
+                                          int64_t level_rows, int parity) {
+    ConvArgs a = {x0, c0, x1, nbr, K, n_out, nbr_stride, wq, scale, shift, residual, relu, y, row_order, (hipStream_t)stream_, level_rows, parity != 0};
     ST_TRY(conv_check_args(&a, cin));
     ST_REQUIRE((cin % 32 == 0 || (cin == 16 && c0 == cin)) && cout % 16 == 0 && c0 % 8 == 0,
                "conv(b3): Cin % 32 (or Cin = 16 without concat), Cout % 16 and a concat split % 8 are required");
@@ -415,12 +420,18 @@
     st_set_error("conv(b3): no kernel instance for cin=%d cout=%d", cin, cout);
     return ST_ERR_INVALID;
 }
-
-extern "C" int st_sparse_conv_f16_fwd(const void* x0, int c0, const void* x1, int cin, const int32_t* nbr, int K, int64_t n_out,
-                                      const void* w, int cout, const float* scale, const float* shift, const void* residual,
-                                      int relu, void* y, int in_half, int out_half, const int32_t* row_order, void* stream_,
-                                      int64_t nbr_stride) {
-    ConvArgs a = {x0, c0, x1, nbr, K, n_out, nbr_stride, w, scale, shift, residual, relu, y, row_order, (hipStream_t)stream_};
+extern "C" int st_sparse_conv_b3_fwd(const float* x0, int c0, const float* x1, int cin, const int32_t* nbr, int K, int64_t n_out,
+                                     const void* wq, int cout, const float* scale, const float* shift, const float* residual,
+                                     int relu, float* y, const int32_t* row_order, void* stream_, int64_t nbr_stride, int variant) {
+    return st_sparse_conv_b3_list_fwd(x0, c0, x1, cin, nbr, K, n_out, wq, cout, scale, shift, residual, relu, y, row_order, stream_, nbr_stride,
+                                      variant, 0, 0);
+}
+
+extern "C" int st_sparse_conv_f16_list_fwd(const void* x0, int c0, const void* x1, int cin, const int32_t* nbr, int K, int64_t n_out,
+                                           const void* w, int cout, const float* scale, const float* shift, const void* residual,
+                                           int relu, void* y, int in_half, int out_half, const int32_t* row_order, void* stream_,
+                                           int64_t nbr_stride, int64_t level_rows, int parity) {
+    ConvArgs a = {x0, c0, x1, nbr, K, n_out, nbr_stride, w, scale, shift, residual, relu, y, row_order, (hipStream_t)stream_, level_rows, parity != 0};
     ST_TRY(conv_check_args(&a, cin));
     ST_REQUIRE(in_half || out_half, "conv(f16): neither side is half precision -- use st_sparse_conv_fwd");
     if (n_out <= 0) return ST_OK;
@@ -452,12 +463,19 @@
     st_set_error("conv(f16): no converting kernel instance for cin=%d cout=%d", cin, cout);
     return ST_ERR_INVALID;
 }
-
-extern "C" int st_sparse_conv_mfma_fwd(const float* x0, int c0, const float* x1, int cin, const int32_t* nbr, int K,
-                                       int64_t n_out, const float* wp, int cout, const float* scale, const float* shift,
-                                       const float* residual, int relu, float* y, const int32_t* row_order, void* stream_,
-                                       int64_t nbr_stride, int variant) {
-    ConvArgs a = {x0, c0, x1, nbr, K, n_out, nbr_stride, wp, scale, shift, residual, relu, y, row_order, (hipStream_t)stream_};
+extern "C" int st_sparse_conv_f16_fwd(const void* x0, int c0, const void* x1, int cin, const int32_t* nbr, int K, int64_t n_out,
+                                      const void* w, int cout, const float* scale, const float* shift, const void* residual,
+                                      int relu, void* y, int in_half, int out_half, const int32_t* row_order, void* stream_,
+                                      int64_t nbr_stride) {
+    return st_sparse_conv_f16_list_fwd(x0, c0, x1, cin, nbr, K, n_out, w, cout, scale, shift, residual, relu, y, in_half, out_half, row_order,
+                                       stream_, nbr_stride, 0, 0);
+}
+
+extern "C" int st_sparse_conv_mfma_list_fwd(const float* x0, int c0, const float* x1, int cin, const int32_t* nbr, int K,
+                                            int64_t n_out, const float* wp, int cout, const float* scale, const float* shift,
+                                            const float* residual, int relu, float* y, const int32_t* row_order, void* stream_,
+                                            int64_t nbr_stride, int variant, int64_t level_rows, int parity) {
+    ConvArgs a = {x0, c0, x1, nbr, K, n_out, nbr_stride, wp, scale, shift, residual, relu, y, row_order, (hipStream_t)stream_, level_rows, parity != 0};
     ST_TRY(conv_check_args(&a, cin));
     ST_REQUIRE(cin % 16 == 0 && cout % 16 == 0 && c0 % 16 == 0, "conv(mfma): channels and concat split must be multiples of 16");
     if (n_out <= 0) return ST_OK;
@@ -473,6 +491,13 @@
 #undef MFMA_CASE
     st_set_error("conv(mfma): no kernel instance for cin=%d cout=%d", cin, cout);
     return ST_ERR_INVALID;
+}
+extern "C" int st_sparse_conv_mfma_fwd(const float* x0, int c0, const float* x1, int cin, const int32_t* nbr, int K,
+                                       int64_t n_out, const float* wp, int cout, const float* scale, const float* shift,
+                                       const float* residual, int relu, float* y, const int32_t* row_order, void* stream_,
+                                       int64_t nbr_stride, int variant) {
+    return st_sparse_conv_mfma_list_fwd(x0, c0, x1, cin, nbr, K, n_out, wp, cout, scale, shift, residual, relu, y, row_order, stream_, nbr_stride,
+                                        variant, 0, 0);
 }
 
 extern "C" int st_sparse_conv_fwd(const float* x0, int c0, const float* x1, int cin, const int32_t* nbr, int K,
@@ -543,9 +568,17 @@
 __global__ void __launch_bounds__(CONV_BLOCK) k_heads(const float* __restrict__ x, int64_t n, const float* __restrict__ params,
                                                       float* __restrict__ radius, float* __restrict__ direction,
                                                       float* __restrict__ class_l, float* __restrict__ medial_vector,
-                                                      int64_t* __restrict__ class_idx) {
+                                                      int64_t* __restrict__ class_idx, const unsigned char* __restrict__ keep) {
     int64_t i = (int64_t)blockIdx.x * CONV_BLOCK + threadIdx.x;
     if (i >= n) return;
+    if (keep && !keep[i]) {
+        radius[i] = 0.0f;
+        direction[3 * i] = 0.0f; direction[3 * i + 1] = 0.0f; direction[3 * i + 2] = 0.0f;
+        class_l[2 * i] = 0.0f; class_l[2 * i + 1] = 0.0f;
+        if (medial_vector) { medial_vector[3 * i] = 0.0f; medial_vector[3 * i + 1] = 0.0f; medial_vector[3 * i + 2] = 0.0f; }
+        if (class_idx) class_idx[i] = 0;
+        return;
+    }
     const float4 a = *reinterpret_cast<const float4*>(x + i * 8);
     const float4 b = *reinterpret_cast<const float4*>(x + i * 8 + 4);
     const float xv[8] = {a.x, a.y, a.z, a.w, b.x, b.y, b.z, b.w};
@@ -568,12 +601,17 @@
 
 extern "C" int st_head_param_floats(void) { return 3 * HEAD_STRIDE; }
 
-extern "C" int st_pointwise_mlp_heads(const float* x, int64_t n, const float* params, float* radius, float* direction,
-                                      float* class_l, float* medial_vector, int64_t* class_idx, void* stream_) {
+extern "C" int st_pointwise_mlp_heads_keep(const float* x, int64_t n, const unsigned char* keep, const float* params, float* radius,
+                                           float* direction, float* class_l, float* medial_vector, int64_t* class_idx, void* stream_) {
     hipStream_t stream = (hipStream_t)stream_;
     if (n <= 0) return ST_OK;
     hipLaunchKernelGGL(k_heads, dim3((unsigned)st_div_up(n, CONV_BLOCK)), dim3(CONV_BLOCK), 0, stream, x, n, params, radius,
-                       direction, class_l, medial_vector, class_idx);
+                       direction, class_l, medial_vector, class_idx, keep);
     ST_CHECK_LAUNCH();
     return ST_OK;
 }
+
+extern "C" int st_pointwise_mlp_heads(const float* x, int64_t n, const float* params, float* radius, float* direction,
+                                      float* class_l, float* medial_vector, int64_t* class_idx, void* stream_) {
+    return st_pointwise_mlp_heads_keep(x, n, nullptr, params, radius, direction, class_l, medial_vector, class_idx, stream_);
+}
diff --git a/smart_tree_amd/csrc/st_rule.h b/smart_tree_amd/csrc/st_rule.h
--- a/smart_tree_amd/csrc/st_rule.h
+++ b/smart_tree_amd/csrc/st_rule.h
@@ -40,6 +40,29 @@
 void st_rule_parity_order(const int32_t* coords, int64_t cap, const int64_t* n_dev, const unsigned* fail, uint32_t* pc, int32_t* order,
                           hipStream_t stream);
 
+#define ST_RULE_NEED_CLASSES 3
+__host__ __device__ inline int st_rule_need_base(int level) {
+    int a = 0;
+    for (int l = 0; l < level; l++) a = (a + 2 + 1) >> 1;
+    return a;
+}
+__host__ __device__ inline void st_rule_need_box(int lo, int hi, int level, int* blo, int* bhi) {
+    *blo = lo >> level;
+    *bhi = (hi + (1 << level) - 1) >> level;
+}
+__host__ __device__ inline int st_rule_need_class(const int c[3], const int lo[3], const int hi[3], int level) {
+    int m = 0;
+    for (int a = 0; a < 3; a++) {
+        if (lo[a] > hi[a]) return ST_RULE_NEED_CLASSES;
+        int blo, bhi;
+        st_rule_need_box(lo[a], hi[a], level, &blo, &bhi);
+        const int d = c[a] < blo ? blo - c[a] : (c[a] > bhi ? c[a] - bhi : 0);
+        m = d > m ? d : m;
+    }
+    const int over = m - st_rule_need_base(level);
+    return over <= 0 ? 0 : (over < ST_RULE_NEED_CLASSES ? over : ST_RULE_NEED_CLASSES);
+}
+
 __device__ __forceinline__ void st_ext_clear(int* m, int nseg) {
     for (int i = threadIdx.x; i < nseg * 3; i += blockDim.x) m[i] = 0;
     __syncthreads();
diff --git a/smart_tree_amd/model/model.py b/smart_tree_amd/model/model.py
--- a/smart_tree_amd/model/model.py
+++ b/smart_tree_amd/model/model.py
@@ -125,20 +125,28 @@
             blocks.append(torch.cat([mat(0).reshape(-1), s1, t1, mat(3).reshape(-1), s2, t2, w3]))
         return torch.cat(blocks).float().contiguous()
 
-    def _conv(self, name, x, nbr, n_out, x1=None, bn=None, residual=None, relu=False, row_order=None):
+    def _conv(self, name, x, nbr, n_out, x1=None, bn=None, residual=None, relu=False, row_order=None, rows=None):
         a = self.bn[bn] if bn else None
         out_half = self.fp16 and self.w[name].shape[2] % 16 == 0
+        listed = {}
+        if rows is not None and rows[0].shape[0] <= self.LIST_MAX_SHARE * n_out:
+            listed = dict(level_rows=n_out, parity=rows[1])
+            row_order, n_out = rows[0], rows[0].shape[0]
         return ops.sparse_conv(x, self.w[name], nbr, n_out, x1=x1, scale=a.scale if a else None,
                                shift=a.shift if a else None, residual=residual, relu=relu,
                                wp=self.wp.get(name) if self.use_mfma else None, out_half=out_half,
                                wp16=self.wp16.get(name), row_order=row_order,
-                               wq=self.wq.get(name) if self.use_mfma and self.use_b3 and not self.fp16 else None)
-
-    def _res_block(self, prefix, x, nbr, x1=None):
+                               wq=self.wq.get(name) if self.use_mfma and self.use_b3 and not self.fp16 else None, **listed)
+
+    LIST_MAX_SHARE = 0.95
+
+    def _res_block(self, prefix, x, nbr, x1=None, need=None):
         n = x.shape[0]
-        h = self._conv(prefix + ".sequence.0", x, nbr, n, x1=x1, bn=prefix + ".sequence.1", relu=True)
-        ident = self._conv(prefix + ".identity.0", x, None, n, x1=x1) if x1 is not None else x
-        return self._conv(prefix + ".sequence.3", h, nbr, n, bn=prefix + ".sequence.4", residual=ident, relu=True)
+        r0 = (need.order[: need.counts[0]], False) if need is not None else None
+        r1 = (need.order[: need.counts[1]], False) if need is not None else None
+        h = self._conv(prefix + ".sequence.0", x, nbr, n, x1=x1, bn=prefix + ".sequence.1", relu=True, rows=r1)
+        ident = self._conv(prefix + ".identity.0", x, None, n, x1=x1, rows=r0) if x1 is not None else x
+        return self._conv(prefix + ".sequence.3", h, nbr, n, bn=prefix + ".sequence.4", residual=ident, relu=True, rows=r0)
 
     def _ublock(self, prefix, x, pyr, level):
         x = self._res_block(prefix + ".Head", x, pyr.subm[level])
@@ -150,10 +158,12 @@
                        relu=True)
         self._record(f"enc{level}", z)
         z = self._ublock(prefix + ".U", z, pyr, level + 1)
+        need = pyr.need[level] if pyr.need else None
         d = self._conv(prefix + ".Decode.sequence.0", z, pyr.up[level], n_fine, bn=prefix + ".Decode.sequence.1",
-                       relu=True, row_order=pyr.up_order[level] if pyr.up_order else None)
+                       relu=True, row_order=pyr.up_order[level] if pyr.up_order else None,
+                       rows=(need.up_order, True) if need is not None else None)
         self._record(f"dec{level}", d)
-        x = self._res_block(prefix + ".Tail", x, pyr.subm[level], x1=d)
+        x = self._res_block(prefix + ".Tail", x, pyr.subm[level], x1=d, need=need)
         self._record(f"tail{level}", x)
         return x
 
@@ -161,13 +171,18 @@
         if self.trace is not None:
             self.trace[name] = x
 
-    def features(self, sparse_input):
+    def features(self, sparse_input, inner_mask=None):
+        return self._features(sparse_input, inner_mask)[0]
+
+    def _features(self, sparse_input, inner_mask=None):
         coords = sparse_input.indices.contiguous()
         feats = sparse_input.features.contiguous().float()
         blk_seg, n_seg = getattr(sparse_input, "blk_seg", None), getattr(sparse_input, "n_seg", 1)
         reorder = self.spatial_order and self.trace is None and coords.shape[0] > 1
         hint = getattr(sparse_input, "brick_hint", None)
-        bricks = ops.brick_pyramid(coords, self.depth, hint[0], hint[1], blk_seg, n_seg) if reorder and hint and self.use_bricks else None
+        if self.generic_heads:
+            inner_mask = None
+        bricks = ops.brick_pyramid(coords, self.depth, hint[0], hint[1], blk_seg, n_seg, inner_mask) if reorder and hint and self.use_bricks else None
         if bricks is not None:
             pyr, order = bricks
             feats = ops.move_rows(feats, order)
@@ -181,17 +196,24 @@
             x = self._conv("input_conv.sequence.0", feats, None, feats.shape[0], bn="input_conv.sequence.1", relu=True)
             self._record("input", x)
             x = self._ublock("UNet", x, pyr, 0)
-        if order is not None:
+        keep = None
+        if bricks is not None and pyr.need and x.element_size() == 4 and pyr.need[0].counts[0] <= self.LIST_MAX_SHARE * x.shape[0]:
+            keep = inner_mask.contiguous().view(torch.uint8)
+            x = ops.move_rows(x, order, scatter=True, rows=pyr.need[0].order[: pyr.need[0].counts[0]])
+        elif order is not None:
             x = ops.move_rows(x, order, scatter=True)
-        return x
-
-    def forward(self, sparse_input) -> Dict[str, torch.Tensor]:
-        x = self.features(sparse_input)
-        radius, direction, class_l, _, _ = self._generic_heads(x, False) if self.generic_heads else ops.mlp_heads(x, self.head_params)
+        return x, keep
+
+    def _heads(self, x, keep, with_tail):
+        if self.generic_heads:
+            return self._generic_heads(x, with_tail)
+        return ops.mlp_heads(x, self.head_params, with_tail=with_tail, keep=keep)
+
+    def forward(self, sparse_input, inner_mask=None) -> Dict[str, torch.Tensor]:
+        radius, direction, class_l, _, _ = self._heads(*self._features(sparse_input, inner_mask), False)
         return {"radius": radius, "direction": direction, "class_l": class_l}
 
     __call__ = forward
 
-    def forward_fused_tail(self, sparse_input):
-        x = self.features(sparse_input)
-        return self._generic_heads(x, True) if self.generic_heads else ops.mlp_heads(x, self.head_params, with_tail=True)
+    def forward_fused_tail(self, sparse_input, inner_mask=None):
+        return self._heads(*self._features(sparse_input, inner_mask), True)
diff --git a/smart_tree_amd/model/model_inference.py b/smart_tree_amd/model/model_inference.py
--- a/smart_tree_amd/model/model_inference.py
+++ b/smart_tree_amd/model/model_inference.py
@@ -34,10 +34,11 @@
 class ModelInference:
     def __init__(self, model_path, weights_path, voxel_size: float, block_size: float, buffer_size: float,
                  num_workers=8, batch_size=4, device=torch.device("cuda:0"), verbose=False, fp16: bool = False,
-                 blocking: str = "blocks"):
+                 blocking: str = "blocks", prune_halo: bool = True):
         if blocking not in ("blocks", "whole"):
             raise ValueError(f"ModelInference: blocking must be 'blocks' or 'whole', got {blocking!r}")
         self.blocking = blocking
+        self.prune_halo = bool(prune_halo)
         self.device = torch.device(device)
         self.verbose = verbose
         self.voxel_size = voxel_size
@@ -68,7 +69,8 @@
         sparse_input = sparse_from_batch(vb.feats[:, :3].contiguous(), vb.coords, device=self.device, blk_seg=vb.blk_seg,
                                          n_seg=vb.n_seg, brick_hint=hint)
         with profiling.stage("unet"):
-            _, _, _, mv, cls = self.model.forward_fused_tail(sparse_input)
+            prune = self.prune_halo and return_masked and self.blocking == "blocks"
+            _, _, _, mv, cls = self.model.forward_fused_tail(sparse_input, vb.mask if prune else None)
         masks = vb.mask
         self.last_point_index = vb.point_index
         lc = Cloud(xyz=sparse_input.features, rgb=vb.feats[:, 3:6].contiguous(), medial_vector=mv, class_l=cls,
diff --git a/smart_tree_amd/model/sparse_ops.py b/smart_tree_amd/model/sparse_ops.py
--- a/smart_tree_amd/model/sparse_ops.py
+++ b/smart_tree_amd/model/sparse_ops.py
@@ -80,12 +80,20 @@
 
 
 @dataclass
+class NeedLists:
+    order: torch.Tensor
+    counts: tuple
+    up_order: torch.Tensor
+
+
+@dataclass
 class RulebookPyramid:
     coords: List[torch.Tensor] = field(default_factory=list)
     subm: List[torch.Tensor] = field(default_factory=list)
     down: List[torch.Tensor] = field(default_factory=list)
     up: List[torch.Tensor] = field(default_factory=list)
     up_order: List[torch.Tensor] = field(default_factory=list)
+    need: List[NeedLists] = field(default_factory=list)
 
 
 def build_pyramid(coords: torch.Tensor, depth: int, blk_seg: Optional[torch.Tensor] = None, n_seg: int = 1) -> RulebookPyramid:
@@ -105,7 +113,7 @@
 
 
 def brick_pyramid(coords: torch.Tensor, depth: int, n_blocks: int, coord_bound: int, blk_seg: Optional[torch.Tensor] = None,
-                  n_seg: int = 1):
+                  n_seg: int = 1, inner_mask: Optional[torch.Tensor] = None):
     L = _lib.lib()
     dev = coords.device
     n0 = coords.shape[0]
@@ -114,6 +122,10 @@
     if blk_seg is None or blk_seg.numel() == 0:
         n_seg = 1
     i32 = dict(dtype=torch.int32, device=dev)
+    if inner_mask is not None:
+        if inner_mask.shape != (n0,) or inner_mask.element_size() != 1:
+            raise ValueError("brick_pyramid: inner_mask must be [n0] uint8 / bool")
+        inner_mask = inner_mask.contiguous().view(torch.uint8)
     for attempt in range(2):
         caps = [n0]
         for l in range(depth):
@@ -134,13 +146,17 @@
             down = [torch.empty((27, caps[l + 1]), **i32) for l in range(depth)]
             up = [torch.empty((27, caps[l]), **i32) for l in range(depth)]
             up_order = [torch.empty(caps[l] + 16, **i32) for l in range(depth)]
+            need_order = [torch.empty(caps[l], **i32) for l in range(depth)] if inner_mask is not None else []
+            up_need = [torch.empty(caps[l], **i32) for l in range(depth)] if inner_mask is not None else []
         except torch.OutOfMemoryError:
             return None
         arr = lambda ts: (ctypes.c_void_p * max(len(ts), 1))(*[t.data_ptr() for t in ts])
         counts = (ctypes.c_int64 * (depth + 1))()
-        rc = L.st_brick_pyramid(_lib.ptr(coords), n0, int(n_blocks), int(coord_bound), depth, _lib.ptr(blk_seg) if n_seg > 1 else None,
-                                n_seg, c_caps, _lib.ptr(order0), arr(coords_out), arr(subm), arr(down), arr(up), arr(up_order), counts,
-                                _lib.ptr(ws), ws.numel(), _lib.stream(dev))
+        need_counts = (ctypes.c_int64 * max(4 * depth, 1))()
+        rc = L.st_brick_pyramid_need(_lib.ptr(coords), n0, int(n_blocks), int(coord_bound), depth, _lib.ptr(blk_seg) if n_seg > 1 else None,
+                                     n_seg, c_caps, _lib.ptr(order0), arr(coords_out), arr(subm), arr(down), arr(up), arr(up_order), counts,
+                                     _lib.ptr(inner_mask), arr(need_order), arr(up_need), need_counts, _lib.ptr(ws), ws.numel(),
+                                     _lib.stream(dev))
         if rc == 0:
             break
         if b"outside the declared bounds" in L.st_last_error():
@@ -149,7 +165,7 @@
             _lib.check(rc)
         if attempt == 1:
             return None
-        del ws, order0, coords_out, subm, down, up, up_order
+        del ws, order0, coords_out, subm, down, up, up_order, need_order, up_need
     n = [int(counts[l]) for l in range(depth + 1)]
     pyr = RulebookPyramid()
     for l in range(depth + 1):
@@ -159,6 +175,9 @@
             pyr.down.append(down[l][:, : n[l + 1]])
             pyr.up.append(up[l][:, : n[l]])
             pyr.up_order.append(up_order[l][: n[l]])
+            if inner_mask is not None:
+                c = tuple(int(need_counts[4 * l + t]) for t in range(4))
+                pyr.need.append(NeedLists(need_order[l][: c[2]], c[:3], up_need[l][: c[3]]))
     return pyr, order0
 
 
@@ -186,10 +205,17 @@
     return order
 
 
-def move_rows(x: torch.Tensor, order: torch.Tensor, scatter: bool = False) -> torch.Tensor:
+def move_rows(x: torch.Tensor, order: torch.Tensor, scatter: bool = False, rows: Optional[torch.Tensor] = None) -> torch.Tensor:
     L = _lib.lib()
     x = x.contiguous()
     assert x.element_size() in (4, 2) and x.ndim == 2 and order.dtype == torch.int32
+    if rows is not None:
+        assert x.element_size() == 4 and rows.dtype == torch.int32
+        out = torch.zeros_like(x)
+        if rows.numel():
+            _lib.check(L.st_move_rows_list(_lib.ptr(x), x.shape[1], _lib.ptr(order), _lib.ptr(rows), rows.numel(), _lib.ptr(out), int(scatter),
+                                           _lib.stream(x.device)))
+        return out
     out = torch.empty_like(x)
     move = L.st_move_rows if x.element_size() == 4 else L.st_move_rows_h
     if x.element_size() == 4 or x.shape[1]:
@@ -278,52 +304,73 @@
                 shift: Optional[torch.Tensor] = None, residual: Optional[torch.Tensor] = None,
                 relu: bool = False, wp: Optional[torch.Tensor] = None, out_half: bool = False,
                 wp16: Optional[torch.Tensor] = None, row_order: Optional[torch.Tensor] = None,
-                wq: Optional[torch.Tensor] = None) -> torch.Tensor:
+                wq: Optional[torch.Tensor] = None, level_rows: Optional[int] = None, parity: Optional[bool] = None) -> torch.Tensor:
     L = _lib.lib()
     K, cin, cout = w.shape
     c0 = x0.shape[1]
     nbr_ptr, nbr_stride = _nbr_args(nbr)
+    listed = level_rows is not None
+    if listed and row_order is None:
+        raise ValueError("sparse_conv: level_rows needs the list of rows (row_order)")
+    n_rows = int(level_rows) if listed else n_out
+    if parity is None:
+        parity = row_order is not None
     if n_out == 0:
-        return torch.empty((0, cout), dtype=torch.float16 if out_half else torch.float32, device=x0.device)
+        return _conv_output(n_rows, cout, out_half, x0.device)
     in_half = x0.dtype == torch.float16
-    big_16 = cin == 16 and cout == 16 and nbr is not None and row_order is None and x1 is None
+    big_16 = cin == 16 and cout == 16 and nbr is not None and not parity and x1 is None
     mid, tail = (), ()
     if in_half or out_half:
         both = in_half and out_half
         if both and wp16 is None:
             raise ValueError("half -> half convolution needs the half-precision MFMA weights (wp16)")
-        entry, wt, mid = L.st_sparse_conv_f16_fwd, (wp16 if both else w), (int(in_half), int(out_half))
+        entry, wt, mid = "st_sparse_conv_f16_fwd", (wp16 if both else w), (int(in_half), int(out_half))
         name = f"k_sparse_conv_mfma_f16x<{cin},{cout}>" if both else f"k_sparse_conv<{cin},{cout}> {'h->f' if in_half else 'f->h'}"
     elif wq is not None and b3_eligible(cin, cout, c0):
-        entry, wt, name, tail = L.st_sparse_conv_b3_fwd, wq, f"k_sparse_conv_mfma_b3<{cin},{cout}>", (int(B3_VARIANT),)
+        entry, wt, name, tail = "st_sparse_conv_b3_fwd", wq, f"k_sparse_conv_mfma_b3<{cin},{cout}>", (int(B3_VARIANT),)
     elif wp is not None and mfma_eligible(cin, cout, c0) and not big_16:
-        entry, wt, name, tail = L.st_sparse_conv_mfma_fwd, wp, f"k_sparse_conv_mfma<{cin},{cout}>", (int(MFMA_VARIANT),)
+        entry, wt, name, tail = "st_sparse_conv_mfma_fwd", wp, f"k_sparse_conv_mfma<{cin},{cout}>", (int(MFMA_VARIANT),)
     else:
-        entry, wt, name = L.st_sparse_conv_fwd, w, f"k_sparse_conv<{cin},{cout}>"
+        entry, wt, name = "st_sparse_conv_fwd", w, f"k_sparse_conv<{cin},{cout}>"
+    if listed and entry != "st_sparse_conv_fwd":
+        entry, tail = entry.replace("_fwd", "_list_fwd"), tail + (n_rows, int(parity))
+    entry = getattr(L, entry)
     esz_in, esz_out = (2 if in_half else 4), (2 if out_half else 4)
-    y = torch.empty((n_out, cout), dtype=torch.float16 if out_half else torch.float32, device=x0.device)
-    nbytes = (lambda: (_pair_count(nbr) if nbr is not None else n_out) * (cin * esz_in + (4 if nbr is not None else 0))
+    y = _conv_output(n_rows, cout, out_half, x0.device)
+    rows = row_order[:n_out] if listed else None
+    nbytes = (lambda: (_pair_count(nbr, rows) if nbr is not None else n_out) * (cin * esz_in + (4 if nbr is not None else 0))
               + n_out * cout * esz_out) if profiling.enabled() else 0
-    nflops = (lambda: 2.0 * (_pair_count(nbr) if nbr is not None else n_out) * cin * cout) if profiling.enabled() else 0
+    nflops = (lambda: 2.0 * (_pair_count(nbr, rows) if nbr is not None else n_out) * cin * cout) if profiling.enabled() else 0
     with profiling.kernel(name + ("" if nbr is not None else " k1"), nbytes, nflops):
         _lib.check(entry(_lib.ptr(x0), c0, _lib.ptr(x1), cin, nbr_ptr, K, n_out, _lib.ptr(wt), cout, _lib.ptr(scale), _lib.ptr(shift),
                          _lib.ptr(residual), int(relu), _lib.ptr(y), *mid, _lib.ptr(row_order), _lib.stream(x0.device), nbr_stride, *tail))
     return y
 
 
+POISON_OUTPUTS = False
+
+
+def _conv_output(n_rows: int, cout: int, out_half: bool, device) -> torch.Tensor:
+    dtype = torch.float16 if out_half else torch.float32
+    if POISON_OUTPUTS:
+        return torch.full((n_rows, cout), float("nan"), dtype=dtype, device=device)
+    return torch.empty((n_rows, cout), dtype=dtype, device=device)
+
+
 _pairs_cache = {}
 
 
-def _pair_count(nbr: torch.Tensor) -> int:
-    key = (id(nbr), profiling.generation())
+def _pair_count(nbr: torch.Tensor, rows: Optional[torch.Tensor] = None) -> int:
+    key = (id(nbr), id(rows), profiling.generation())
     if key not in _pairs_cache:
         if len(_pairs_cache) > 4096:
             _pairs_cache.clear()
-        _pairs_cache[key] = int((nbr >= 0).sum().item())
+        cols = nbr if rows is None else nbr[:, (rows & 0x0FFFFFFF).long()]
+        _pairs_cache[key] = int((cols >= 0).sum().item())
     return _pairs_cache[key]
 
 
-def mlp_heads(x: torch.Tensor, params: torch.Tensor, with_tail: bool = False):
+def mlp_heads(x: torch.Tensor, params: torch.Tensor, with_tail: bool = False, keep: Optional[torch.Tensor] = None):
     L = _lib.lib()
     n, dev = x.shape[0], x.device
     radius = torch.empty((n, 1), dtype=torch.float32, device=dev)
@@ -333,6 +380,6 @@
     cls = torch.empty((n, 1), dtype=torch.int64, device=dev) if with_tail else None
     if n == 0:
         return radius, direction, class_l, mv, cls
-    _lib.check(L.st_pointwise_mlp_heads(_lib.ptr(x), n, _lib.ptr(params), _lib.ptr(radius), _lib.ptr(direction),
-                                        _lib.ptr(class_l), _lib.ptr(mv), _lib.ptr(cls), _lib.stream(dev)))
+    _lib.check(L.st_pointwise_mlp_heads_keep(_lib.ptr(x), n, _lib.ptr(keep), _lib.ptr(params), _lib.ptr(radius), _lib.ptr(direction),
+                                             _lib.ptr(class_l), _lib.ptr(mv), _lib.ptr(cls), _lib.stream(dev)))
     return radius, direction, class_l, mv, cls
```

After: 976.4 million (median of 6 runs). +4.6%, better.
